# sid2364/dna-sequences-pg-extension

Hardware: AMD Instinct MI355X
Metric: k-mers/sec for k=31 count over 3 Gbase synthetic; % of HBM-read roofline (higher is better)
Workload: dtype u64; 1 GPU; config 4: k=31 count over 3000000000 synthetic bases (splitmix64 seed 0xd2a0003), unordered groups (super-k-mer partitioning), single GPU; n_bases=3000000000, k=31, distinct=2999999968

## Files before the change

dna-sequences-pg-extension_amd/binding.py:

```python
import ctypes as C
import os

import numpy as np

_HERE = os.path.dirname(os.path.abspath(__file__))
_LIB = None

OK = 0
ERR_INVALID_K = 1
ERR_QKMER_LEN_MISMATCH = 2
ERR_PREFIX_TOO_LONG = 3
ERR_QKMER_INVALID = 4
ERR_BAD_ARG = 5
ERR_TOO_LARGE = 6
ERR_NO_DEVICE = 7
ERR_OOM = 8
ERR_HIP = 9
ERR_DNA_EMPTY = 11
ERR_DNA_INVALID_CHAR = 12
DEBUG_POISON_POOL = 1
DEBUG_FORCE_SUPERKMER = 2
DEBUG_HEAVY_EXPAND = 4
DEBUG_GUARD_POOL = 8
DEBUG_NO_SPEC1 = 16
# ... 151 lines not shown
    L.dnagpu_multi_size.argtypes = [vp]
    L.dnagpu_multi_ctx.argtypes = [vp, C.c_int]
    L.dnagpu_multi_ctx.restype = vp
    L.dnagpu_multi_transport.argtypes = [vp]
    L.dnagpu_multi_transport.restype = C.c_char_p
    L.dnagpu_multi_dna_upload.argtypes = [vp, u64p, C.c_uint64, C.POINTER(vp)]
    L.dnagpu_multi_dna_synth.argtypes = [vp, C.c_uint64, C.c_uint64, C.c_uint64, C.POINTER(vp)]
    L.dnagpu_multi_dna_length.argtypes = [vp]
    L.dnagpu_multi_dna_length.restype = C.c_uint64
    L.dnagpu_multi_dna_free.argtypes = [vp, vp]
    L.dnagpu_multi_dna_free.restype = None
    L.dnagpu_count_multi.argtypes = [vp, vp, C.c_int, C.c_uint64, C.c_uint64, C.POINTER(vp)]
    L.dnagpu_count_multi_unordered.argtypes = [vp, vp, C.c_int, C.c_uint64, C.c_uint64, C.POINTER(vp)]
    L.dnagpu_device_count.restype = C.c_int
    L.dnagpu_multi_set_option.argtypes = [vp, C.c_int, C.c_double]
    L.dnagpu_multi_last_times.argtypes = [vp, C.POINTER(_MultiTimes)]
    L.dnagpu_multi_exchange_transport.argtypes = [vp]
    L.dnagpu_multi_exchange_transport.restype = C.c_char_p
    L.dnagpu_multi_rccl_ranks.argtypes = [vp]
    L.dnagpu_multi_last_phase_times.argtypes = [vp, C.c_int, C.POINTER(_PhaseTimes)]
    L.dnagpu_hist_parts.argtypes = [vp]
    L.dnagpu_hist_parts.restype = C.c_uint32
    L.dnagpu_hist_part.argtypes = [vp, C.c_uint32]
    L.dnagpu_hist_part.restype = vp
    L.dnagpu_last_phase_times.argtypes = [vp, C.POINTER(_PhaseTimes)]
    L.dnagpu_set_profiling.argtypes = [vp, C.c_int]
    L.dnagpu_set_debug.argtypes = [vp, C.c_uint]
    _LIB = L
    return L


class DnaGpuError(Exception):
    def __init__(self, code):
        self.code = code
        self.message = lib().dnagpu_strerror(code).decode()
        detail = lib().dnagpu_last_error().decode()
        super().__init__(self.message + (f" [{detail}]" if detail and code >= ERR_BAD_ARG else ""))


def _chk(rc):
    if rc != OK:
        raise DnaGpuError(rc)


def strerror(code):
    return lib().dnagpu_strerror(code).decode()


def device_count():
    return int(lib().dnagpu_device_count())


def abi_version():
    return lib().dnagpu_abi_version()


def kmer_count(n_bases, k):
    out = C.c_uint64()
    _chk(lib().dnagpu_kmer_count(n_bases, k, C.byref(out)))
    return out.value


class Filter:

    def __init__(self, kind, length=0, bits=0, pattern=""):
        self.c = _FilterC()
        self.c.kind = kind
        self.c.length = length
        self.c.bits = int(bits)
        self.c.pattern = pattern.encode()[:35]

    @staticmethod
    def equals(length, bits):
        return Filter(FILTER_EQUALS, length, bits)

    @staticmethod
    def starts_with(length, bits):
        return Filter(FILTER_STARTS_WITH, length, bits)

    @staticmethod
    def contains(pattern):
        return Filter(FILTER_CONTAINS, 0, 0, pattern)


class Dna:
    def __init__(self, ctx, handle):
        self.ctx, self.h = ctx, handle

    @property
    def n_bases(self):
        return int(lib().dnagpu_dna_length(self.h))

    @property
    def device_words(self):
        return lib().dnagpu_dna_device_words(self.h)

    def download(self):
        nw = (self.n_bases + 31) // 32
        out = np.empty(max(nw, 1), dtype=np.uint64)
        _chk(lib().dnagpu_dna_download(self.ctx.h, self.h, out.ctypes.data_as(u64p)))
        return out[:nw]

    def set_sequences(self, seq_starts):
        st = np.ascontiguousarray(seq_starts, dtype=np.uint64)
        _chk(lib().dnagpu_dna_set_sequences(self.ctx.h, self.h, st.ctypes.data_as(u64p), max(len(st) - 1, 0)))

    @property
    def n_sequences(self):
        return int(lib().dnagpu_dna_sequences(self.h))

    def free(self):
        if self.h:
            lib().dnagpu_dna_free(self.ctx.h, self.h)
            self.h = None


class Records:

    def __init__(self, ctx, h):
        self.ctx, self.h = ctx, h
        self.n_buckets = int(lib().dnagpu_records_buckets(h))
        self.offsets = np.zeros(self.n_buckets + 1, dtype=np.uint64)
        _chk(lib().dnagpu_records_offsets(h, self.offsets.ctypes.data_as(u64p)))
        self.device_ptr = lib().dnagpu_records_device(h)
        self.n_records = int(self.offsets[-1])

    def free(self):
        if self.h:
            lib().dnagpu_records_free(self.ctx.h, self.h)
            self.h = None


class _CountQueries:

    _obj = None

    def _q(self, name):
        return getattr(lib(), f"dnagpu_{self._obj}_{name}")

    def spectrum(self, n_bins):
        bins = np.zeros(max(int(n_bins), 1), dtype=np.uint64)
        _chk(self._q("spectrum")(self.ctx.h, self.h, n_bins, bins.ctypes.data_as(u64p)))
        return bins[:n_bins]

    def select(self, min_count, max_count=U64_MAX, cap=None, on_device=False, out=None):
        n = C.c_uint64()
        fn = self._q("select")
        if cap is None:
            _chk(fn(self.ctx.h, self.h, min_count, max_count, None, None, 0, C.byref(n), 0))
            cap = n.value
        if on_device:
            dk, dc = out if out is not None else (self.ctx.buffer_alloc(8 * max(cap, 1)), self.ctx.buffer_alloc(8 * max(cap, 1)))
            _chk(fn(self.ctx.h, self.h, min_count, max_count, dk, dc, cap, C.byref(n), 1))
            return n.value if out is not None else (dk, dc, n.value)
        keys = np.empty(max(cap, 1), dtype=np.uint64)
        counts = np.empty(max(cap, 1), dtype=np.uint64)
        _chk(fn(self.ctx.h, self.h, min_count, max_count, keys.ctypes.data, counts.ctypes.data, cap, C.byref(n), 0))
        m = min(n.value, cap)
        return keys[:m], counts[:m], n.value

    def top(self, n, on_device=False, out=None):
        got = C.c_uint64()
        fn = self._q("top")
        if on_device:
            dk, dc = out if out is not None else (self.ctx.buffer_alloc(8 * max(n, 1)), self.ctx.buffer_alloc(8 * max(n, 1)))
            _chk(fn(self.ctx.h, self.h, n, dk, dc, C.byref(got), 1))
            return got.value if out is not None else (dk, dc, got.value)
        rows = min(n, self.distinct)
        keys = np.empty(max(rows, 1), dtype=np.uint64)
        counts = np.empty(max(rows, 1), dtype=np.uint64)
        _chk(fn(self.ctx.h, self.h, n, keys.ctypes.data, counts.ctypes.data, C.byref(got), 0))
        return keys[:got.value], counts[:got.value]


class Hist(_CountQueries):
    _obj = "hist"

    def __init__(self, ctx, handle):
        self.ctx, self.h = ctx, handle

    @property
    def distinct(self):
        return int(lib().dnagpu_hist_distinct(self.h))

    @property
    def total(self):
        return int(lib().dnagpu_hist_total(self.h))

    @property
    def extent(self):
        return int(lib().dnagpu_hist_extent(self.h))

    @property
    def device_keys(self):
        return lib().dnagpu_hist_device_keys(self.h)

    @property
    def device_counts(self):
        return lib().dnagpu_hist_device_counts(self.h)

    @property
    def n_parts(self):
        return int(lib().dnagpu_hist_parts(self.h))

    def part_arrays(self, i):
        ph = C.c_void_p(lib().dnagpu_hist_part(self.h, i))
        return (lib().dnagpu_hist_device_keys(ph), lib().dnagpu_hist_device_counts(ph), int(lib().dnagpu_hist_extent(ph)))

    @property
    def is_sorted(self):
        return bool(lib().dnagpu_hist_is_sorted(self.h))

    def download(self, first=0, count=None, want_keys=True, want_counts=True):
        if count is None:
            count = self.distinct - first
        keys = np.empty(max(count, 1), dtype=np.uint64) if want_keys else None
        counts = np.empty(max(count, 1), dtype=np.uint64) if want_counts else None
        _chk(lib().dnagpu_hist_download(self.ctx.h, self.h, first, count,
                                        keys.ctypes.data_as(u64p) if want_keys else None,
                                        counts.ctypes.data_as(u64p) if want_counts else None))
        return (keys[:count] if want_keys else None, counts[:count] if want_counts else None)

    def sorted_view_device(self, dev_keys, dev_counts, first=0, count=None):
        if count is None:
            count = self.distinct - first
        _chk(lib().dnagpu_hist_sorted_view(self.ctx.h, self.h, first, count, dev_keys, dev_counts))

    def summary(self):
        t, u, c = C.c_uint64(), C.c_uint64(), C.c_uint64()
        _chk(lib().dnagpu_hist_summary(self.ctx.h, self.h, C.byref(t), C.byref(u), C.byref(c)))
        return t.value, self.distinct, u.value, c.value

    def merge(self, other):
        h = C.c_void_p()
        _chk(lib().dnagpu_hist_merge(self.ctx.h, self.h, other.h, C.byref(h)))
        return Hist(self.ctx, h)

    def free(self):
        if self.h:
            if self.ctx._base_debug & DEBUG_GUARD_POOL:
                self.ctx.synchronize()
            lib().dnagpu_hist_free(self.ctx.h, self.h)
            self.h = None


class Accumulator(_CountQueries):

    _obj = "acc"

    def __init__(self, ctx, k):
        self.ctx, self.h = ctx, C.c_void_p()
        _chk(lib().dnagpu_acc_create(ctx.h, k, C.byref(self.h)))

    def add(self, hist):
        _chk(lib().dnagpu_acc_add(self.ctx.h, self.h, hist.h))

    @property
    def distinct(self):
        return int(lib().dnagpu_acc_distinct(self.h))

    @property
    def total(self):
        return int(lib().dnagpu_acc_total(self.h))

    def summary(self):
        t, u, c = C.c_uint64(), C.c_uint64(), C.c_uint64()
        _chk(lib().dnagpu_acc_summary(self.ctx.h, self.h, C.byref(t), C.byref(u), C.byref(c)))
        return t.value, self.distinct, u.value, c.value

    def download(self, first=0, count=None):
        if count is None:
            count = self.distinct - first
        keys = np.empty(max(count, 1), dtype=np.uint64)
        counts = np.empty(max(count, 1), dtype=np.uint64)
        _chk(lib().dnagpu_acc_download(self.ctx.h, self.h, first, count, keys.ctypes.data_as(u64p),
                                       counts.ctypes.data_as(u64p)))
        return keys[:count], counts[:count]

    def free(self):
        if self.h:
            if self.ctx._base_debug & DEBUG_GUARD_POOL:
                self.ctx.synchronize()
            lib().dnagpu_acc_free(self.ctx.h, self.h)
            self.h = None

    def __enter__(self):
        return self

    def __exit__(self, *a):
        self.free()


class Context:
    def __init__(self, device=0):
        self.h = C.c_void_p()
        _chk(lib().dnagpu_init(device, C.byref(self.h)))
        self._base_debug = _env_debug()
        if self._base_debug:
            self.set_debug(0)

    def set_debug(self, flags):
        _chk(lib().dnagpu_set_debug(self.h, int(flags) | self._base_debug))

    def close(self):
        if self.h:
            lib().dnagpu_destroy(self.h)
            self.h = None

    def __enter__(self):
        return self

    def __exit__(self, *a):
        self.close()

    def synchronize(self):
        _chk(lib().dnagpu_synchronize(self.h))

    @property
    def stream(self):
        return lib().dnagpu_stream(self.h)

    def trim(self):
        _chk(lib().dnagpu_trim(self.h))

    def device_bytes(self):
        return int(lib().dnagpu_device_bytes(self.h))

    def set_profiling(self, on):
        _chk(lib().dnagpu_set_profiling(self.h, int(bool(on))))

    def last_phase_times(self):
        pt = _PhaseTimes()
        _chk(lib().dnagpu_last_phase_times(self.h, C.byref(pt)))
        return [(pt.names[i].decode(), float(pt.ms[i])) for i in range(pt.n)]

    def upload(self, words, n_bases):
        w = np.ascontiguousarray(words, dtype=np.uint64)
        if w.size < (n_bases + 31) // 32:
            raise ValueError("words shorter than n_bases")
        h = C.c_void_p()
        _chk(lib().dnagpu_dna_upload(self.h, w.ctypes.data_as(u64p), n_bases, C.byref(h)))
        return Dna(self, h)

    def wrap(self, dev_ptr, n_words, n_bases):
        h = C.c_void_p()
        _chk(lib().dnagpu_dna_wrap(self.h, dev_ptr, n_words, n_bases, C.byref(h)))
        return Dna(self, h)

    def _pack(self, text, n_bases, on_device):
        h = C.c_void_p()
        pos, ch = C.c_uint64(), C.create_string_buffer(1)
        rc = lib().dnagpu_dna_pack(self.h, text, n_bases, on_device, C.byref(h), C.byref(pos), ch)
        if rc == ERR_DNA_INVALID_CHAR:
            e = DnaGpuError(rc)
            e.message = f"{e.message}: {ch.raw.decode(errors='replace')}"
            e.bad_pos = pos.value
            e.bad_char = ch.raw
            e.args = (e.message,)
            raise e
        _chk(rc)
        return Dna(self, h)

    def pack(self, text):
        b = text.encode() if isinstance(text, str) else bytes(text)
        return self._pack(b, len(b), 0)

    def pack_device(self, dev_text, n_bases):
        return self._pack(C.cast(C.c_void_p(dev_text), C.c_char_p), n_bases, 1)

    def unpack(self, dna, first=0, count=None):
        if count is None:
            count = dna.n_bases - first
        buf = C.create_string_buffer(max(count, 1))
        _chk(lib().dnagpu_dna_unpack(self.h, dna.h, first, count, buf, 0))
        return buf.raw[:count].decode()

    def unpack_device(self, dna, first, count, dev_text):
        _chk(lib().dnagpu_dna_unpack(self.h, dna.h, first, count, dev_text, 1))

    def from_wire_device(self, dev_wire, wire_bytes):
        h = C.c_void_p()
        _chk(lib().dnagpu_dna_from_wire(self.h, dev_wire, wire_bytes, 1, C.byref(h)))
        return Dna(self, h)

    def to_wire_device(self, dna, dev_wire, wire_cap):
        _chk(lib().dnagpu_dna_to_wire(self.h, dna.h, dev_wire, wire_cap, 1))

    def kmers_to_text_device(self, dev_keys, n, k, dev_text):
        _chk(lib().dnagpu_kmers_to_text(self.h, dev_keys, n, k, dev_text, 1))

    def from_wire(self, wire):
        b = bytes(wire)
        h = C.c_void_p()
        _chk(lib().dnagpu_dna_from_wire(self.h, b, len(b), 0, C.byref(h)))
        return Dna(self, h)

    def to_wire(self, dna):
        n = lib().dnagpu_dna_wire_size(dna.n_bases)
        buf = C.create_string_buffer(int(n))
        _chk(lib().dnagpu_dna_to_wire(self.h, dna.h, buf, n, 0))
        return buf.raw

    def kmers_to_text(self, keys, k):
        a = np.ascontiguousarray(keys, dtype=np.uint64)
        buf = C.create_string_buffer(max(a.size * (k + 1), 1))
        _chk(lib().dnagpu_kmers_to_text(self.h, a.ctypes.data, a.size, k, buf, 0))
        raw = buf.raw
        return [raw[i * (k + 1): i * (k + 1) + k].decode() for i in range(a.size)]

    def synth(self, seed, n_bases, motif_len=0):
        h = C.c_void_p()
        _chk(lib().dnagpu_dna_synth(self.h, seed, n_bases, motif_len, C.byref(h)))
        return Dna(self, h)

    def generate_kmers(self, dna, k, first=0, count=None):
        total = kmer_count(dna.n_bases, k)
        if count is None:
            count = max(total - first, 0)
        out = np.empty(max(count, 1), dtype=np.uint64)
        _chk(lib().dnagpu_generate_kmers(self.h, dna.h, k, first, count, out.ctypes.data, 0))
        return out[:count]

    def generate_kmers_device(self, dna, k, first, count, dev_out):
        _chk(lib().dnagpu_generate_kmers(self.h, dna.h, k, first, count, dev_out, 1))

    def generate_kmers_filtered(self, dna, k, flt, first=0, count=None, cap=None, want_keys=True,
                                want_pos=True):
        total = kmer_count(dna.n_bases, k)
        if count is None:
            count = max(total - first, 0)
        if cap is None:
            cap = count
        keys = np.empty(max(cap, 1), dtype=np.uint64) if want_keys else None
        pos = np.empty(max(cap, 1), dtype=np.uint64) if want_pos else None
        n = C.c_uint64()
        _chk(lib().dnagpu_generate_kmers_filtered(
            self.h, dna.h, k, C.byref(flt.c), first, count,
            keys.ctypes.data if want_keys else None, pos.ctypes.data if want_pos else None,
            cap, C.byref(n), 0))
        m = min(n.value, cap)
        return (keys[:m] if want_keys else None, pos[:m] if want_pos else None, n.value)

    def count_matches_device(self, dna, k, flt, first, count, dev_keys=None, dev_pos=None, cap=0):
        n = C.c_uint64()
        _chk(lib().dnagpu_generate_kmers_filtered(self.h, dna.h, k, C.byref(flt.c), first, count,
                                                  dev_keys, dev_pos, cap, C.byref(n), 1))
        return n.value

    def count_kmers(self, dna, k, first=0, count=None):
        total = kmer_count(dna.n_bases, k)
        if count is None:
            count = max(total - first, 0)
        h = C.c_void_p()
        _chk(lib().dnagpu_count_kmers(self.h, dna.h, k, first, count, C.byref(h)))
        return Hist(self, h)

    def count_kmers_unordered(self, dna, k, first=0, count=None):
        total = kmer_count(dna.n_bases, k)
        if count is None:
            count = max(total - first, 0)
        h = C.c_void_p()
        _chk(lib().dnagpu_count_kmers_unordered(self.h, dna.h, k, first, count, C.byref(h)))
        return Hist(self, h)

    def count_kmers_batch(self, dna, seq_starts, k):
        st = np.ascontiguousarray(seq_starts, dtype=np.uint64)
        h = C.c_void_p()
        _chk(lib().dnagpu_count_kmers_batch(self.h, dna.h, st.ctypes.data_as(u64p), max(len(st) - 1, 0), k, C.byref(h)))
        return Hist(self, h)

    def count_kmers_table(self, dna, k):
        h = C.c_void_p()
        _chk(lib().dnagpu_count_kmers_table(self.h, dna.h, k, C.byref(h)))
        return Hist(self, h)

    def accumulator(self, k):
        return Accumulator(self, k)

    def sk_buckets(self, global_rows, k):
        return int(lib().dnagpu_sk_buckets(self.h, global_rows, k))

    def sk_records(self, dna, k, first, count, global_rows):
        r = C.c_void_p()
        _chk(lib().dnagpu_sk_records(self.h, dna.h, k, first, count, global_rows, C.byref(r)))
        return Records(self, r)

    def count_records(self, pieces, k, global_rows):
        n = len(pieces)
        ptrs = (C.c_void_p * max(n, 1))(*[C.c_void_p(int(p[0])) for p in pieces])
        lens = np.asarray([int(p[1]) for p in pieces], dtype=np.uint64)
        bks = np.asarray([int(p[2]) for p in pieces], dtype=np.uint32)
        h = C.c_void_p()
        _chk(lib().dnagpu_count_records(self.h, ptrs, lens.ctypes.data_as(u64p), bks.ctypes.data_as(C.POINTER(C.c_uint32)), n, k,
                                        global_rows, C.byref(h)))
        return Hist(self, h)

    def count_kmers_owned(self, dna, k, owner, n_owners, first=0, count=None):
        total = kmer_count(dna.n_bases, k)
        if count is None:
            count = max(total - first, 0)
        h = C.c_void_p()
        _chk(lib().dnagpu_count_kmers_owned(self.h, dna.h, k, first, count, owner, n_owners, C.byref(h)))
        return Hist(self, h)

    def count_keys_device(self, dev_keys, n, k):
        h = C.c_void_p()
        _chk(lib().dnagpu_count_keys(self.h, dev_keys, n, k, C.byref(h)))
        return Hist(self, h)

    def count_keys_device_in_range(self, dev_keys, n, k, key_min, key_max):
        h = C.c_void_p()
        _chk(lib().dnagpu_count_keys_in_range(self.h, dev_keys, n, k, key_min, key_max, C.byref(h)))
        return Hist(self, h)

    def partition_kmers(self, dna, k, first, count, n_owners):
        ptr = C.c_void_p()
        offs = np.zeros(n_owners + 1, dtype=np.uint64)
        _chk(lib().dnagpu_partition_kmers(self.h, dna.h, k, first, count, n_owners, C.byref(ptr),
                                          offs.ctypes.data_as(u64p)))
        return ptr.value, offs

    def buffer_alloc(self, nbytes):
        p = C.c_void_p()
        _chk(lib().dnagpu_buffer_alloc(self.h, nbytes, C.byref(p)))
        return p.value

    def buffer_free(self, ptr):
        lib().dnagpu_buffer_free(self.h, ptr)

    def download_bytes(self, ptr, n):
        out = np.empty(max(n, 1), dtype=np.uint8)
        _chk(lib().dnagpu_buffer_download(self.h, ptr, n, out.ctypes.data))
        return out[:n]

    def upload_bytes(self, ptr, arr):
        a = np.ascontiguousarray(arr, dtype=np.uint8)
        _chk(lib().dnagpu_buffer_upload(self.h, ptr, a.ctypes.data, a.size))

    def download_u64(self, ptr, n):
        out = np.empty(max(n, 1), dtype=np.uint64)
        _chk(lib().dnagpu_buffer_download(self.h, ptr, n * 8, out.ctypes.data))
        return out[:n]

    def upload_u64(self, ptr, arr):
        a = np.ascontiguousarray(arr, dtype=np.uint64)
        _chk(lib().dnagpu_buffer_upload(self.h, ptr, a.ctypes.data, a.size * 8))

    def kmer_hash(self, keys):
        k = np.ascontiguousarray(keys, dtype=np.uint64)
        out = np.empty(max(k.size, 1), dtype=np.uint32)
        _chk(lib().dnagpu_kmer_hash(self.h, k.ctypes.data, k.size, out.ctypes.data, 0))
        return out[:k.size]

    def kmer_hash_device(self, dev_keys, n, dev_out):
        _chk(lib().dnagpu_kmer_hash(self.h, dev_keys, n, dev_out, 1))

    def kmer_match_device(self, dev_keys, n, k, flt, dev_flags):
        _chk(lib().dnagpu_kmer_match(self.h, dev_keys, n, k, C.byref(flt.c), dev_flags, 1))

    def kmer_match(self, keys, k, flt):
        a = np.ascontiguousarray(keys, dtype=np.uint64)
        out = np.empty(max(a.size, 1), dtype=np.uint8)
        _chk(lib().dnagpu_kmer_match(self.h, a.ctypes.data, a.size, k, C.byref(flt.c), out.ctypes.data, 0))
        return out[:a.size].astype(bool)


MULTI_AUTO, MULTI_RCCL, MULTI_COPY = 0, 1, 2
MULTI_OPT_PARTS, MULTI_OPT_EMULATE_LINK_GBS, MULTI_OPT_PROBE_OWNER, MULTI_OPT_EXCHANGE_RCCL = 1, 2, 3, 4


class _BorrowedContext(Context):

    def __init__(self, handle):
        self.h = C.c_void_p(handle)
        self._base_debug = _env_debug()
        if self._base_debug:
            self.set_debug(0)

    def close(self):
        self.h = None


class Multi:

    def __init__(self, devices, transport=MULTI_AUTO):
        n = len(devices)
        arr = (C.c_int * n)(*devices)
        self.h = C.c_void_p()
        _chk(lib().dnagpu_multi_init(arr, n, transport, C.byref(self.h)))
        self.n = n
        self.ranks = [_BorrowedContext(lib().dnagpu_multi_ctx(self.h, r)) for r in range(n)]

    @property
    def transport(self):
        return lib().dnagpu_multi_transport(self.h).decode()

    @property
    def exchange_transport(self):
        return lib().dnagpu_multi_exchange_transport(self.h).decode()

    @property
    def rccl_ranks(self):
        return int(lib().dnagpu_multi_rccl_ranks(self.h))

    def set_exchange_rccl(self, mode):
        _chk(lib().dnagpu_multi_set_option(self.h, MULTI_OPT_EXCHANGE_RCCL, float(mode)))
# ... 63 lines not shown
```

dna-sequences-pg-extension_amd/csrc/kernels.hpp:

```cpp
#pragma once
#include <hip/hip_runtime.h>
#include <stdint.h>

#include "kmer_device.hpp"

namespace dnagpu {

hipError_t launch_synth(u64 *words, u64 w_begin, u64 w_end, u64 n_bases, u64 seed, u64 motif_len, hipStream_t s);
hipError_t launch_extract(const u64 *words, u64 n_words, u64 first, u64 count, int k, u64 *out_keys,
                          hipStream_t s);

constexpr int FILTER_MAX_GROUPS = 8192;
void filter_bits_geometry(u64 count, u32 *n_groups, u32 *tiles_per_group);
hipError_t launch_filter_bits_count(const u64 *words, u64 n_words, u64 first, u64 count, const FilterBits &fb,
                                    u32 *group_counts, hipStream_t s);
hipError_t launch_filter_bits_write(const u64 *words, u64 n_words, u64 first, u64 count, int k, const FilterBits &fb,
                                    const u32 *group_counts, u64 *out_keys, u64 *out_pos, u64 cap, u64 *total_out,
                                    hipStream_t s);

hipError_t launch_hash_batch(const u64 *keys, u64 n, u32 *out, hipStream_t s);
hipError_t launch_match_batch(const u64 *keys, u64 n, const FilterDev &f, uint8_t *flags, hipStream_t s);
hipError_t launch_hist_summary(const u64 *keys, const u32 *counts, u64 n, u64 *result3, hipStream_t s);

hipError_t launch_pack(const unsigned char *text, u64 n_bases, u64 *words, u64 *bad_pos, hipStream_t s);
hipError_t launch_unpack(const u64 *words, u64 first, u64 count, unsigned char *text, hipStream_t s);
hipError_t launch_kmers_to_text(const u64 *keys, u64 n, int k, unsigned char *text, hipStream_t s);
hipError_t launch_wire_swap(const u64 *src, u64 *dst, u64 n_words, u64 last_mask, hipStream_t s);

u64 scan_tmp_words(u64 n);
struct ScanSet {
    const u32 *in[4];
    u32 *out[4];
    u32 *total[4];
    u32 *tmp;
};
hipError_t launch_scan_u32_multi(const ScanSet &set, int n_arrays, u64 n, hipStream_t s);
hipError_t launch_scan_u32(const u32 *in, u32 *out, u64 n, u32 *tmp, u32 *total, hipStream_t s);

constexpr int LEAF_CAP = 6144;
constexpr int LEAF_CAP_TINY = 1024;
constexpr int LEAF_CAP_SMALL = 4096;
constexpr int LEAF_TARGET = 5800;
constexpr int MAX_SPLIT_BITS = 10;
constexpr int ROW_STRIDE = 1 << MAX_SPLIT_BITS;

struct Node {
    u32 start;
    u32 len;
    u32 meta;
    u32 split;
    u64 prefix;
    u32 child_base;
    u32 chunk_base;
};
constexpr u32 NODE_BUF = 1u << 8;
constexpr u32 NODE_TERMINAL = 1u << 9;
constexpr u32 NODE_SKIP = 1u << 10;
constexpr u32 NODE_PEEL = 1u << 11;
constexpr int NODE_STAT_WORDS = 8;

struct Chunk {
    u32 node;
    u32 off;
    u32 len;
    u32 pad;
};

struct LevelCounters {
    u32 n_next;
    u32 n_chunks;
    u32 n_split;
    u32 n_scatter;
    u32 max_bits;
    u32 n_big;
    u32 n_small;
    u32 n_tiny;
    u32 n_over;
};

hipError_t launch_plan(Node *nodes, u32 n_nodes, int level, u32 chunk_len, u32 *outc, u32 *nch,
                       LevelCounters *ctr, hipStream_t s, int skew_from = 2);
hipError_t launch_plan_level(Node *nodes, u32 n_nodes, int level, u32 chunk_len, u32 *outc, u32 *nch, u32 *scan_tmp,
                             LevelCounters *ctr, hipStream_t s, int skew_from = 2);
hipError_t launch_fill_chunks(const Node *nodes, u32 n_nodes, u32 chunk_len, const u32 *child_base,
                              const u32 *chunk_base, Node *nodes_rw, Chunk *chunks, hipStream_t s);
hipError_t launch_level_hist(const Node *nodes, const Chunk *chunks, u32 n_chunks, int src_dna,
                             const u64 *words, u64 n_words, u64 first, int k, const u64 *buf0,
                             const u64 *buf1, u32 *hist, u32 flt_lo, u32 flt_span, u32 flt_tb, u32 *vary, int multi_ref,
                             u32 stat_min_len, hipStream_t s);
hipError_t launch_level_prefix(const Node *nodes, const Chunk *chunks, u32 n_chunks, u32 n_split_nodes, u32 chunk_len,
                               u32 *hist, u32 *tot, hipStream_t s, u32 n_nodes = 0);
hipError_t launch_level_children(Node *nodes, u32 n_nodes, u32 *tot, Node *next, u32 *vary, const u64 *buf0,
                                 const u64 *buf1, u32 stat_min_len, hipStream_t s);
hipError_t launch_peel_scatter(const Node *nodes, u32 n_nodes, const Chunk *chunks, u32 n_chunks, Node *next, u64 *buf0,
                               u64 *buf1, u32 *stat, hipStream_t s);
hipError_t launch_level_scatter(const Node *nodes, const Chunk *chunks, u32 n_chunks, int src_dna,
                                const u64 *words, u64 n_words, u64 first, int k, u64 *buf0, u64 *buf1,
                                const u32 *hist, const u32 *tot, u32 flt_lo, u32 flt_span, u32 flt_tb, u32 max_bits,
                                hipStream_t s);
hipError_t launch_leaves(const Node *leaves, u32 n_leaves, u32 n_tiny, u32 n_small, u32 n_big, const u64 *buf0, const u64 *buf1,
                         u64 *cursor, u64 *seg_off, u32 *seg_cnt, u64 *out_keys, u32 *out_counts, u32 *flags,
                         u32 *scan_tmp, u32 *list, hipStream_t s, bool hashed = false, u64 out_base = 0);
int dense_max_bits();
hipError_t launch_dense_count(const u64 *words, u64 n_words, u64 first, u64 count, int bits, u32 *table, u64 *out_keys,
                              u32 *out_counts, u64 *n_out, hipStream_t s);
hipError_t launch_dense_table(const u64 *words, u64 n_words, u64 first, u64 count, int bits, u32 *table, hipStream_t s);
hipError_t launch_dense_compact(const u32 *table, int bits, u64 *out_keys, u32 *out_counts, u64 *n_out, hipStream_t s);
hipError_t launch_table_add(u32 *dst, const u32 *src, u32 n, hipStream_t s);
hipError_t launch_gather_sorted(const u64 *seg_off, const u32 *seg_cnt, const u32 *seg_pre, u32 n_leaves,
                                u64 first, u64 count, const u64 *keys, const u32 *counts, u64 *dst_keys,
                                u64 *dst_counts, hipStream_t s);

hipError_t launch_merge_insert(const u64 *keys, const u32 *counts, u64 n, u64 *tkeys, u32 *tcnt, u64 t_slots,
                               unsigned long long *ones, hipStream_t s);
hipError_t launch_merge_compact(const u64 *tkeys, const u32 *tcnt, u64 t_slots, u64 *out_keys, u32 *out_counts,
                                unsigned long long *cursor, hipStream_t s);

constexpr int ACC_SLOTS = 4096;
hipError_t launch_acc_bin(const u64 *keys, const u32 *counts, u64 n, int pbits, u32 *cursor, u64 *bins, u32 bin_cap,
                          hipStream_t s);
hipError_t launch_acc_bin_stats(const u32 *occ, const u32 *cursor, u64 P, u32 *stats, hipStream_t s);
hipError_t launch_acc_merge(u64 *table, u32 *occ, u64 P, const u32 *cursor, const u64 *bins, u32 bin_cap, int commit, u32 *stats,
                            hipStream_t s);
hipError_t launch_acc_split(const u64 *old_table, const u32 *old_occ, int old_bits, u64 *new_table, u32 *new_occ, int new_bits,
                            u32 *stats, hipStream_t s);
hipError_t launch_acc_summary(const u64 *table, const u32 *occ, u64 P, u64 *res3, hipStream_t s);
hipError_t launch_acc_gather(const u64 *table, const u32 *occ, const u64 *pre, u64 p_lo, u64 n_parts, u64 first, u64 count,
                             u64 *out_keys, u64 *out_counts, hipStream_t s);

constexpr int Q_TILE = 2048;
constexpr int Q_DIGITS = 2048;
constexpr u32 Q_LDS_BINS = 8192;
struct QHistSrc {
    const u64 *keys;
    const u32 *counts;
    u64 n;
};
struct QAccSrc {
    const u64 *table;
    const u32 *occ;
    u64 n;
};
struct QDigit {
    int spectrum;
    u64 n_bins;
    int shift;
    int has_prefix;
    int prefix_shift;
    u64 prefix;
    u32 lds_bins;
    int want_max;
};
hipError_t launch_query_digits(const QHistSrc &s, const QDigit &a, u64 *bins, u64 *maxc, hipStream_t st);
hipError_t launch_query_digits(const QAccSrc &s, const QDigit &a, u64 *bins, u64 *maxc, hipStream_t st);
hipError_t launch_query_select(const QHistSrc &s, u64 lo, u64 hi, u64 *out_keys, u64 *out_counts, u64 cap, u64 *cursor,
                               hipStream_t st);
hipError_t launch_query_select(const QAccSrc &s, u64 lo, u64 hi, u64 *out_keys, u64 *out_counts, u64 cap, u64 *cursor,
                               hipStream_t st);
hipError_t launch_query_sort(u64 *keys, u64 *counts, u32 m, hipStream_t st);

hipError_t launch_batch_marks(const u64 *starts, u64 n_seqs, u32 *marks, u64 n_mark_words, hipStream_t s);
hipError_t launch_batch_rows(const u64 *starts, u64 n_seqs, int k, u64 *rows, hipStream_t s);
hipError_t launch_batch_keys(const u64 *words, u64 n_words, const u32 *marks, u64 n_mark_words, u64 n_rows, int k, u64 *out_keys,
                             unsigned long long *cursor, hipStream_t s);

int sk_min_k();
int sk_minimizer_len(int k);
int sk_tile_rows();
int sk_max_c0();
hipError_t launch_sk_level0(bool scatter, const Chunk *chunks, u32 n_chunks, const u64 *words, u64 n_words, u64 first, int k,
                            u32 c0n, u32 b1bits, u32 r0bits, u32 *hist, const u32 *tot, void *recs, hipStream_t s,
                            u32 *aux = nullptr, const u32 *marks = nullptr, u64 n_mark_words = 0);
hipError_t launch_sk_sample_chunks(Chunk *chunks, u32 n_chunks, u32 stride, u32 len, u32 n, hipStream_t s);
int sk_slab_words();
u32 sk_slab_cap(u32 est, u64 chunk_rows, u64 sampled);
hipError_t launch_sk_slab_init(const u32 *est, u32 r0bits, u32 chunk_rows, u32 sampled, u32 n_chunks, u32 *slab, Node *nodes,
                               hipStream_t s);
hipError_t launch_sk_hist1(const Node *nodes, const Chunk *chunks, u32 n_chunks, const void *recs, u32 *hist, u32 *kcount,
                           hipStream_t s, bool by_d2 = false);
hipError_t launch_sk_scatter1(const Node *nodes, const Chunk *chunks, u32 n_chunks, const void *src, void *dst, const u32 *hist,
                              const u32 *tot, hipStream_t s, bool by_d2 = false, u32 *gcur = nullptr);
u64 sk_spec_span(u32 len, int bits);
hipError_t launch_sk_spec_regions(const Node *nodes, u32 n_nodes, u32 *spec, u32 *out, u32 *gcur, hipStream_t s,
                                  const u32 *rstart = nullptr);
hipError_t launch_sk_scatter1_spec(const Node *nodes, const Chunk *chunks, u32 n_chunks, const void *src, void *dst, u32 *gcur,
                                   const u32 *spec, u32 *kcount, u32 *over, hipStream_t s, const u32 *rstart = nullptr,
                                   const u32 *rcap = nullptr);
hipError_t launch_sk_spec_nodes(const Node *nodes, u32 n_nodes, const u32 *spec, const u32 *gcur, Node *next, u32 *over,
                                hipStream_t s, const u32 *rstart = nullptr, const u32 *rcap = nullptr);
u32 sk_sample1_len();
u32 sk_sample1_every();
hipError_t launch_sk_sampled_regions(const Node *nodes, const Chunk *samples, u32 n_samples, const void *recs, u32 n_mid, u32 *est,
                                     u32 *rcap, u32 *rstart, u32 *scan_tmp, u32 *total, hipStream_t s);
hipError_t launch_sk_heavy_finals(const Node *kids, u32 n, const u32 *kcount, Node *out, hipStream_t s);
int sk_flat_slice();
hipError_t launch_sk_take_heavy(Node *mids, const u32 *idx, u32 n_heavy, const u32 *kcount, Node *out, hipStream_t s);
hipError_t launch_sk_slice_count(const Node *buckets, u32 nb, u32 *n_slices, hipStream_t s);
hipError_t launch_sk_slice_fill(const Node *buckets, u32 nb, const u32 *slice_first, u32 *slice_rec0, u32 *slice_nrec, hipStream_t s);
hipError_t launch_sk_slice_kmers(const void *recs, const u32 *slice_rec0, const u32 *slice_nrec, u32 n_slices, u32 *slice_km,
                                 hipStream_t s);
hipError_t launch_sk_slice_nodes(const Node *buckets, u32 nb, const u32 *slice_first, const u32 *slice_koff, u32 n_slices,
                                 const u32 *total_keys, u32 key_base, int k, bool check_kmers, Node *out, u64 *n_bad, hipStream_t s);
hipError_t launch_sk_unmix(u64 *keys, u64 first, const u64 *end, u64 max_groups, int k, hipStream_t s);
hipError_t launch_sk_expand_flat(const void *recs, const u32 *slice_rec0, const u32 *slice_nrec, const u32 *slice_koff, u32 key_base,
                                 u32 n_slices, int k, u64 *keys, hipStream_t s);
int sk_regroup_tile();
hipError_t launch_sk_regroup(const Node *mids, u32 n_mids, const void *src, void *dst, Node *out_nodes, bool any_long, hipStream_t s);
hipError_t launch_sk_count(const Node *fin, const u32 *list, const u32 *list_off, u32 n_list, const void *recs, int k, u64 *n_groups,
                           u64 *seg_off, u32 *seg_cnt, u64 *out_keys, u32 *out_counts, u32 *left, hipStream_t s);

int sk_count_cap();
hipError_t launch_sk_select_flags(const Node *fin, u32 n_fin, u32 cap, u32 big_limit, u32 *f_small, u32 *f_big, u32 *k_range,
                                  u32 *k_big, hipStream_t s);
hipError_t launch_sk_select_lists(const Node *fin, u32 n_fin, u32 cap, u32 big_limit, const u32 *p_small, const u32 *p_big,
                                  const u32 *kb_range, u32 *list_small, u32 *off_small, u32 *list_big, u32 *off_big, hipStream_t s);
hipError_t launch_sk_over_flags(const Node *fin, u32 n_fin, u32 cap, u32 big_limit, const u32 *p_big, const u32 *big_status,
                                u32 *f_over, u32 *k_over, hipStream_t s);
hipError_t launch_sk_over_list(const Node *fin, u32 n_fin, const u32 *f_raw, const u32 *p_over, const u32 *kb_over, Node *over_nodes,
                               u32 *over_kbase, hipStream_t s);
hipError_t launch_sk_node_lens(const Node *nodes, u32 n, u32 *lens, hipStream_t s);
u32 sk_big_slice_records();
u64 sk_big_partial_slots();
hipError_t launch_sk_big_slices(const Node *fin, const u32 *list, u32 n_list, u32 *nsl, u32 *msl, hipStream_t s);
hipError_t launch_sk_big_slice_fill(const u32 *nsl_raw, const u32 *sfirst, u32 n_list, u32 *sl_bucket, u32 *sl_idx, hipStream_t s);
hipError_t launch_sk_count_big(const Node *fin, const u32 *list, const u32 *list_off, const u32 *nsl, const u32 *mfirst,
                               const u32 *sl_bucket, const u32 *sl_idx, u32 n_slices, u32 n_list, const void *recs, int k,
                               u64 *n_groups, u64 *seg_off, u32 *seg_cnt, u64 *out_keys, u32 *out_counts, u32 *status, u64 *part_keys,
                               u32 *part_cnts, u32 *part_n, bool any_sliced, hipStream_t s);

int scatter_tile_keys();
int scatter_threads();

}
```

dna-sequences-pg-extension_amd/csrc/sk_host.hip:

```cpp
#include "host_common.hpp"

using namespace dnagpu;

constexpr u64 SK_LEAF_MEAN = 2500;
constexpr u64 SK_MID_LIMIT = (u64)1 << 27;
#ifndef SK_MID_RECORDS_LOG2
#define SK_MID_RECORDS_LOG2 16
#endif
constexpr u32 SK_MID_RECORDS = 1u << SK_MID_RECORDS_LOG2;
constexpr u64 SK_BIG_LIMIT = 0xFFFFFFFFull;
constexpr int SK_B1_MAX = 9;

struct SkLevel {
    Node *next;
    u32 n_next;
    u32 *hist, *tot;
    Chunk *chunks;
    u32 n_chunks;
};

static int sk_level_begin(dnagpu_ctx *ctx, PoolScope &ps, Node *cur, u32 n_nodes, int bits, u32 chunk_len, SkLevel *lv)
{
    hipStream_t st = ctx->stream;
    u32 *outc = nullptr, *nch = nullptr, *scan_tmp = nullptr;
    LevelCounters *ctr = nullptr;
    RC_TRY(ps.alloc(n_nodes, &outc));
    RC_TRY(ps.alloc(n_nodes, &nch));
    RC_TRY(ps.alloc((size_t)scan_tmp_words(n_nodes), &scan_tmp));
    RC_TRY(ps.alloc(1, &ctr));
    HIP_TRY(launch_plan_level(cur, n_nodes, -bits, chunk_len, outc, nch, scan_tmp, ctr, st));
    LevelCounters hc;
    RC_TRY(read_back(ctx, &hc, ctr, sizeof hc));
    lv->n_next = hc.n_next;
    lv->n_chunks = hc.n_chunks;
    RC_TRY(ps.alloc(std::max<u32>(hc.n_chunks, 1), &lv->chunks));
    RC_TRY(ps.alloc((size_t)std::max<u32>(hc.n_chunks, 1) * ROW_STRIDE, &lv->hist));
    RC_TRY(ps.alloc((size_t)std::max<u32>(hc.n_chunks, 1) * ROW_STRIDE, &lv->tot));
    RC_TRY(ps.alloc(std::max<u32>(hc.n_next, 1), &lv->next));
    HIP_TRY(launch_fill_chunks(cur, n_nodes, chunk_len, outc, nch, cur, lv->chunks, st));
    return DNAGPU_OK;
}

struct SkHeavy {
    Node *nodes = nullptr;
    u32 n = 0;
    bool counted = true;
    void *recs = nullptr;
    u64 total = 0;
};
SkGeom dnagpu::sk_geometry(const dnagpu_ctx *ctx, u64 n, int k)
{
    SkGeom g;
    const u64 leaf_mean = std::min<u64>(SK_LEAF_MEAN, 225 * (u64)(k - sk_minimizer_len(k) + 2));
    const u64 n_final = std::max<u64>(n / leaf_mean, 16);
    const u64 n_mid = (n_final + 15) / 16;
    g.b1 = 1;
    while (g.b1 < SK_B1_MAX && ((u64)1 << g.b1) < n_mid)
        g.b1++;
    g.c0n = (u32)std::min<u64>((n_mid + ((u64)1 << g.b1) - 1) >> g.b1, (u64)sk_max_c0());
    g.r0bits = 1;
    while ((1u << g.r0bits) < g.c0n)
        g.r0bits++;
    g.mid_limit = (ctx->debug_flags & DNAGPU_DEBUG_FORCE_SUPERKMER) ? 3 * (n / ((u64)g.c0n << g.b1) + 1) : SK_MID_LIMIT;
    return g;
}

static bool sk_even(const u32 *lens, u32 n, double tol, int b1 = 0, u64 *span_out = nullptr)
{
    u64 tot = 0, big = 0, used = 0, span = 0;
    for (u32 i = 0; i < n; i++) {
        tot += lens[i];
        big = std::max<u64>(big, lens[i]);
        used += lens[i] ? 1 : 0;
        if (span_out)
            span += sk_spec_span(lens[i], b1);
    }
    if (span_out)
        *span_out = span;
    return (double)big * (double)used <= tol * (double)tot + 64.0 * (double)used;
}

static int sk_level0_begin(dnagpu_ctx *ctx, PoolScope &ps, u64 n, int r0bits, u64 chunk_target, Node **cur_out, u32 *chunk_rows_out,
                           SkLevel *l0)
{
    Node root;
    memset(&root, 0, sizeof root);
    root.len = (u32)n;
    root.meta = 32;
    Node *cur = nullptr;
    RC_TRY(ps.alloc(1, &cur));
    HIP_TRY(poke(cur, &root, sizeof root, ctx->stream));
    const u64 tile = (u64)sk_tile_rows();
    u64 chunk_rows = std::max<u64>(4 * tile, (n + chunk_target - 1) / chunk_target);
    chunk_rows = (chunk_rows + tile - 1) / tile * tile;
    prof_mark(ctx, "sk_plan0");
    RC_TRY(sk_level_begin(ctx, ps, cur, 1, r0bits, (u32)chunk_rows, l0));
    *cur_out = cur;
    *chunk_rows_out = (u32)chunk_rows;
    return DNAGPU_OK;
}

static int sk_level0(dnagpu_ctx *ctx, PoolScope &ps, const SkRows &rows, int k, const SkGeom &g, void **rec0_out, Node **coarse,
                     u32 *n_coarse, std::vector<u32> *lens_out, u64 *n_recs_out, u64 *rec0_cap = nullptr)
{
    hipStream_t st = ctx->stream;
    const dnagpu_dna *dna = rows.dna;
    const int b1 = g.b1, r0bits = g.r0bits;
    const u32 c0n = g.c0n;
    Node *cur = nullptr;
    u32 chunk_rows = 0;
    SkLevel l0;
    RC_TRY(sk_level0_begin(ctx, ps, rows.n, r0bits, 4096, &cur, &chunk_rows, &l0));
    prof_mark(ctx, "sk_hist0");
    HIP_TRY(launch_sk_level0(false, l0.chunks, l0.n_chunks, dna->words, dna->n_words, rows.first, k, c0n, (u32)b1, (u32)r0bits,
                             l0.hist, nullptr, nullptr, st, nullptr, rows.marks, rows.n_mark_words));
    prof_mark(ctx, "sk_prefix0");
    HIP_TRY(launch_level_prefix(cur, l0.chunks, l0.n_chunks, 1, chunk_rows, l0.hist, l0.tot, st));
    HIP_TRY(launch_level_children(cur, 1, l0.tot, l0.next, nullptr, nullptr, nullptr, 0, st));
    std::vector<Node> kids(l0.n_next);
    RC_TRY(read_back(ctx, kids.data(), l0.next, (size_t)l0.n_next * sizeof(Node)));
    std::vector<u32> &lens = *lens_out;
    lens.resize(kids.size());
    u64 n_recs = 0;
    for (size_t i = 0; i < kids.size(); i++) {
        lens[i] = kids[i].len;
        n_recs += kids[i].len;
    }
    if (n_recs > 0xFFFFFFFFull)
        return DNAGPU_ERR_TOO_LARGE;
    void *rec0 = nullptr;
    u64 cap = std::max<u64>(n_recs, 1);
    if (rec0_cap) {
        u64 span = 0;
        const bool even = sk_even(lens.data(), (u32)lens.size(), 1.02, b1, &span);
        if (span <= 0xFFFFFFFFull)
            cap = std::max(cap, span);
        if ((ctx->debug_flags & DNAGPU_DEBUG_SAMPLE1) || !even) {
            const u64 roomy = n_recs + n_recs / 3 + ((u64)lens.size() << b1) * 136;
            if (roomy <= 0xFFFFFFFFull)
                cap = std::max(cap, roomy);
        }
        *rec0_cap = cap;
    }
    RC_TRY(pool_alloc(ctx, (size_t)cap * 16, &rec0));
    ps.ptrs.push_back(rec0);
    prof_mark(ctx, "sk_scatter0");
    HIP_TRY(launch_sk_level0(true, l0.chunks, l0.n_chunks, dna->words, dna->n_words, rows.first, k, c0n, (u32)b1, (u32)r0bits,
                             l0.hist, l0.tot, rec0, st, nullptr, rows.marks, rows.n_mark_words));
    *rec0_out = rec0;
    *coarse = l0.next;
    *n_coarse = l0.n_next;
    *n_recs_out = n_recs;
    return DNAGPU_OK;
}

constexpr u64 SK_SLAB_MIN_ROWS = (u64)1 << 29;
static int sk_level0_slab(dnagpu_ctx *ctx, PoolScope &ps, const SkRows &rows, int k, const SkGeom &g, void **rec0_out, Node **coarse,
                          u32 *n_coarse, std::vector<u32> *lens, u64 *n_recs, u64 *rec0_cap, bool *ok)
{
    hipStream_t st = ctx->stream;
    const dnagpu_dna *dna = rows.dna;
    const u64 first = rows.first, n = rows.n;
    *ok = false;
    const u32 r0n = 1u << g.r0bits;
    const u64 tile = (u64)sk_tile_rows();
    Node *cur = nullptr;
    u32 chunk_rows = 0;
    SkLevel l0;
    RC_TRY(sk_level0_begin(ctx, ps, n, g.r0bits, 1024, &cur, &chunk_rows, &l0));
    if (l0.n_chunks == 0)
        return DNAGPU_OK;
    const u64 samp_len = 4 * tile, samp_stride = 64 * samp_len;
    const u32 n_samp = (u32)((n + samp_stride - 1) / samp_stride);
    u64 sampled = 0;
    for (u32 i = 0; i < n_samp; i++)
        sampled += std::min<u64>(samp_len, n - (u64)i * samp_stride);
    Chunk *samp = nullptr;
    u32 *est = nullptr, *slab = nullptr;
    Node *nodes = nullptr;
    RC_TRY(ps.alloc((size_t)n_samp, &samp));
    RC_TRY(ps.alloc((size_t)sk_max_c0(), &est));
    RC_TRY(ps.alloc((size_t)sk_slab_words(), &slab));
    RC_TRY(ps.alloc((size_t)r0n, &nodes));
    prof_mark(ctx, "sk_sample0");
    HIP_TRY(hipMemsetAsync(est, 0, (size_t)sk_max_c0() * sizeof(u32), st));
    HIP_TRY(launch_sk_sample_chunks(samp, n_samp, (u32)samp_stride, (u32)samp_len, (u32)n, st));
    HIP_TRY(launch_sk_level0(false, samp, n_samp, dna->words, dna->n_words, first, k, g.c0n, (u32)g.b1, (u32)g.r0bits, nullptr, nullptr,
                             nullptr, st, est, rows.marks, rows.n_mark_words));
    HIP_TRY(launch_sk_slab_init(est, (u32)g.r0bits, chunk_rows, (u32)sampled, l0.n_chunks, slab, nodes, st));
    std::vector<u32> h_est(r0n);
    RC_TRY(read_back(ctx, h_est.data(), est, (size_t)r0n * sizeof(u32)));
    u64 tot = 0, span = 0, span1 = 0;
    lens->assign(r0n, 0);
    for (u32 d = 0; d < r0n; d++) {
        tot += h_est[d];
        const u64 len = (u64)sk_slab_cap(h_est[d], chunk_rows, sampled) * l0.n_chunks;
        span += len;
        if (len > 0xFFFFFFFFull)
            return DNAGPU_OK;
        (*lens)[d] = (u32)len;
        span1 += sk_spec_span((u32)len, g.b1);
    }
    if (tot == 0 || !sk_even(h_est.data(), r0n, 1.05) || span > 0xFFFFFFFFull)
        return DNAGPU_OK;
    const u64 cap = std::max<u64>(span, span1 <= 0xFFFFFFFFull ? span1 : 0);
    void *rec0 = nullptr;
    RC_TRY(pool_alloc(ctx, (size_t)std::max<u64>(cap, 1) * 16, &rec0));
    prof_mark(ctx, "sk_scatter0");
    const hipError_t e = launch_sk_level0(true, l0.chunks, l0.n_chunks, dna->words, dna->n_words, first, k, g.c0n, (u32)g.b1,
                                          (u32)g.r0bits, nullptr, nullptr, rec0, st, slab, rows.marks, rows.n_mark_words);
    u32 status[2] = {1, 0};
    int rc = e == hipSuccess ? read_back(ctx, status, slab + 18 * (size_t)sk_max_c0(), sizeof status) : DNAGPU_ERR_HIP;
    if (rc != DNAGPU_OK || status[0] || status[1] != (u32)span || (ctx->debug_flags & DNAGPU_DEBUG_SLAB0_OVERFLOW)) {
        pool_free(ctx, rec0);
        if (e != hipSuccess)
            set_err("sk_scatter0 (slabs): %s", hipGetErrorString(e));
        return rc;
    }
    ps.ptrs.push_back(rec0);
    *rec0_out = rec0;
    *coarse = nodes;
    *n_coarse = r0n;
    *n_recs = span;
    *rec0_cap = cap;
    *ok = true;
    return DNAGPU_OK;
}

static int sk_levels12(dnagpu_ctx *ctx, PoolScope &ps, const SkGeom &g, Node *coarse, u32 n_coarse, void *rec0, u64 n_recs, u64 n,
                       void **recs, Node **fin, u32 *n_fin, SkHeavy *heavy, u64 *n_kmers, const u32 *host_lens = nullptr,
                       u64 rec0_cap = 0)
{
    hipStream_t st = ctx->stream;
    const int b1 = g.b1;
    const u64 mid_limit = g.mid_limit;
    void *rec1 = nullptr;

    u64 chunk_recs = std::max<u64>(4 * 8192, (n_recs + 4095) / 4096);
    chunk_recs = (chunk_recs + 8191) / 8192 * 8192;
    prof_mark(ctx, "sk_plan1");
    SkLevel l1;
    RC_TRY(sk_level_begin(ctx, ps, coarse, n_coarse, b1, (u32)chunk_recs, &l1));
    u32 *kcount = nullptr;
    RC_TRY(ps.alloc(std::max<u32>(l1.n_next, 1), &kcount));
    HIP_TRY(hipMemsetAsync(kcount, 0, (size_t)std::max<u32>(l1.n_next, 1) * sizeof(u32), st));
    u32 *d_lens = nullptr;
    RC_TRY(ps.alloc((size_t)l1.n_next + 4, &d_lens));
    u32 *gcur = nullptr;
    RC_TRY(ps.alloc((size_t)std::max<u32>(l1.n_chunks, 1) * ROW_STRIDE, &gcur));
    std::vector<u32> kc(l1.n_next), rcn((size_t)l1.n_next + 4);
    auto lens_to_host = [&](u32 extra) -> int {
        const size_t nb = (size_t)l1.n_next * sizeof(u32), nb2 = nb + (size_t)extra * sizeof(u32);
        if (nb + nb2 <= MAILBOX_BYTES - 8) {
            char *mb = reinterpret_cast<char *>(ctx->mailbox);
            HIP_TRY(hipMemcpyAsync(mb, kcount, nb, hipMemcpyDeviceToHost, st));
            HIP_TRY(hipMemcpyAsync(mb + nb, d_lens, nb2, hipMemcpyDeviceToHost, st));
            HIP_TRY(hipStreamSynchronize(st));
            memcpy(kc.data(), mb, nb);
            memcpy(rcn.data(), mb + nb, nb2);
        } else {
            HIP_TRY(hipMemcpyAsync(kc.data(), kcount, nb, hipMemcpyDeviceToHost, st));
            RC_TRY(read_back(ctx, rcn.data(), d_lens, nb2));
        }
        return DNAGPU_OK;
    };
    u64 span = 0;
    bool even = true;
    if (host_lens) {
        even = sk_even(host_lens, n_coarse, 1.02, b1, &span);
    }
    const bool can_spec = host_lens && !(ctx->debug_flags & DNAGPU_DEBUG_NO_SPEC1) && n_coarse <= (u32)sk_max_c0() && l1.n_chunks > 0;
    const bool force_sample = (ctx->debug_flags & DNAGPU_DEBUG_SAMPLE1) != 0;
    bool spec = can_spec && even && !force_sample && span <= rec0_cap && span <= 0xFFFFFFFFull;
    u32 *rstart = nullptr, *rcapv = nullptr;
    bool sampled = false;
    if (can_spec && (!even || force_sample) && !spec) {
        std::vector<Chunk> samp;
        const u32 slen = sk_sample1_len(), sstep = slen * sk_sample1_every();
        for (u32 i = 0; i < n_coarse; i++)
            for (u64 off = 0; off < host_lens[i]; off += sstep) {
                Chunk c;
                c.node = i;
                c.off = (u32)off;
                c.len = (u32)std::min<u64>(slen, host_lens[i] - off);
                c.pad = 0;
                samp.push_back(c);
            }
        Chunk *d_samp = nullptr;
        u32 *est = nullptr, *stmp = nullptr, *tot1 = nullptr;
        RC_TRY(ps.alloc(std::max<size_t>(samp.size(), 1), &d_samp));
        RC_TRY(ps.alloc((size_t)l1.n_next, &est));
        RC_TRY(ps.alloc((size_t)l1.n_next, &rcapv));
        RC_TRY(ps.alloc((size_t)l1.n_next, &rstart));
        RC_TRY(ps.alloc((size_t)scan_tmp_words(l1.n_next), &stmp));
        RC_TRY(ps.alloc(1, &tot1));
        prof_mark(ctx, "sk_sample1");
        if (!samp.empty())
            HIP_TRY(hipMemcpyAsync(d_samp, samp.data(), samp.size() * sizeof(Chunk), hipMemcpyHostToDevice, st));
        HIP_TRY(launch_sk_sampled_regions(coarse, d_samp, (u32)samp.size(), rec0, l1.n_next, est, rcapv, rstart, stmp, tot1, st));
        u32 total = 0;
        RC_TRY(read_back(ctx, &total, tot1, sizeof total));
        u64 chk = 0;
        for (u32 i = 0; i < n_coarse; i++)
            chk += host_lens[i];
        if ((u64)total >= chk && (u64)total <= rec0_cap) {
            span = total;
            spec = sampled = true;
        }
    }
    bool moved = false;
    if (spec) {
        u32 *sp = nullptr;
        RC_TRY(ps.alloc((size_t)2 * n_coarse, &sp));
        u32 *status = d_lens + l1.n_next;
        prof_mark(ctx, "sk_spec1");
        HIP_TRY(launch_sk_spec_regions(coarse, n_coarse, sp, status, gcur, st, sampled ? rstart : nullptr));
        RC_TRY(pool_alloc(ctx, (size_t)std::max<u64>(std::max(n_recs, span), 1) * 16, &rec1));
        ps.ptrs.push_back(rec1);
        prof_mark(ctx, "sk_scatter1");
        HIP_TRY(launch_sk_scatter1_spec(coarse, l1.chunks, l1.n_chunks, rec0, rec1, gcur, sp, kcount, status + 2, st,
                                        sampled ? rstart : nullptr, sampled ? rcapv : nullptr));
        HIP_TRY(launch_sk_spec_nodes(coarse, n_coarse, sp, gcur, l1.next, status + 2, st, sampled ? rstart : nullptr,
                                     sampled ? rcapv : nullptr));
        HIP_TRY(launch_sk_node_lens(l1.next, l1.n_next, d_lens, st));
        RC_TRY(lens_to_host(3));
        const u32 *stw = rcn.data() + l1.n_next;
        if ((!sampled && stw[0] != (u32)span) || (!sampled && stw[1]) || stw[2] || (ctx->debug_flags & DNAGPU_DEBUG_SPEC1_OVERFLOW)) {
            spec = false;
            HIP_TRY(hipMemsetAsync(kcount, 0, (size_t)std::max<u32>(l1.n_next, 1) * sizeof(u32), st));
        } else {
            moved = true;
        }
    }
    if (!spec) {
        prof_mark(ctx, "sk_hist1");
        HIP_TRY(launch_sk_hist1(coarse, l1.chunks, l1.n_chunks, rec0, l1.hist, kcount, st));
        prof_mark(ctx, "sk_prefix1");
        HIP_TRY(launch_level_prefix(coarse, l1.chunks, l1.n_chunks, n_coarse, (u32)chunk_recs, l1.hist, l1.tot, st, n_coarse));
        HIP_TRY(launch_level_children(coarse, n_coarse, l1.tot, l1.next, nullptr, nullptr, nullptr, 0, st));
        HIP_TRY(launch_sk_node_lens(l1.next, l1.n_next, d_lens, st));
        RC_TRY(lens_to_host(0));
    }
    const bool forced = (ctx->debug_flags & DNAGPU_DEBUG_FORCE_SUPERKMER) != 0;
    auto is_heavy = [&](u32 i) { return kc[i] > mid_limit || (!forced && rcn[i] > SK_MID_RECORDS); };
    u64 run = 0, heaviest = 0;
    for (u32 i = 0; i < l1.n_next; i++) {
        run += kc[i];
        if (is_heavy(i))
            heaviest = std::max<u64>(heaviest, std::max<u64>(kc[i], mid_limit + 1));
    }
    if (n != 0 && run != n) {
        set_err("super-k-mer partition lost rows: %llu of %llu", (unsigned long long)run, (unsigned long long)n);
        return DNAGPU_ERR_INTERNAL;
    }
    if (run > 0xFFFFFFFFull)
        return DNAGPU_ERR_TOO_LARGE;
    *n_kmers = run;
    std::vector<u32> heavy_idx;
    if (heaviest > mid_limit) {
        for (u32 i = 0; i < l1.n_next; i++)
            if (is_heavy(i)) {
                heavy_idx.push_back(i);
                heavy->total += kc[i];
            }
        if (((ctx->debug_flags & DNAGPU_DEBUG_HEAVY_EXPAND) && heavy->total * 2 > run) || heavy_idx.size() > 32768)
            return DNAGPU_SK_SKEWED;
    }

    if (!moved) {
        if (!rec1) {
            RC_TRY(pool_alloc(ctx, (size_t)std::max<u64>(n_recs, 1) * 16, &rec1));
            ps.ptrs.push_back(rec1);
        }
        prof_mark(ctx, "sk_scatter1");
        HIP_TRY(hipMemcpyAsync(gcur, l1.tot, (size_t)std::max<u32>(l1.n_chunks, 1) * ROW_STRIDE * sizeof(u32), hipMemcpyDeviceToDevice, st));
        HIP_TRY(launch_sk_scatter1(coarse, l1.chunks, l1.n_chunks, rec0, rec1, l1.hist, l1.tot, st, false, gcur));
    }

    const u32 nh = (u32)heavy_idx.size();
    const bool heavy_expand = (ctx->debug_flags & DNAGPU_DEBUG_HEAVY_EXPAND) != 0;
    SkLevel lh;
    memset(&lh, 0, sizeof lh);
    u32 *kcount2 = nullptr;
    Node *hnodes = nullptr;
    if (nh) {
        u32 *d_idx = nullptr;
        RC_TRY(ps.alloc((size_t)nh, &d_idx));
        RC_TRY(ps.alloc((size_t)nh, &hnodes));
        HIP_TRY(hipMemcpyAsync(d_idx, heavy_idx.data(), (size_t)nh * sizeof(u32), hipMemcpyHostToDevice, st));
        HIP_TRY(launch_sk_take_heavy(l1.next, d_idx, nh, kcount, hnodes, st));
        HIP_TRY(hipStreamSynchronize(st));
        if (heavy_expand) {
            heavy->nodes = hnodes;
            heavy->n = nh;
            heavy->recs = rec1;
        } else {
            u64 hrecs = 0;
            for (u32 i : heavy_idx)
                hrecs += rcn[i];
            u64 chunk_h = std::max<u64>(4 * 8192, (hrecs + 4095) / 4096);
            chunk_h = (chunk_h + 8191) / 8192 * 8192;
            prof_mark(ctx, "sk_heavy_split");
            RC_TRY(sk_level_begin(ctx, ps, hnodes, nh, 4, (u32)chunk_h, &lh));
            RC_TRY(ps.alloc(std::max<u32>(lh.n_next, 1), &kcount2));
            HIP_TRY(hipMemsetAsync(kcount2, 0, (size_t)std::max<u32>(lh.n_next, 1) * sizeof(u32), st));
            HIP_TRY(launch_sk_hist1(hnodes, lh.chunks, lh.n_chunks, rec1, lh.hist, kcount2, st, true));
            HIP_TRY(launch_level_prefix(hnodes, lh.chunks, lh.n_chunks, nh, (u32)chunk_h, lh.hist, lh.tot, st, nh));
            HIP_TRY(launch_level_children(hnodes, nh, lh.tot, lh.next, nullptr, nullptr, nullptr, 0, st));
            HIP_TRY(launch_sk_scatter1(hnodes, lh.chunks, lh.n_chunks, rec1, rec0, lh.hist, lh.tot, st, true));
            heavy->total = 0;
        }
    }
    Node *fn = nullptr;
    RC_TRY(ps.alloc((size_t)l1.n_next * 16 + lh.n_next, &fn));
    prof_mark(ctx, "sk_regroup");
    bool any_long = false;
    for (u32 i = 0; i < l1.n_next && !any_long; i++)
        any_long = rcn[i] > (u32)sk_regroup_tile();
    HIP_TRY(launch_sk_regroup(l1.next, l1.n_next, rec1, rec0, fn, any_long, st));
    if (lh.n_next)
        HIP_TRY(launch_sk_heavy_finals(lh.next, lh.n_next, kcount2, fn + (size_t)l1.n_next * 16, st));
    if (nh == 0 || !heavy_expand)
        ps.free_now(rec1);
    *recs = rec0;
    *fin = fn;
    *n_fin = l1.n_next * 16 + lh.n_next;
    return DNAGPU_OK;
}

static int count_sk_tail(dnagpu_ctx *ctx, PoolScope &ps, void *recs, Node *fin, u32 n_fin, const SkHeavy &heavy, u64 n, int k,
                         dnagpu_hist *h)
{
    hipStream_t st = ctx->stream;
    const u32 n_heavy = heavy.n;
    prof_mark(ctx, "sk_select");
    const u32 cap = (u32)sk_count_cap();
    const u32 big_limit = (u32)SK_BIG_LIMIT;
    u32 *f_small = nullptr, *f_big = nullptr, *f_over = nullptr, *f_over_raw = nullptr, *k_over = nullptr, *k_range = nullptr,
        *scan_tmp = nullptr, *totals = nullptr, *list_small = nullptr, *off_small = nullptr, *list_big = nullptr, *off_big = nullptr;
    RC_TRY(ps.alloc((size_t)n_fin, &f_small));
    RC_TRY(ps.alloc((size_t)n_fin, &f_big));
    RC_TRY(ps.alloc((size_t)n_fin, &k_range));
    RC_TRY(ps.alloc((size_t)scan_tmp_words(n_fin) * 4, &scan_tmp));
    RC_TRY(ps.alloc(8, &totals));
    RC_TRY(ps.alloc((size_t)n_fin, &list_small));
    RC_TRY(ps.alloc((size_t)n_fin, &off_small));
    RC_TRY(ps.alloc((size_t)n_fin, &f_over));
    HIP_TRY(launch_sk_select_flags(fin, n_fin, cap, big_limit, f_small, f_big, k_range, f_over, st));
    {
        ScanSet ss;
        u32 *arr[4] = {f_small, f_big, k_range, f_over};
        for (int a = 0; a < 4; a++) {
            ss.in[a] = arr[a];
            ss.out[a] = arr[a];
            ss.total[a] = totals + a;
        }
        ss.tmp = scan_tmp;
        HIP_TRY(launch_scan_u32_multi(ss, 4, n_fin, st));
    }
    u32 ht[4] = {0, 0, 0, 0};
    RC_TRY(read_back(ctx, ht, totals, sizeof ht));
    const u32 n_small = ht[0], n_big = ht[1];
    const u64 small_keys = ht[2];
    const u64 out_cap = n + ht[3];
    RC_TRY(ps.alloc((size_t)std::max<u32>(n_big, 1), &list_big));
    RC_TRY(ps.alloc((size_t)std::max<u32>(n_big, 1), &off_big));
    HIP_TRY(launch_sk_select_lists(fin, n_fin, cap, big_limit, f_small, f_big, k_range, list_small, off_small, list_big, off_big, st));

    u64 *cursor = nullptr, *ok = nullptr;
    u32 *oc = nullptr;
    RC_TRY(ps.alloc(3, &cursor));
    RC_TRY(ps.alloc((size_t)out_cap, &ok));
    RC_TRY(ps.alloc((size_t)out_cap, &oc));
    {
        const u64 init[3] = {small_keys, 0, 0};
        HIP_TRY(poke(cursor, init, sizeof init, st));
    }
    u64 *seg_off = nullptr;
    u32 *seg_cnt = nullptr;
    u64 *seg_off_fin = nullptr;
    u32 *seg_cnt_fin = nullptr;
    RC_TRY(ps.alloc((size_t)std::max<u32>(n_fin, 1), &seg_off_fin));
    RC_TRY(ps.alloc((size_t)std::max<u32>(n_fin, 1), &seg_cnt_fin));
    HIP_TRY(hipMemsetAsync(seg_cnt_fin, 0, (size_t)n_fin * sizeof(u32), st));
    HIP_TRY(hipMemsetAsync(seg_off_fin, 0, (size_t)n_fin * sizeof(u64), st));
    u32 *big_status = nullptr;
    RC_TRY(ps.alloc((size_t)std::max<u32>(n_big, 1), &big_status));
    if (n_big) {
        prof_mark(ctx, "sk_count_big");
        u32 *nsl = nullptr, *sfirst = nullptr, *mfirst = nullptr, *sl_bucket = nullptr, *sl_idx = nullptr, *part_n = nullptr, *part_cnts = nullptr;
        u64 *part_keys = nullptr;
        RC_TRY(ps.alloc((size_t)n_big, &nsl));
        RC_TRY(ps.alloc((size_t)n_big, &sfirst));
        RC_TRY(ps.alloc((size_t)n_big, &mfirst));
        HIP_TRY(launch_sk_big_slices(fin, list_big, n_big, nsl, mfirst, st));
        HIP_TRY(launch_scan_u32(nsl, sfirst, n_big, scan_tmp, totals + 6, st));
        HIP_TRY(launch_scan_u32(mfirst, mfirst, n_big, scan_tmp, totals + 7, st));
        u32 hs[2] = {0, 0};
        RC_TRY(read_back(ctx, hs, totals + 6, sizeof hs));
        const u32 n_slices = hs[0], n_part = hs[1];
        RC_TRY(ps.alloc((size_t)std::max<u32>(n_slices, 1), &sl_bucket));
        RC_TRY(ps.alloc((size_t)std::max<u32>(n_slices, 1), &sl_idx));
        RC_TRY(ps.alloc((size_t)std::max<u32>(n_part, 1), &part_n));
        RC_TRY(ps.alloc((size_t)std::max<u32>(n_part, 1) * sk_big_partial_slots(), &part_keys));
        RC_TRY(ps.alloc((size_t)std::max<u32>(n_part, 1) * sk_big_partial_slots(), &part_cnts));
        HIP_TRY(launch_sk_big_slice_fill(nsl, sfirst, n_big, sl_bucket, sl_idx, st));
        HIP_TRY(launch_sk_count_big(fin, list_big, off_big, nsl, mfirst, sl_bucket, sl_idx, n_slices, n_big, recs, k, cursor + 2,
                                    seg_off_fin, seg_cnt_fin, ok, oc, big_status, part_keys, part_cnts, part_n, n_part > 0, st));
    }
    prof_mark(ctx, "sk_select_over");
    RC_TRY(ps.alloc((size_t)n_fin, &f_over_raw));
    RC_TRY(ps.alloc((size_t)n_fin, &k_over));
    HIP_TRY(launch_sk_over_flags(fin, n_fin, cap, big_limit, f_big, big_status, f_over_raw, k_over, st));
    {
        ScanSet ss;
        memset(&ss, 0, sizeof ss);
        ss.in[0] = f_over_raw;
        ss.out[0] = f_over;
        ss.total[0] = totals + 4;
        ss.in[1] = k_over;
        ss.out[1] = k_over;
        ss.total[1] = totals + 5;
        ss.tmp = scan_tmp;
        HIP_TRY(launch_scan_u32_multi(ss, 2, n_fin, st));
    }
    u32 ho[2] = {0, 0};
    RC_TRY(read_back(ctx, ho, totals + 4, sizeof ho));
    const u32 n_over = ho[0];
    const u64 over_keys = ho[1];
    Node *over_nodes = nullptr;
    u32 *over_kbase = nullptr;
    RC_TRY(ps.alloc((size_t)std::max<u32>(n_over, 1), &over_nodes));
    RC_TRY(ps.alloc((size_t)std::max<u32>(n_over, 1), &over_kbase));
    HIP_TRY(launch_sk_over_list(fin, n_fin, f_over_raw, f_over, k_over, over_nodes, over_kbase, st));
    TreeResult tr;
    memset(&tr, 0, sizeof tr);
    if (n_over + n_heavy > 0) {
        const u64 tree_keys = over_keys + heavy.total;
        if (tree_keys > 0xFFFFFFFFull)
            return DNAGPU_ERR_TOO_LARGE;
        const u32 n_tree = n_over + n_heavy;
        u64 *kbuf = nullptr;
        Node *knodes = nullptr;
        RC_TRY(ps.alloc((size_t)tree_keys, &kbuf));
        RC_TRY(ps.alloc((size_t)n_tree, &knodes));
        prof_mark(ctx, "sk_expand_flat");
        for (int part = 0; part < 2; part++) {
            const u32 nb = part == 0 ? n_over : n_heavy;
            if (nb == 0)
                continue;
            const void *rbuf = part == 0 ? recs : heavy.recs;
            const Node *bk = part == 0 ? over_nodes : heavy.nodes;
            u32 *sfirst = nullptr, *stmp = nullptr, *stot = nullptr;
            RC_TRY(ps.alloc((size_t)nb, &sfirst));
            RC_TRY(ps.alloc((size_t)scan_tmp_words(nb), &stmp));
            RC_TRY(ps.alloc(2, &stot));
            HIP_TRY(launch_sk_slice_count(bk, nb, sfirst, st));
            HIP_TRY(launch_scan_u32(sfirst, sfirst, nb, stmp, stot, st));
            u32 n_slices = 0;
            RC_TRY(read_back(ctx, &n_slices, stot, 4));
            u32 *d_r0 = nullptr, *d_nr = nullptr, *d_ko = nullptr, *ktmp = nullptr;
            RC_TRY(ps.alloc((size_t)std::max<u32>(n_slices, 1), &d_r0));
            RC_TRY(ps.alloc((size_t)std::max<u32>(n_slices, 1), &d_nr));
            RC_TRY(ps.alloc((size_t)std::max<u32>(n_slices, 1), &d_ko));
            RC_TRY(ps.alloc((size_t)scan_tmp_words(std::max<u32>(n_slices, 1)), &ktmp));
            HIP_TRY(launch_sk_slice_fill(bk, nb, sfirst, d_r0, d_nr, st));
            HIP_TRY(launch_sk_slice_kmers(rbuf, d_r0, d_nr, n_slices, d_ko, st));
            HIP_TRY(launch_scan_u32(d_ko, d_ko, n_slices, ktmp, stot + 1, st));
            const u32 key_base = part == 0 ? 0u : (u32)over_keys;
            HIP_TRY(launch_sk_slice_nodes(bk, nb, sfirst, d_ko, n_slices, stot + 1, key_base, k, part == 0 || heavy.counted,
                                          knodes + (part == 0 ? 0 : n_over), cursor + 1, st));
            HIP_TRY(launch_sk_expand_flat(rbuf, d_r0, d_nr, d_ko, key_base, n_slices, k, kbuf, st));
        }
        RC_TRY(run_tree(ctx, ps, nullptr, 0, tree_keys, k, kbuf, 0, &tr, 0, 0, true, 0, ~0u, 0, knodes, n_tree, 2));
    }
#ifdef DNAGPU_STAMPS
    fprintf(stderr, "[sk select] n_fin %u small %u big %u (k-mers of big %u) over %u (keys %llu) heavy %u (keys %llu) tree nodes %u tiny %u small %u big %u\n",
            n_fin, n_small, n_big, ht[3], n_over, (unsigned long long)over_keys, n_heavy, (unsigned long long)heavy.total, tr.n_nodes,
            tr.n_tiny, tr.n_small, tr.n_big);
#endif
    const u32 n_segs = n_fin + tr.n_nodes;
    RC_TRY(ps.alloc((size_t)n_segs, &seg_off));
    RC_TRY(ps.alloc((size_t)n_segs, &seg_cnt));
    HIP_TRY(hipMemcpyAsync(seg_cnt, seg_cnt_fin, (size_t)n_fin * sizeof(u32), hipMemcpyDeviceToDevice, st));
    HIP_TRY(hipMemcpyAsync(seg_off, seg_off_fin, (size_t)n_fin * sizeof(u64), hipMemcpyDeviceToDevice, st));
    if (tr.n_nodes > 0) {
        u32 *flags = nullptr, *ltmp = nullptr, *cls_list = nullptr;
        RC_TRY(ps.alloc((size_t)tr.n_nodes + 1, &flags));
        RC_TRY(ps.alloc((size_t)scan_tmp_words(tr.n_nodes), &ltmp));
        RC_TRY(ps.alloc((size_t)tr.n_nodes, &cls_list));
        prof_mark(ctx, "leaves");
        HIP_TRY(launch_leaves(tr.nodes, tr.n_nodes, tr.n_tiny, tr.n_small, tr.n_big, tr.buf0, tr.buf1, cursor, seg_off + n_fin,
                              seg_cnt + n_fin, ok, oc, flags, ltmp, cls_list, st, true, small_keys));
        HIP_TRY(launch_sk_unmix(ok, small_keys, cursor, tr.n_keys, k, st));
    }
    prof_mark(ctx, "sk_count");
    u32 *left = nullptr;
    RC_TRY(ps.alloc((size_t)2 * n_small + 1, &left));
    HIP_TRY(launch_sk_count(fin, list_small, off_small, n_small, recs, k, cursor + 2, seg_off, seg_cnt, ok, oc, left, st));
#ifdef DNAGPU_STAMPS
    {
        u32 nl = 0;
        RC_TRY(read_back(ctx, &nl, left + 2 * (size_t)n_small, 4));
        fprintf(stderr, "[sk count] %u small buckets, %u left to sk_count by sk_count_clean\n", n_small, nl);
    }
#endif
    prof_mark(ctx, "end");
    u64 fin_ctr[3] = {0, 0, 0};
    RC_TRY(read_back(ctx, fin_ctr, cursor, 24));
    const u64 extent = fin_ctr[0];
    const u64 total_groups = fin_ctr[2] + (extent - small_keys);
    if (fin_ctr[1] != 0) {
        set_err("super-k-mer count: %llu buckets whose records expand to a different number of k-mers than the partition counted",
                (unsigned long long)fin_ctr[1]);
        return DNAGPU_ERR_INTERNAL;
    }
    if (extent > out_cap) {
        set_err("super-k-mer count: %llu output slots used, %llu allocated", (unsigned long long)extent, (unsigned long long)out_cap);
        return DNAGPU_ERR_INTERNAL;
    }
    if (total_groups > n) {
        set_err("super-k-mer count: %llu groups for %llu rows", (unsigned long long)total_groups, (unsigned long long)n);
        return DNAGPU_ERR_INTERNAL;
    }
    h->total = n;
    hist_adopt(ps, h, ok, oc, seg_off, seg_cnt, n_segs, total_groups, false, extent);
    return DNAGPU_OK;
}

int dnagpu::count_sk(dnagpu_ctx *ctx, const SkRows &rows, int k, dnagpu_hist *h, u64 n_kmers_expected)
{
    PoolScope ps(ctx);
    const SkGeom g = sk_geometry(ctx, std::max<u64>(n_kmers_expected, 1), k);
    void *rec0 = nullptr, *recs = nullptr;
    Node *coarse = nullptr, *fin = nullptr;
    u32 n_coarse = 0, n_fin = 0;
    u64 n_recs = 0, n_kmers = 0;
    SkHeavy heavy;
    u64 rec0_cap = 0;
    std::vector<u32> lens;
    bool slabs = false;
    const unsigned dbg = ctx->debug_flags;
    if (!(dbg & DNAGPU_DEBUG_NO_SLAB0) && (rows.n >= SK_SLAB_MIN_ROWS || (dbg & (DNAGPU_DEBUG_SLAB0 | DNAGPU_DEBUG_SLAB0_OVERFLOW))))
        RC_TRY(sk_level0_slab(ctx, ps, rows, k, g, &rec0, &coarse, &n_coarse, &lens, &n_recs, &rec0_cap, &slabs));
    if (!slabs)
        RC_TRY(sk_level0(ctx, ps, rows, k, g, &rec0, &coarse, &n_coarse, &lens, &n_recs, &rec0_cap));
    RC_TRY(sk_levels12(ctx, ps, g, coarse, n_coarse, rec0, n_recs, n_kmers_expected, &recs, &fin, &n_fin, &heavy, &n_kmers,
                       lens.size() == n_coarse ? lens.data() : nullptr, rec0_cap));
    return count_sk_tail(ctx, ps, recs, fin, n_fin, heavy, n_kmers_expected, k, h);
}

u64 dnagpu::sk_received_cap(const std::vector<u64> &blen, u32 n_coarse, const SkGeom &g)
{
    u64 n_recs = 0, span = 0;
    for (u32 d = 0; d < n_coarse; d++) {
        n_recs += blen[d];
        span += sk_spec_span((u32)std::min<u64>(blen[d], 0xFFFFFFFFull), g.b1);
    }
    return span <= 0xFFFFFFFFull ? std::max(n_recs, span) : n_recs;
}

int dnagpu::count_sk_received(dnagpu_ctx *ctx, void *rec0, const std::vector<u64> &boff, const std::vector<u64> &blen, const SkGeom &g,
                              int k, dnagpu_hist *h, u64 rec0_cap)
{
    hipStream_t st = ctx->stream;
    PoolScope ps(ctx);
    ps.ptrs.push_back(rec0);
    const u32 n_coarse = 1u << g.r0bits;
    const u64 n_recs = boff[n_coarse];
    std::vector<Node> hn(n_coarse);
    for (u32 d = 0; d < n_coarse; d++) {
        memset(&hn[d], 0, sizeof(Node));
        hn[d].start = (u32)boff[d];
        hn[d].len = (u32)blen[d];
        hn[d].meta = (u32)(32 - g.r0bits);
    }
    Node *coarse = nullptr;
    RC_TRY(ps.alloc((size_t)n_coarse, &coarse));
    HIP_TRY(hipMemcpyAsync(coarse, hn.data(), (size_t)n_coarse * sizeof(Node), hipMemcpyHostToDevice, st));
    HIP_TRY(hipStreamSynchronize(st));
    void *recs = nullptr;
    Node *fin = nullptr;
    u32 n_fin = 0;
    u64 n_kmers = 0;
    SkHeavy heavy;
    std::vector<u32> lens(n_coarse);
    for (u32 d = 0; d < n_coarse; d++)
        lens[d] = (u32)blen[d];
    int rc = sk_levels12(ctx, ps, g, coarse, n_coarse, rec0, n_recs, 0, &recs, &fin, &n_fin, &heavy, &n_kmers, lens.data(), rec0_cap);
    if (rc == DNAGPU_SK_SKEWED) {
        heavy = SkHeavy();
        heavy.nodes = coarse;
        heavy.n = n_coarse;
        heavy.recs = rec0;
        heavy.total = n_kmers;
        heavy.counted = false;
        n_fin = 0;
        rc = DNAGPU_OK;
    }
    RC_TRY(rc);
    return count_sk_tail(ctx, ps, recs, fin, n_fin, heavy, n_kmers, k, h);
}

static int count_sk_records(dnagpu_ctx *ctx, const void *const *pieces, const u64 *piece_len, const u32 *piece_bucket, u32 n_pieces,
                            int k, u64 global_rows, dnagpu_hist *h)
{
    hipStream_t st = ctx->stream;
    const SkGeom g = sk_geometry(ctx, global_rows, k);
    const u32 n_coarse = 1u << g.r0bits;
    std::vector<u64> blen(n_coarse, 0), boff(n_coarse + 1, 0);
    for (u32 i = 0; i < n_pieces; i++) {
        if (piece_bucket[i] >= g.c0n || (piece_len[i] && !pieces[i]))
            return DNAGPU_ERR_BAD_ARG;
        blen[piece_bucket[i]] += piece_len[i];
    }
    for (u32 d = 0; d < n_coarse; d++)
        boff[d + 1] = boff[d] + blen[d];
    const u64 n_recs = boff[n_coarse];
    if (n_recs > 0xFFFFFFFFull)
        return DNAGPU_ERR_TOO_LARGE;
    if (n_recs == 0) {
        h->total = 0;
        return DNAGPU_OK;
    }
    void *rec0 = nullptr;
    const u64 cap0 = sk_received_cap(blen, n_coarse, g);
    RC_TRY(pool_alloc(ctx, (size_t)cap0 * 16, &rec0));
    std::vector<u64> fill(boff.begin(), boff.end() - 1);
    for (u32 i = 0; i < n_pieces; i++)
        if (piece_len[i]) {
            const hipError_t e = hipMemcpyAsync(static_cast<char *>(rec0) + fill[piece_bucket[i]] * 16, pieces[i], (size_t)piece_len[i] * 16,
                                                hipMemcpyDeviceToDevice, st);
            if (e != hipSuccess) {
                pool_free(ctx, rec0);
                set_err("record pieces: %s", hipGetErrorString(e));
                return DNAGPU_ERR_HIP;
            }
            fill[piece_bucket[i]] += piece_len[i];
        }
    return count_sk_received(ctx, rec0, boff, blen, g, k, h, cap0);
}

extern "C" int dnagpu_sk_buckets(const dnagpu_ctx *ctx, uint64_t global_rows, int k)
{
    if (!ctx || k < sk_min_k() || k > 32 || global_rows == 0 || global_rows > 0xFFFFFFFFull)
        return 0;
    return (int)sk_geometry(ctx, global_rows, k).c0n;
}

extern "C" int dnagpu_sk_records(dnagpu_ctx *ctx, const dnagpu_dna *dna, int k, uint64_t first, uint64_t count,
                                 uint64_t global_rows, dnagpu_records **out)
{
    return guarded([&]() -> int {
    if (!ctx || !dna || !out || k < sk_min_k() || k > 32 || global_rows < count || global_rows == 0 || global_rows > 0xFFFFFFFFull)
        return DNAGPU_ERR_BAD_ARG;
    RC_TRY(check_range(dna, k, first, count));
    HIP_TRY(hipSetDevice(ctx->device));
    const SkGeom g = sk_geometry(ctx, global_rows, k);
    std::unique_ptr<dnagpu_records> r(new (std::nothrow) dnagpu_records());
    if (!r)
        return DNAGPU_ERR_OOM;
    r->off.assign((size_t)g.c0n + 1, 0);
    if (count > 0) {
        PoolScope ps(ctx);
        void *rec0 = nullptr;
        Node *coarse = nullptr;
        u32 n_coarse = 0;
        u64 n_recs = 0;
        std::vector<u32> lens;
        prof_begin(ctx);
        const int rc = sk_level0(ctx, ps, SkRows{dna, first, count, nullptr, 0}, k, g, &rec0, &coarse, &n_coarse, &lens, &n_recs);
        prof_mark(ctx, "end");
        prof_end(ctx);
        RC_TRY(rc);
        for (u32 d = 0; d < g.c0n; d++)
            r->off[d + 1] = r->off[d] + (d < lens.size() ? lens[d] : 0);
        const hipError_t se = hipStreamSynchronize(ctx->stream);
        if (r->off[g.c0n] != n_recs || se != hipSuccess) {
            set_err("super-k-mer level 0: %llu records in the buckets, %llu counted (%s)", (unsigned long long)r->off[g.c0n],
                    (unsigned long long)n_recs, hipGetErrorString(se));
            return se != hipSuccess ? DNAGPU_ERR_HIP : DNAGPU_ERR_INTERNAL;
        }
        ps.release(rec0);
        r->recs = rec0;
    }
    *out = r.release();
    return DNAGPU_OK;
    });
}

extern "C" uint32_t dnagpu_records_buckets(const dnagpu_records *r) { return r ? (uint32_t)(r->off.size() - 1) : 0; }
extern "C" int dnagpu_records_offsets(const dnagpu_records *r, uint64_t *offsets)
{
    if (!r || !offsets)
        return DNAGPU_ERR_BAD_ARG;
    for (size_t i = 0; i < r->off.size(); i++)
        offsets[i] = r->off[i];
    return DNAGPU_OK;
}
extern "C" void *dnagpu_records_device(const dnagpu_records *r) { return r ? r->recs : nullptr; }
extern "C" void dnagpu_records_free(dnagpu_ctx *ctx, dnagpu_records *r)
{
    if (!r)
        return;
    if (ctx)
        pool_free(ctx, r->recs);
    delete r;
}

extern "C" int dnagpu_count_records(dnagpu_ctx *ctx, const void *const *pieces, const uint64_t *piece_len,
                                    const uint32_t *piece_bucket, uint32_t n_pieces, int k, uint64_t global_rows, dnagpu_hist **out)
{
    return guarded([&]() -> int {
    if (!ctx || !out || (n_pieces && (!pieces || !piece_len || !piece_bucket)) || k < sk_min_k() || k > 32 || global_rows == 0 ||
        global_rows > 0xFFFFFFFFull)
        return DNAGPU_ERR_BAD_ARG;
    HIP_TRY(hipSetDevice(ctx->device));
    HistPtr h = hist_new(0, false);
    if (!h)
        return DNAGPU_ERR_OOM;
    prof_begin(ctx);
    const int rc = count_sk_records(ctx, pieces, piece_len, piece_bucket, n_pieces, k, global_rows, h.get());
    prof_end(ctx);
    RC_TRY(rc);
    *out = h.release();
    return DNAGPU_OK;
    });
}
```

dna-sequences-pg-extension_amd/csrc/superkmer_kernels.hip:

```cpp
#include <algorithm>
#include <cstdlib>
#include <type_traits>

#include "kernels.hpp"

namespace dnagpu {

constexpr int SK_NT = 256;
constexpr int SKW_ROWS = 63 * 32;
constexpr int SK_TILE_ROWS = (SK_NT / 64) * SKW_ROWS;
constexpr int SK_MAX_C0 = 256;
constexpr int SKW_LIST = 768;
__host__ __device__ constexpr u32 sk_plain_max(int w) { return (u32)(2 * SKW_ROWS * 17 / (10 * (w + 1))) < (u32)SKW_LIST ? (u32)(2 * SKW_ROWS * 17 / (10 * (w + 1))) : (u32)SKW_LIST; }

int sk_tile_rows() { return SK_TILE_ROWS; }
int sk_max_c0() { return SK_MAX_C0; }
int sk_count_cap() { return 4096; }

typedef unsigned long long ull2_t __attribute__((ext_vector_type(2)));

constexpr int SK_REC_MULTI_BIT = 58;
constexpr int SK_POS_SHIFT = 39;
constexpr u32 SK_POS_MASK = 31u;
constexpr u32 SK_GPOS_MASK = 63u;
// ... 195 lines not shown
    const int lane = threadIdx.x & 63;
    u32 r0 = (u32)lane * 32;
    asm volatile("" : "+v"(r0));
    u32 lb = 0;
    u32 kprev = key.prev_last;
    const u32 k0 = key(0);
    u32 kcur = k0;
#pragma unroll 8
    for (int j = 0; j < 32; j++) {
        const bool brk = j == 0 ? (lane == 0 || kcur != kprev) : kcur != kprev;
        if (brk)
            lb = r0 + (u32)j + 1u;
        kprev = kcur;
        if (j < 31)
            kcur = key(j + 1);
    }
    const u32 before = wave_prev(wave_incl_max(lb));
    f.ns0 = before ? before - 1u : 0u;
    const bool first_break = lane == 0 || k0 != key.prev_last;
    f.c0 = first_break ? 0u : (r0 - f.ns0) % lmax;
    if (first_break)
        f.ns0 = r0;
}

template <int W, typename Keys, typename Emit>
__device__ __forceinline__ void sk_records_all(const SkFront<W> &f, const Keys &key, u32 lmax, Emit &&emit)
{
    u32 r0 = (u32)(threadIdx.x & 63) * 32;
    asm volatile("" : "+v"(r0));
    u32 c = f.c0;
    u32 kprev = 0, kcur = key(0);
#pragma unroll 8
    for (int j = 0; j < 32; j++) {
        const u32 nxt = j < 31 ? key(j + 1) : key.next_first;
        bool end = false;
        if ((u32)j < f.n_valid) {
            if (j > 0 && kcur != kprev)
                c = 0;
            end = r0 + (u32)j + 1 == f.n_rows || nxt != kcur || c + 1 == lmax;
        }
        emit(j, end, r0 + (u32)j, c + 1, f.hm[j], kcur);
        c = end ? 0u : c + 1;
        kprev = kcur;
        kcur = nxt;
    }
}

template <int W, typename Keys, typename Emit>
__device__ __forceinline__ void sk_records(const SkFront<W> &f, const Keys &key, u32 lmax, Emit &&emit)
{
    u32 r0 = (u32)(threadIdx.x & 63) * 32;
    asm volatile("" : "+v"(r0));
    u32 c = f.c0;
    u32 kprev = 0, kcur = key(0);
#pragma unroll 8
    for (int j = 0; j < 32; j++) {
        const u32 nxt = j < 31 ? key(j + 1) : key.next_first;
        if ((u32)j < f.n_valid) {
            if (j > 0 && kcur != kprev)
                c = 0;
            const bool last = r0 + (u32)j + 1 == f.n_rows;
            const bool end = last || nxt != kcur || c + 1 == lmax;
            if (end) {
                emit(j, r0 + (u32)j, c + 1, f.hm[j], kcur);
                c = 0;
            } else {
                c++;
            }
        }
        kprev = kcur;
        kcur = nxt;
    }
}

template <int W, bool BATCH>
__device__ __forceinline__ u32 sk_uniform_value(const SkFront<W> &f, const u64 *__restrict__ words, u64 n_words, u64 pos0, u32 mmask)
{
    const int lane = threadIdx.x & 63;
    u32 x = 0, y = f.hm[0];
#pragma unroll 2
    for (int j = 1; j < 32; j++) {
        x |= f.hm[j] ^ f.hm[0];
        if (BATCH)
            y &= f.hm[j];
    }
    const u32 h0 = (u32)__builtin_amdgcn_readfirstlane((int)f.hm[0]) >> 7;
    const bool same = lane == 63 || ((x >> 7) == 0 && (f.hm[0] >> 7) == h0 && (!BATCH || (y & 64u)));
    if (__ballot(!same))
        return ~0u;
    const u64 pos = pos0 + (u64)lane * 32;
    const u64 w = pos >> 5;
    const unsigned sh = (unsigned)(pos & 31) * 2;
    const u64 w0 = w < n_words ? words[w] : 0, w1 = w + 1 < n_words ? words[w + 1] : 0;
    u64 lo = w0, hi = w1;
    if (sh) {
        const u64 w2 = w + 2 < n_words ? words[w + 2] : 0;
        lo = (w0 >> sh) | (w1 << (64 - sh));
        hi = (w1 >> sh) | (w2 << (64 - sh));
    }
    const u32 v0 = (u32)sk_shr128(lo, hi, 2u * (f.hm[0] & SK_GPOS_MASK)) & mmask;
    u32 d = 0;
#pragma unroll 2
    for (int j = 1; j < 32; j++)
        d |= ((u32)sk_shr128(lo, hi, 2u * (f.hm[j] & SK_GPOS_MASK)) & mmask) ^ v0;
    const u32 V = (u32)__builtin_amdgcn_readfirstlane((int)v0);
    const bool ok = lane == 63 || (d == 0 && v0 == V);
    return __ballot(!ok) ? ~0u : V;
}

template <int W, bool BATCH>
__device__ __forceinline__ void sk_hist0_general(SkFront<W> &f, const u64 *__restrict__ words, u64 n_words, u64 pos0, u32 lmax, u32 mmask,
                                              u32 c0n, u32 *h )
{
    SkKeys<W, BATCH, true> vk(f, words, n_words, pos0, mmask);
    sk_front_open<W>(f, vk, lmax);
    vk.forget();
    if ((threadIdx.x & 63) < 63)
        sk_records<W>(f, vk, lmax, [&](int, u32, u32, u32 hmin, u32 v) {
            if (!BATCH || v != ~0u)
                atomicAdd(&h[sk_digit0(sk_digit_word(hmin), c0n)], 1u);
        });
}

template <int W, bool BATCH>
__global__ __launch_bounds__(SK_NT, 4) void sk_hist0_kernel(const Chunk *__restrict__ chunks, u32 n_chunks,
                                                         const u64 *__restrict__ words, u64 n_words, u64 first,
                                                         u32 lmax, u32 mmask, u32 c0n, u32 b1mask, u32 r0n ,
                                                         u32 *__restrict__ hist, u32 *__restrict__ accum ,
                                                         const u32 *__restrict__ marks, u64 n_mark_words)
{
    __shared__ u32 h[SK_MAX_C0 + 64];
    if (blockIdx.x >= n_chunks)
        return;
    const Chunk ch = chunks[blockIdx.x];
    const int wave = threadIdx.x >> 6, lane = threadIdx.x & 63;
    for (u32 d = threadIdx.x; d < r0n; d += SK_NT)
        h[d] = 0;
    __syncthreads();
    for (u32 t0 = (u32)wave * SKW_ROWS; t0 < ch.len; t0 += SK_TILE_ROWS) {
        const u32 n_rows = ch.len - t0 < (u32)SKW_ROWS ? ch.len - t0 : (u32)SKW_ROWS;
        SkFront<W> f;
        sk_front<W, BATCH>(f, words, n_words, first + ch.off + t0, n_rows, lmax, mmask, nullptr, marks, n_mark_words);
        bool plain = f.plain;
        const u32 nf = lane == 62 ? ~f.hm[31] : f.next_first;
        if (plain) {
            u32 cnt = 0;
#pragma unroll
            for (int j = 0; j < 32; j++)
                cnt += ((j < 31 ? f.hm[j + 1] : nf) != f.hm[j]) ? 1u : 0u;
            plain = wave_sum(lane < 63 ? cnt : 0u) <= sk_plain_max(W);
        }
        if (plain) {
            if (lane < 63) {
#pragma unroll
                for (int j = 0; j < 32; j++) {
                    const u32 nxt = j < 31 ? f.hm[j + 1] : nf;
                    const u32 d0 = sk_digit0(sk_digit_word(f.hm[j]), c0n);
                    atomicAdd(&h[nxt != f.hm[j] && (!BATCH || f.hm[j] >= 64u) ? d0 : (u32)SK_MAX_C0 + (u32)lane], 1u);
                }
            }
        } else {
            SkFront<W> fm = f;
            const u32 uv = fm.plain ? sk_uniform_value<W, BATCH>(fm, words, n_words, first + ch.off + t0, mmask) : ~0u;
            if (uv != ~0u) {
                if (lane == 0)
                    atomicAdd(&h[sk_digit0(sk_digit_word(fm.hm[0]), c0n)], ((u32)SKW_ROWS + lmax - 1u) / lmax);
            } else {
                sk_hist0_general<W, BATCH>(fm, words, n_words, first + ch.off + t0, lmax, mmask, c0n, h);
            }
        }
    }
    __syncthreads();
    if (accum) {
        for (u32 d = threadIdx.x; d < r0n; d += SK_NT)
            if (h[d])
                atomicAdd(&accum[d], h[d]);
        return;
    }
    u32 *row = hist + (u64)blockIdx.x * ROW_STRIDE;
    for (u32 d = threadIdx.x; d < r0n; d += SK_NT)
        row[d] = h[d];
}

struct SkBuild {
    u64 *wl;
    const u64 *wsh;
    u32 *gpos;
    const u32 *gend;
    ull2_t *recs;
    u32 fo, c0n, b1mask, mmask;
    int k, dbg;
};

template <bool BATCH>
__device__ __forceinline__ bool sk_build(const SkBuild &b, u32 wrun, int mode)
{
    const bool exact = mode != 0;
    const int dbg = b.dbg;
    (void)dbg;
    bool dropped = false;
    if (SK_DBG(2))
        return false;
    for (u32 e = threadIdx.x & 63u; e < wrun; e += 64) {
        const u64 en = b.wl[e];
        const u32 key = (u32)(en >> 32);
        if (BATCH && (exact ? key < 64u : key == ~0u))
            continue;
        const u32 end_row = (u32)en & 0xFFFFu;
        u32 v = key, hmin = key;
        if (exact) {
            const u32 xq = (end_row & ~31u) + (key & SK_GPOS_MASK) + b.fo;
            v = (u32)funnel(b.wsh[xq >> 5], b.wsh[(xq >> 5) + 1], (xq & 31u) * 2u) & b.mmask;
        } else {
            hmin = sk_hash_of(v);
        }
        const SkDigits dg = sk_digits(hmin, v, b.c0n, b.b1mask);
        const u32 gslot = atomicAdd(&b.gpos[dg.d0], 1u);
        u32 start = ((u32)en >> 16) & 0xFFFFu;
        if (mode == 2)
            start = e ? ((u32)b.wl[e - 1] & 0xFFFFu) + 1u : 0u;
        const u32 len = end_row - start + 1u;
        const u32 q = start + b.fo;
        const u32 wi = q >> 5, sh = (q & 15u) * 2u;
        const u64 a0 = b.wsh[wi], a1 = b.wsh[wi + 1], a2 = b.wsh[wi + 2];
        const bool odd = (q & 16u) != 0;
        const u32 e0 = odd ? (u32)(a0 >> 32) : (u32)a0, e1 = odd ? (u32)a1 : (u32)(a0 >> 32),
                  e2 = odd ? (u32)(a1 >> 32) : (u32)a1, e3 = odd ? (u32)a2 : (u32)(a1 >> 32),
                  e4 = odd ? (u32)(a2 >> 32) : (u32)a2;
        u64 lo = ((u64)__builtin_amdgcn_alignbit(e2, e1, sh) << 32) | __builtin_amdgcn_alignbit(e1, e0, sh);
        u64 hi = ((u64)__builtin_amdgcn_alignbit(e4, e3, sh) << 32) | __builtin_amdgcn_alignbit(e3, e2, sh);
        const u32 nb = len + (u32)b.k - 1;
        if (nb < 32) {
            lo &= ((u64)1 << (2 * nb)) - 1;
            hi = 0;
        } else {
            hi &= ((u64)1 << (2 * (nb - 32))) - 1;
        }
        const u32 mpos = (end_row & ~31u) + (key & SK_GPOS_MASK) - start;
        const u32 tag = exact ? (mpos & SK_POS_MASK) << (SK_POS_SHIFT - 32) : 1u << (SK_REC_MULTI_BIT - 32);
        hi |= ((u64)(len - 1) << 44) | ((u64)dg.d1 << 49) | ((u64)dg.d2 << 59) | ((u64)tag << 32);
        ull2_t r;
        r.x = lo;
        r.y = hi;
        if (gslot >= b.gend[dg.d0])
            dropped = true;
        else if (!SK_DBG(1))
            b.recs[gslot] = r;
        else if (r.x == 0x1234567 && r.y == 0x89)
            b.recs[0] = r;
    }
    return dropped;
}

template <int W, bool BATCH, bool BYV>
__device__ __forceinline__ bool sk_scatter0_walk(SkFront<W> &f, const SkBuild &bx, const u64 *__restrict__ words, u64 n_words,
                                                 u64 tile_pos, u32 lmax)
{
    const u64 below = ((u64)1 << (threadIdx.x & 63)) - 1;
    u64 *wl = bx.wl;
    bool dropped = false;
    SkKeys<W, BATCH, BYV> key(f, words, n_words, tile_pos, bx.mmask);
    sk_front_open<W>(f, key, lmax);
    for (int n_pass = BYV ? 1 : 4, pass = 0; pass < n_pass; pass++) {
        const int jlo = pass * (32 / n_pass), jhi = jlo + 32 / n_pass;
        u32 wrun = 0;
        key.forget();
        sk_records_all<W>(f, key, lmax, [&](int j, bool end_any, u32 end_row, u32 len, u32, u32 kj) {
            const bool end = end_any && j >= jlo && j < jhi;
            const u64 b = __ballot(end);
            if (end) {
                const u32 pos = wrun + (u32)__popcll(b & below);
                if (pos < (u32)SKW_LIST)
                    wl[pos] = ((u64)kj << 32) | ((u64)(end_row + 1 - len) << 16) | (u64)end_row;
            }
            wrun += (u32)__popcll(b);
        });
        if (wrun > (u32)SKW_LIST) {
            n_pass = 4;
            pass = -1;
            sk_wave_fence();
            continue;
        }
        sk_wave_fence();
        if (sk_build<BATCH>(bx, wrun, BYV ? 0 : 1))
            dropped = true;
        sk_wave_fence();
    }
    return dropped;
}
template <int W, bool BATCH>
__device__ __forceinline__ bool sk_scatter0_general(SkFront<W> &f, const SkBuild &bx, const u64 *__restrict__ words, u64 n_words,
                                                    u64 tile_pos, u32 lmax)
{
    return sk_scatter0_walk<W, BATCH, true>(f, bx, words, n_words, tile_pos, lmax);
}

template <int W, bool BATCH>
__global__ __launch_bounds__(SK_NT, 4) void sk_scatter0_kernel(const Chunk *__restrict__ chunks, u32 n_chunks,
                                                            const u64 *__restrict__ words, u64 n_words, u64 first, int k,
                                                            u32 lmax, u32 mmask, u32 c0n, u32 b1mask, u32 r0n,
                                                            const u32 *__restrict__ hist, const u32 *__restrict__ tot,
                                                            ull2_t *__restrict__ recs, int dbg,
                                                            u32 *__restrict__ slab ,
                                                            const u32 *__restrict__ marks, u64 n_mark_words)
{
    __shared__ u32 gpos[SK_MAX_C0];
    __shared__ u32 gend[SK_MAX_C0], gbeg[SK_MAX_C0];
    __shared__ u64 wsh_all[SK_NT / 64][66];
    __shared__ u64 list_all[SK_NT / 64][SKW_LIST + 64];
    if (blockIdx.x >= n_chunks)
        return;
    const int tid = threadIdx.x, wave = tid >> 6, lane = tid & 63;
    const Chunk ch = chunks[blockIdx.x];
    if (slab) {
        for (u32 d = tid; d < r0n; d += SK_NT) {
            const u32 cap = slab[d];
            const u32 base = cap ? atomicAdd(&slab[SK_MAX_C0 + 16 * d], cap) : 0u;
            gpos[d] = base;
            gbeg[d] = base;
            gend[d] = base + cap;
        }
    } else {
        const u32 *hrow = hist + (u64)blockIdx.x * ROW_STRIDE;
        const u32 *trow = tot;
        for (u32 d = tid; d < r0n; d += SK_NT) {
            gpos[d] = trow[d] + hrow[d];
            gend[d] = ~0u;
        }
    }
    __syncthreads();
    u64 *wsh = wsh_all[wave], *wl = list_all[wave];
    bool dropped = false;
    SkBuild bx;
    bx.wl = wl;
    bx.wsh = wsh;
    bx.gpos = gpos;
    bx.gend = gend;
    bx.recs = recs;
    bx.fo = 0;
    bx.c0n = c0n;
    bx.b1mask = b1mask;
    bx.mmask = mmask;
    bx.k = k;
    bx.dbg = dbg;
    for (u32 t0 = (u32)wave * SKW_ROWS; t0 < ch.len; t0 += SK_TILE_ROWS) {
        const u32 n_rows = ch.len - t0 < (u32)SKW_ROWS ? ch.len - t0 : (u32)SKW_ROWS;
        const u64 tile_pos = first + ch.off + t0;
        const u32 fo = (u32)(tile_pos & 31);
        SkFront<W> f;
        sk_front<W, BATCH>(f, words, n_words, tile_pos, n_rows, lmax, mmask, wsh, marks, n_mark_words);
        bx.fo = fo;
        auto build = [&](u32 wrun, int mode) {
            if (sk_build<BATCH>(bx, wrun, mode))
                dropped = true;
        };
        if (f.plain) {
            const u32 nf = lane == 62 ? ~f.hm[31] : f.next_first;
            u32 cnt = 0;
#pragma unroll
            for (int j = 0; j < 32; j++)
                cnt += ((j < 31 ? f.hm[j + 1] : nf) != f.hm[j]) ? 1u : 0u;
            cnt = lane < 63 ? cnt : 0u;
            const u32 incl = wave_incl_scan(cnt);
            const u32 wrun = (u32)__builtin_amdgcn_readlane((int)incl, 63);
            if (wrun <= sk_plain_max(W)) {
                u32 p = incl - cnt;
                const u32 dummy = (u32)SKW_LIST + (u32)lane;
                u32 r0 = (u32)lane * 32;
                asm volatile("" : "+v"(r0));
#pragma unroll
                for (int j = 0; j < 32; j++) {
                    const bool end = ((j < 31 ? f.hm[j + 1] : nf) != f.hm[j]) && lane < 63;
                    wl[end ? p : dummy] = ((u64)f.hm[j] << 32) | (u64)(r0 + (u32)j);
                    p += end ? 1u : 0u;
                }
                sk_wave_fence();
                build(wrun, 2);
                sk_wave_fence();
                continue;
            }
        }
        {
            SkFront<W> fm = f;
            const SkBuild bm = bx;
            const u32 uv = fm.plain ? sk_uniform_value<W, BATCH>(fm, words, n_words, tile_pos, mmask) : ~0u;
            if (uv != ~0u) {
                const u32 n_rec = ((u32)SKW_ROWS + lmax - 1u) / lmax;
                for (u32 e = (u32)lane; e < n_rec; e += 64) {
                    const u32 s0 = e * lmax, e1 = (s0 + lmax < (u32)SKW_ROWS ? s0 + lmax : (u32)SKW_ROWS) - 1u;
                    wl[e] = ((u64)uv << 32) | (u64)((s0 << 16) | e1);
                }
                sk_wave_fence();
                if (sk_build<BATCH>(bm, n_rec, 0))
                    dropped = true;
                sk_wave_fence();
            } else if (sk_scatter0_general<W, BATCH>(fm, bm, words, n_words, tile_pos, lmax)) {
                dropped = true;
            }
        }
    }
    if (slab) {
        if (dropped)
            slab[18 * SK_MAX_C0] = 1u;
        __syncthreads();
        ull2_t null_rec;
        null_rec.x = 0;
        null_rec.y = (unsigned long long)1 << 63;
        for (u32 d = (u32)wave; d < r0n; d += SK_NT / 64) {
            const u32 e = gend[d], u = gpos[d] < e ? gpos[d] : e;
            for (u32 i = u + (u32)lane; i < e; i += 64)
                __builtin_nontemporal_store(null_rec, &recs[i]);
            if (lane == 0 && u > gbeg[d])
                atomicAdd(&slab[17 * SK_MAX_C0 + d], u - gbeg[d]);
        }
    }
}

__global__ __launch_bounds__(256) void sk_sample_chunks_kernel(Chunk *__restrict__ chunks, u32 n_chunks, u32 stride, u32 len, u32 n)
{
    const u32 i = blockIdx.x * blockDim.x + threadIdx.x;
    if (i >= n_chunks)
        return;
    const u64 off = (u64)i * stride;
    Chunk c;
    c.node = 0;
    c.off = (u32)off;
    c.len = off >= (u64)n ? 0u : (u32)((u64)len < (u64)n - off ? (u64)len : (u64)n - off);
    c.pad = 0;
    chunks[i] = c;
}

__host__ __device__ inline u32 sk_isqrt(u64 v)
{
    u64 r = 0, bit = (u64)1 << 62;
    while (bit > v)
        bit >>= 2;
    while (bit) {
        if (v >= r + bit) {
            v -= r + bit;
            r = (r >> 1) + bit;
        } else {
            r >>= 1;
        }
        bit >>= 2;
    }
    return (u32)r;
}
__host__ __device__ inline u32 sk_slab_cap_of(u32 est, u64 chunk_rows, u64 sampled)
{
    if (est == 0)
        return 0;
    const u64 e = ((u64)est * chunk_rows) / sampled + 1;
    return (u32)((e + e / 32 + 6 * (u64)sk_isqrt(e) + 24 + 7) & ~(u64)7);
}
u32 sk_slab_cap(u32 est, u64 chunk_rows, u64 sampled) { return sk_slab_cap_of(est, chunk_rows, sampled); }

__global__ __launch_bounds__(SK_MAX_C0) void sk_slab_init_kernel(const u32 *__restrict__ est, u32 r0n, u32 chunk_rows, u32 sampled,
                                                                u32 n_chunks, u32 child_meta, u32 *__restrict__ slab,
                                                                Node *__restrict__ nodes)
{
    __shared__ u64 sc[SK_MAX_C0];
    const u32 d = threadIdx.x;
    const u32 cap = d < r0n ? sk_slab_cap_of(est[d], chunk_rows, sampled) : 0u;
    sc[d] = (u64)cap * n_chunks;
    __syncthreads();
    if (d == 0) {
        u64 run = 0;
        for (u32 i = 0; i < (u32)SK_MAX_C0; i++) {
            const u64 c = sc[i];
            sc[i] = run;
            run += c;
        }
        slab[18 * SK_MAX_C0] = 0;
        slab[18 * SK_MAX_C0 + 1] = (u32)(run < 0xFFFFFFFFull ? run : 0xFFFFFFFFull);
    }
    __syncthreads();
    if (d < r0n) {
        const u32 start = (u32)(sc[d] < 0xFFFFFFFFull ? sc[d] : 0xFFFFFFFFull);
        slab[d] = cap;
        slab[SK_MAX_C0 + 16 * d] = start;
        slab[17 * SK_MAX_C0 + d] = 0;
        Node o;
        o.start = start;
        o.len = cap * n_chunks;
        o.meta = child_meta;
        o.split = 0;
        o.prefix = 0;
        o.child_base = 0;
        o.chunk_base = 0;
        nodes[d] = o;
    }
}

constexpr int SK1_NT = 1024;
__global__ __launch_bounds__(SK1_NT) void sk_hist1_kernel(const Node *__restrict__ nodes, const Chunk *__restrict__ chunks,
                                                          u32 n_chunks, const ull2_t *__restrict__ recs,
                                                          u32 *__restrict__ hist, u32 *__restrict__ kcount, int shift)
{
    __shared__ u32 h[ROW_STRIDE];
    __shared__ u32 kc[ROW_STRIDE];
    if (blockIdx.x >= n_chunks)
        return;
    const Chunk ch = chunks[blockIdx.x];
    const Node nd = nodes[ch.node];
    const u32 R = 1u << nd.split;
    for (u32 d = threadIdx.x; d < R; d += SK1_NT) {
        h[d] = 0;
        kc[d] = 0;
    }
    __syncthreads();
    const u64 *hi = reinterpret_cast<const u64 *>(recs + (u64)nd.start + ch.off) + 1;
    u32 i = threadIdx.x;
    for (; i + 3u * SK1_NT < ch.len; i += 4u * SK1_NT) {
        u64 m[4];
#pragma unroll
        for (int j = 0; j < 4; j++)
            m[j] = __builtin_nontemporal_load(&hi[(u64)(i + (u32)j * SK1_NT) * 2]);
#pragma unroll
        for (int j = 0; j < 4; j++) {
            if (m[j] >> 63)
                continue;
            const u32 d1 = (u32)(m[j] >> shift) & (R - 1);
            atomicAdd(&h[d1], 1u);
            atomicAdd(&kc[d1], (u32)((m[j] >> 44) & 31) + 1u);
        }
    }
    for (; i < ch.len; i += SK1_NT) {
        const u64 m = __builtin_nontemporal_load(&hi[(u64)i * 2]);
        if (m >> 63)
            continue;
        const u32 d1 = (u32)(m >> shift) & (R - 1);
        atomicAdd(&h[d1], 1u);
        atomicAdd(&kc[d1], (u32)((m >> 44) & 31) + 1u);
    }
    __syncthreads();
    u32 *row = hist + (u64)blockIdx.x * ROW_STRIDE;
    for (u32 d = threadIdx.x; d < R; d += SK1_NT) {
        row[d] = h[d];
        if (kc[d])
            atomicAdd(&kcount[nd.child_base + d], kc[d]);
    }
}

constexpr u32 SK1_SAMPLE_LEN = 1024, SK1_SAMPLE_EVERY = 8;
u32 sk_sample1_len() { return SK1_SAMPLE_LEN; }
u32 sk_sample1_every() { return SK1_SAMPLE_EVERY; }
__global__ __launch_bounds__(SK1_NT) void sk_sample1_kernel(const Node *__restrict__ nodes, const Chunk *__restrict__ chunks,
                                                            u32 n_chunks, const ull2_t *__restrict__ recs, u32 *__restrict__ est)
{
    __shared__ u32 h[ROW_STRIDE];
    if (blockIdx.x >= n_chunks)
        return;
    const Chunk ch = chunks[blockIdx.x];
    const Node nd = nodes[ch.node];
    const u32 R = 1u << nd.split;
    for (u32 d = threadIdx.x; d < R; d += SK1_NT)
        h[d] = 0;
    __syncthreads();
    const u64 *hi = reinterpret_cast<const u64 *>(recs + (u64)nd.start + ch.off) + 1;
    for (u32 i = threadIdx.x; i < ch.len; i += SK1_NT) {
        const u64 m = __builtin_nontemporal_load(&hi[(u64)i * 2]);
        if (!(m >> 63))
            atomicAdd(&h[(u32)(m >> 49) & (R - 1)], 1u);
    }
    __syncthreads();
    for (u32 d = threadIdx.x; d < R; d += SK1_NT)
        if (h[d])
            atomicAdd(&est[nd.child_base + d], h[d]);
}

__global__ __launch_bounds__(256) void sk_sampled_caps_kernel(const u32 *__restrict__ est, u32 n_mid, u32 *__restrict__ rcap)
{
    const u32 i = blockIdx.x * blockDim.x + threadIdx.x;
    if (i >= n_mid)
        return;
    const u64 e = est[i];
    const u64 cap = e * SK1_SAMPLE_EVERY + 5ull * SK1_SAMPLE_EVERY * sk_isqrt(e) + 128ull + 7ull;
    rcap[i] = (u32)(cap < 0xFFFFFFF8ull ? cap : 0xFFFFFFF8ull) & ~7u;
}

constexpr int SK1_ITEMS = 8;
constexpr int SK1_TILE = SK1_NT * SK1_ITEMS;
constexpr int SK1_STAGE = SK1_TILE / 2 + 64;
template <bool SPEC>
__global__ __launch_bounds__(SK1_NT, 8) void sk_scatter1_kernel(const Node *__restrict__ nodes, const Chunk *__restrict__ chunks,
                                                             u32 n_chunks, const ull2_t *__restrict__ src_all,
                                                             ull2_t *__restrict__ dst_all, const u32 *__restrict__ hist,
                                                             const u32 *__restrict__ tot, int shift, u32 *__restrict__ gcur,
                                                             const u32 *__restrict__ spec, u32 *__restrict__ kcount,
                                                             u32 *__restrict__ over, const u32 *__restrict__ rstart,
                                                             const u32 *__restrict__ rcapv )
{
    __shared__ u32 cnt[ROW_STRIDE];
    __shared__ u32 glim[SPEC ? ROW_STRIDE : 1];
    __shared__ u32 gadj[ROW_STRIDE];
    __shared__ u32 gpos[SPEC ? 1 : ROW_STRIDE];
    __shared__ __attribute__((aligned(16))) ull2_t stage[SK1_STAGE];
    unsigned short *idx = reinterpret_cast<unsigned short *>(stage);
    u64 *c64 = reinterpret_cast<u64 *>(stage);
    u32 kacc = 0;
    __shared__ u32 wtmp[SK1_NT / 64];
    __shared__ u32 split[4];
    if (blockIdx.x >= n_chunks)
        return;
    int tid = threadIdx.x;
    const Chunk ch = chunks[blockIdx.x];
    const Node nd = nodes[ch.node];
    const u32 R = 1u << nd.split;
    const u32 *hrow = hist + (u64)blockIdx.x * ROW_STRIDE;
    const u32 *trow = tot + (u64)nd.chunk_base * ROW_STRIDE;
    u32 *gc = gcur ? gcur + (u64)nd.chunk_base * ROW_STRIDE : nullptr;
    if (!SPEC && !gc)
        for (u32 d = tid; d < R; d += SK1_NT)
            gpos[d] = trow[d] + hrow[d];
    const ull2_t *src = src_all + (u64)nd.start + ch.off;
    const u32 dmask = R - 1;
    bool dropped = false;
    if (SPEC) {
        const u32 reg0 = spec[2 * ch.node], rcap = spec[2 * ch.node + 1];
        for (u32 d = tid; d < R; d += SK1_NT)
            glim[d] = rcapv ? rstart[nd.child_base + d] + rcapv[nd.child_base + d] : reg0 + (d + 1) * rcap;
    }
    u32 pl_base = 0;
    bool pl_pending = false;
    auto place_issue = [&]() {
        if ((u32)tid < R) {
            const u32 lo = cnt[tid], c = cnt[tid + 1] - lo;
            pl_base = 0;
            if (gc) {
                if (c)
                    pl_base = atomicAdd(&gc[tid], c);
            } else if (!SPEC) {
                pl_base = gpos[tid];
                gpos[tid] = pl_base + c;
            }
            gadj[tid] = 0u - lo;
            pl_pending = true;
        }
    };
    auto place_finish = [&]() {
        if (pl_pending) {
            gadj[tid] += pl_base;
            pl_pending = false;
        }
    };
    auto scan_counts = [&]() {
        u32 v = 0;
        if ((u32)tid <= R) {
            if (SPEC) {
                const u64 w = c64[tid];
                v = (u32)w;
                kacc += (u32)(w >> 32);
            } else {
                v = cnt[tid];
            }
        }
        block_scan_value<SK1_NT>(v, cnt, (int)R + 1, wtmp, tid);
    };
    for (u32 t0 = 0; t0 < ch.len; t0 += SK1_TILE) {
        const u32 n_tile = ch.len - t0 < (u32)SK1_TILE ? ch.len - t0 : (u32)SK1_TILE;
        asm volatile("" : "+v"(tid));
        for (u32 d = tid; d <= R; d += SK1_NT) {
            if (SPEC)
                c64[d] = 0;
            else
                cnt[d] = 0;
        }
        if (tid == 0) {
            split[0] = R;
            split[2] = 0;
        }
        __syncthreads();
        bool gather = n_tile != (u32)SK1_TILE, placed = false;
        if (!gather) {
            ull2_t rec[SK1_ITEMS];
#pragma unroll
            for (int j = 0; j < SK1_ITEMS; j++)
                rec[j] = src[t0 + tid + j * SK1_NT];
#pragma unroll
            for (int j = 0; j < SK1_ITEMS; j++) {
                const bool null = (rec[j].y >> 63) != 0;
                const u32 dg = null ? R : (u32)(rec[j].y >> shift) & dmask;
                if (SPEC)
                    atomicAdd(reinterpret_cast<unsigned long long *>(&c64[dg]),
                              null ? 1ull : 1ull | ((unsigned long long)(((u32)(rec[j].y >> 44) & 31u) + 1u) << 32));
                else
                    atomicAdd(&cnt[dg], 1u);
            }
            __syncthreads();
            scan_counts();
            const u32 n_valid = cnt[R];
            if ((u32)tid < R && cnt[tid] <= (u32)SK1_STAGE && cnt[tid + 1] > (u32)SK1_STAGE) {
                split[0] = (u32)tid;
                split[1] = cnt[tid];
                split[2] = n_valid - cnt[tid] > (u32)SK1_STAGE ? 1u : 0u;
            }
            place_issue();
            placed = true;
            __syncthreads();
            const u32 s_dig = split[0];
            gather = split[2] != 0;
            if (!gather) {
                const u32 s_off = s_dig < R ? split[1] : n_valid;
#pragma unroll
                for (int h = 0; h < 2; h++) {
                    const u32 lo = h ? s_off : 0u, hi = h ? n_valid : s_off;
                    if (lo == hi)
                        continue;
#pragma unroll
                    for (int j = 0; j < SK1_ITEMS; j++) {
                        const u32 dg = (u32)(rec[j].y >> shift) & dmask;
                        if (!(rec[j].y >> 63) && (dg >= s_dig) == (h != 0))
                            stage[atomicAdd(&cnt[dg], 1u) - lo] = rec[j];
                    }
                    place_finish();
                    __syncthreads();
#pragma unroll
                    for (int j = 0; j < (SK1_STAGE + SK1_NT - 1) / SK1_NT; j++) {
                        const u32 sl = lo + (u32)tid + (u32)j * SK1_NT;
                        if (sl >= hi)
                            continue;
                        const ull2_t r = stage[sl - lo];
                        const u32 d = (u32)(r.y >> shift) & dmask;
                        const u32 p = gadj[d] + sl;
                        if (!SPEC || p < glim[d])
                            dst_all[p] = r;
                        else
                            dropped = true;
                    }
                    __syncthreads();
                }
            } else {
                place_finish();
                for (u32 d = tid; d <= R; d += SK1_NT)
                    cnt[d] = 0;
                __syncthreads();
            }
        }
        if (gather) {
            u32 dig[SK1_ITEMS], rank[SK1_ITEMS];
#pragma unroll
            for (int j = 0; j < SK1_ITEMS; j++) {
                const u32 i = tid + j * SK1_NT;
                dig[j] = 0;
                rank[j] = 0;
                if (i < n_tile) {
                    const u64 m = reinterpret_cast<const u64 *>(src + t0 + i)[1];
                    const bool null = (m >> 63) != 0;
                    dig[j] = null ? R : (u32)(m >> shift) & dmask;
                    if (SPEC && !placed) {
                        rank[j] = (u32)atomicAdd(reinterpret_cast<unsigned long long *>(&c64[dig[j]]),
                                                 null ? 1ull : 1ull | ((unsigned long long)(((u32)(m >> 44) & 31u) + 1u) << 32));
                    } else {
                        rank[j] = atomicAdd(&cnt[dig[j]], 1u);
                    }
                }
            }
            __syncthreads();
            if (SPEC && !placed)
                scan_counts();
            else
                block_scan_small<SK1_NT>(cnt, (int)R + 1, wtmp, tid);
            if (!placed) {
                place_issue();
                place_finish();
            }
#pragma unroll
            for (int j = 0; j < SK1_ITEMS; j++) {
                const u32 i = tid + j * SK1_NT;
                if (i < n_tile)
                    idx[cnt[dig[j]] + rank[j]] = (unsigned short)i;
            }
            __syncthreads();
#pragma unroll
            for (int j = 0; j < SK1_ITEMS; j++) {
                const u32 sl = tid + j * SK1_NT;
                if (sl < cnt[R]) {
                    const ull2_t r = src[t0 + idx[sl]];
                    const u32 d = (u32)(r.y >> shift) & dmask;
                    const u32 p = gadj[d] + sl;
                    if (!SPEC || p < glim[d])
                        __builtin_nontemporal_store(r, &dst_all[p]);
                    else
                        dropped = true;
                }
            }
            __syncthreads();
        }
    }
    if (SPEC) {
        if ((u32)tid < R && kacc)
            atomicAdd(&kcount[nd.child_base + (u32)tid], kacc);
        if (dropped)
            *over = 1u;
    }
}

__host__ __device__ inline u32 sk_spec_cap(u32 len, u32 R)
{
    return ((u32)(((u64)len + (len >> 3)) / R) + 72u + 7u) & ~7u;
}
u64 sk_spec_span(u32 len, int bits) { return len ? (u64)sk_spec_cap(len, 1u << bits) << bits : 0; }

__global__ __launch_bounds__(SK_MAX_C0) void sk_spec_caps_kernel(const Node *__restrict__ nodes, u32 n_nodes, u32 *__restrict__ spec,
                                                                u32 *__restrict__ out)
{
    __shared__ u64 span[SK_MAX_C0];
    const u32 i = threadIdx.x;
    u32 cap = 0;
    u64 sp = 0;
    if (i < n_nodes && nodes[i].split) {
        cap = sk_spec_cap(nodes[i].len, 1u << nodes[i].split);
        sp = (u64)cap << nodes[i].split;
    }
    span[i] = sp;
    __syncthreads();
    if (i == 0) {
        u64 run = 0;
        for (u32 q = 0; q < (u32)SK_MAX_C0; q++) {
            const u64 c = span[q];
            span[q] = run;
            run += c;
        }
        out[0] = (u32)(run < 0xFFFFFFFFull ? run : 0xFFFFFFFFull);
        out[1] = run > 0xFFFFFFFFull ? 1u : 0u;
        out[2] = 0;
    }
    __syncthreads();
    if (i < n_nodes) {
        spec[2 * i] = (u32)(span[i] < 0xFFFFFFFFull ? span[i] : 0xFFFFFFFFull);
        spec[2 * i + 1] = cap;
    }
}

__global__ __launch_bounds__(ROW_STRIDE) void sk_spec_init_kernel(const Node *__restrict__ nodes, u32 n_nodes, const u32 *__restrict__ spec,
                                                                 u32 *__restrict__ gcur, const u32 *__restrict__ rstart)
{
    const u32 i = blockIdx.x, d = threadIdx.x;
    if (i >= n_nodes)
        return;
    const Node nd = nodes[i];
    if (nd.split && d < (1u << nd.split))
        gcur[(u64)nd.chunk_base * ROW_STRIDE + d] = rstart ? rstart[nd.child_base + d] : spec[2 * i] + d * spec[2 * i + 1];
}

__global__ __launch_bounds__(ROW_STRIDE) void sk_spec_nodes_kernel(const Node *__restrict__ nodes, u32 n_nodes, const u32 *__restrict__ spec,
                                                                  const u32 *__restrict__ gcur, Node *__restrict__ next,
                                                                  u32 *__restrict__ over, const u32 *__restrict__ rstart,
                                                                  const u32 *__restrict__ rcapv)
{
    const u32 i = blockIdx.x, d = threadIdx.x;
    if (i >= n_nodes)
        return;
    const Node nd = nodes[i];
    if (nd.split == 0) {
        if (d == 0) {
            Node o = nd;
            o.split = 0;
            next[nd.child_base] = o;
        }
        return;
    }
    if (d >= (1u << nd.split))
        return;
    const int bits = (int)nd.split, rem = (int)(nd.meta & 0xff);
    const u32 cap = rcapv ? rcapv[nd.child_base + d] : spec[2 * i + 1];
    const u32 start = rcapv ? rstart[nd.child_base + d] : spec[2 * i] + d * cap;
    u32 used = gcur[(u64)nd.chunk_base * ROW_STRIDE + d] - start;
    if (used > cap) {
        used = cap;
        *over = 1u;
    }
    Node c;
    c.start = start;
    c.len = used;
    c.meta = (u32)(rem - bits) | ((nd.meta & NODE_BUF) ^ NODE_BUF) | ((bits == rem) ? NODE_TERMINAL : 0u);
    c.split = 0;
    c.prefix = nd.prefix | ((u64)d << (rem - bits));
    c.child_base = 0;
    c.chunk_base = 0;
    next[nd.child_base + d] = c;
}

__device__ __forceinline__ u32 row16_excl_scan(u32 x)
{
    int v = (int)x;
    v += __builtin_amdgcn_update_dpp(0, v, 0x111, 0xf, 0xf, false);
    v += __builtin_amdgcn_update_dpp(0, v, 0x112, 0xf, 0xf, false);
    v += __builtin_amdgcn_update_dpp(0, v, 0x114, 0xf, 0xf, false);
    v += __builtin_amdgcn_update_dpp(0, v, 0x118, 0xf, 0xf, false);
    return (u32)v - x;
}

constexpr int SKF_SLICE = 4096;
int sk_flat_slice() { return SKF_SLICE; }

__global__ __launch_bounds__(256) void sk_slice_count_kernel(const Node *__restrict__ buckets, u32 nb, u32 *__restrict__ n_slices)
{
    const u32 i = blockIdx.x * blockDim.x + threadIdx.x;
    if (i < nb)
        n_slices[i] = (buckets[i].len + (u32)SKF_SLICE - 1u) / (u32)SKF_SLICE;
}

__global__ __launch_bounds__(256) void sk_slice_fill_kernel(const Node *__restrict__ buckets, u32 nb,
                                                            const u32 *__restrict__ slice_first, u32 *__restrict__ slice_rec0,
                                                            u32 *__restrict__ slice_nrec)
{
    const u32 lane = threadIdx.x & 63;
    const u32 i = blockIdx.x * 4 + (threadIdx.x >> 6);
    if (i >= nb)
        return;
    const u32 start = buckets[i].start, len = buckets[i].len, s0 = slice_first[i];
    const u32 ns = (len + (u32)SKF_SLICE - 1u) / (u32)SKF_SLICE;
    for (u32 j = lane; j < ns; j += 64) {
        slice_rec0[s0 + j] = start + j * (u32)SKF_SLICE;
        slice_nrec[s0 + j] = min((u32)SKF_SLICE, len - j * (u32)SKF_SLICE);
    }
}

__global__ __launch_bounds__(256) void sk_slice_kmers_kernel(const ull2_t *__restrict__ recs, const u32 *__restrict__ slice_rec0,
                                                             const u32 *__restrict__ slice_nrec, u32 n_slices,
                                                             u32 *__restrict__ slice_km)
{
    const int lane = threadIdx.x & 63;
    const u32 si = blockIdx.x * 4 + (threadIdx.x >> 6);
    if (si >= n_slices)
        return;
    const u64 *hi = reinterpret_cast<const u64 *>(recs + (u64)slice_rec0[si]) + 1;
    const u32 n = slice_nrec[si];
    u32 sum = 0;
    for (u32 r = lane; r < n; r += 64)
        sum += (u32)((__builtin_nontemporal_load(&hi[(u64)r * 2]) >> 44) & 31) + 1u;
    sum = wave_sum(sum);
    if (lane == 0)
        slice_km[si] = sum;
}

__global__ __launch_bounds__(256) void sk_slice_nodes_kernel(const Node *__restrict__ buckets, u32 nb,
                                                             const u32 *__restrict__ slice_first, const u32 *__restrict__ slice_koff,
                                                             u32 n_slices, const u32 *__restrict__ total_keys, u32 key_base, int k,
                                                             int check_kmers, Node *__restrict__ out,
                                                             unsigned long long *__restrict__ n_bad)
{
    const u32 i = blockIdx.x * blockDim.x + threadIdx.x;
    if (i >= nb)
        return;
    const u32 s0 = slice_first[i], s1 = i + 1 < nb ? slice_first[i + 1] : n_slices;
    const u32 k0 = s0 < n_slices ? slice_koff[s0] : *total_keys, k1 = s1 < n_slices ? slice_koff[s1] : *total_keys;
    Node nd;
    nd.prefix = 0;
    nd.start = key_base + k0;
    nd.len = k1 - k0;
    nd.meta = (u32)(2 * k);
    nd.split = 0;
    nd.child_base = 0;
    nd.chunk_base = 0;
    out[i] = nd;
    if (check_kmers && buckets[i].child_base != k1 - k0)
        atomicAdd(n_bad, 1ull);
}

__global__ __launch_bounds__(256) void sk_expand_flat_kernel(const ull2_t *__restrict__ recs, const u32 *__restrict__ slice_rec0,
                                                             const u32 *__restrict__ slice_nrec,
                                                             const u32 *__restrict__ slice_koff, u32 key_base, u32 n_slices, int k,
                                                             u32 lmax, u64 *__restrict__ keys)
{
    extern __shared__ __attribute__((aligned(16))) unsigned char skf_smem[];
    const int lane = threadIdx.x & 63, wave = threadIdx.x >> 6;
    const u32 si = blockIdx.x * 4 + (u32)wave;
    if (si >= n_slices)
        return;
    u64 *stage = reinterpret_cast<u64 *>(skf_smem) + (size_t)wave * 64 * lmax;
    const ull2_t *src = recs + (u64)slice_rec0[si];
    const u32 n = slice_nrec[si];
    const u64 kmask = kmer_mask(k);
    u64 out = (u64)key_base + slice_koff[si];
    ull2_t nxt;
    nxt.x = nxt.y = 0;
    if ((u32)lane < n)
        nxt = src[lane];
    for (u32 b0 = 0; b0 < n; b0 += 64) {
        const ull2_t rec = nxt;
        const bool have = b0 + (u32)lane < n;
        if (b0 + 64 + (u32)lane < n)
            nxt = src[b0 + 64 + lane];
        const u32 len = have ? (u32)((rec.y >> 44) & 31) + 1u : 0u;
        const u32 inc = wave_incl_scan(len);
        const u32 n_keys = (u32)__builtin_amdgcn_readlane((int)inc, 63);
        const u32 o = inc - len;
        const u64 hi = rec.y & (((u64)1 << 44) - 1);
        for (u32 j = 0; j < len; j++)
            stage[o + j] = key_mix(funnel(rec.x, hi, 2 * j) & kmask, k, kmask);
        sk_wave_fence();
        for (u32 s = lane; s < n_keys; s += 64)
            __builtin_nontemporal_store(stage[s], &keys[out + s]);
        sk_wave_fence();
        out += n_keys;
    }
}

__global__ __launch_bounds__(256) void sk_unmix_kernel(u64 *__restrict__ keys, u64 first, const unsigned long long *__restrict__ end,
                                                       int k)
{
    const u64 e = *end, mask = kmer_mask(k);
    for (u64 i = first + (u64)blockIdx.x * 256 + threadIdx.x; i < e; i += (u64)gridDim.x * 256)
        keys[i] = key_unmix(keys[i], k, mask);
}

hipError_t launch_sk_unmix(u64 *keys, u64 first, const u64 *end, u64 max_groups, int k, hipStream_t s)
{
    if (max_groups == 0)
        return hipSuccess;
    const u64 g = (max_groups + 1023) / 1024;
    hipLaunchKernelGGL(sk_unmix_kernel, dim3((u32)(g < 4096 ? g : 4096)), dim3(256), 0, s, keys, first,
                       reinterpret_cast<const unsigned long long *>(end), k);
    return hipGetLastError();
}

__global__ __launch_bounds__(256) void sk_take_heavy_kernel(Node *__restrict__ mids, const u32 *__restrict__ idx, u32 n_heavy,
                                                            const u32 *__restrict__ kcount, Node *__restrict__ out)
{
    const u32 j = blockIdx.x * blockDim.x + threadIdx.x;
    if (j >= n_heavy)
        return;
    const u32 i = idx[j];
    Node nd = mids[i];
    nd.child_base = kcount[i];
    out[j] = nd;
    mids[i].len = 0;
}

hipError_t launch_sk_take_heavy(Node *mids, const u32 *idx, u32 n_heavy, const u32 *kcount, Node *out, hipStream_t s)
{
    if (n_heavy == 0)
        return hipSuccess;
    hipLaunchKernelGGL(sk_take_heavy_kernel, dim3((n_heavy + 255) / 256), dim3(256), 0, s, mids, idx, n_heavy, kcount, out);
    return hipGetLastError();
}

hipError_t launch_sk_slice_count(const Node *buckets, u32 nb, u32 *n_slices, hipStream_t s)
{
    if (nb == 0)
        return hipSuccess;
    hipLaunchKernelGGL(sk_slice_count_kernel, dim3((nb + 255) / 256), dim3(256), 0, s, buckets, nb, n_slices);
    return hipGetLastError();
}

hipError_t launch_sk_slice_fill(const Node *buckets, u32 nb, const u32 *slice_first, u32 *slice_rec0, u32 *slice_nrec, hipStream_t s)
{
    if (nb == 0)
        return hipSuccess;
    hipLaunchKernelGGL(sk_slice_fill_kernel, dim3((nb + 3) / 4), dim3(256), 0, s, buckets, nb, slice_first, slice_rec0, slice_nrec);
    return hipGetLastError();
}

hipError_t launch_sk_slice_kmers(const void *recs, const u32 *slice_rec0, const u32 *slice_nrec, u32 n_slices, u32 *slice_km,
                                 hipStream_t s)
{
    if (n_slices == 0)
        return hipSuccess;
    hipLaunchKernelGGL(sk_slice_kmers_kernel, dim3((n_slices + 3) / 4), dim3(256), 0, s, reinterpret_cast<const ull2_t *>(recs),
                       slice_rec0, slice_nrec, n_slices, slice_km);
    return hipGetLastError();
}

hipError_t launch_sk_slice_nodes(const Node *buckets, u32 nb, const u32 *slice_first, const u32 *slice_koff, u32 n_slices,
                                 const u32 *total_keys, u32 key_base, int k, bool check_kmers, Node *out, u64 *n_bad, hipStream_t s)
{
    if (nb == 0)
        return hipSuccess;
    hipLaunchKernelGGL(sk_slice_nodes_kernel, dim3((nb + 255) / 256), dim3(256), 0, s, buckets, nb, slice_first, slice_koff, n_slices,
                       total_keys, key_base, k, check_kmers ? 1 : 0, out, reinterpret_cast<unsigned long long *>(n_bad));
    return hipGetLastError();
}

hipError_t launch_sk_expand_flat(const void *recs, const u32 *slice_rec0, const u32 *slice_nrec, const u32 *slice_koff, u32 key_base,
                                 u32 n_slices, int k, u64 *keys, hipStream_t s)
{
    if (n_slices == 0)
        return hipSuccess;
    u32 lmax = (u32)(54 - k + 1);
// ... 1022 lines not shown
        }
        if (ns == 1) {
            if (!failed) {
                const u32 groups = skb_emit(tab, cnt, ones, wtot, out_keys + obase, out_counts + obase);
                for (u32 i = groups + (u32)tid; i < nd.child_base; i += SKB_NT)
                    out_counts[obase + i] = 0;
                if (tid == 0) {
                    seg_off[li] = obase;
                    seg_cnt[li] = groups;
                    status[lq] = 0;
                    my_groups += groups;
                }
            } else {
                for (u32 i = tid; i < nd.child_base; i += SKB_NT)
                    out_counts[obase + i] = 0;
                if (tid == 0) {
                    seg_off[li] = obase;
                    seg_cnt[li] = 0;
                    status[lq] = 1;
                }
            }
        } else {
            const u64 pa = (u64)(mfirst[lq] + sj);
            u32 groups = SKB_FAILED;
            if (!failed)
                groups = skb_emit(tab, cnt, ones, wtot, part_keys + pa * SKB_SLOTS, part_cnts + pa * SKB_SLOTS);
            if (tid == 0)
                part_n[pa] = groups;
        }
        __syncthreads();
    }
    if (tid == 0 && my_groups)
        atomicAdd(n_groups, (unsigned long long)my_groups);
}

__global__ __launch_bounds__(SKB_NT) void sk_big_merge_kernel(const Node *__restrict__ fin, const u32 *__restrict__ list,
                                                              const u32 *__restrict__ list_off, const u32 *__restrict__ nsl,
                                                              const u32 *__restrict__ mfirst, u32 n_list,
                                                              unsigned long long *__restrict__ n_groups,
                                                              u64 *__restrict__ seg_off, u32 *__restrict__ seg_cnt,
                                                              u64 *__restrict__ out_keys, u32 *__restrict__ out_counts,
                                                              u32 *__restrict__ status, const u64 *__restrict__ part_keys,
                                                              const u32 *__restrict__ part_cnts, const u32 *__restrict__ part_n)
{
    constexpr int WAVES = SKB_NT / 64;
    __shared__ __attribute__((aligned(16))) u64 tab[SKB_SLOTS];
    __shared__ u32 cnt[SKB_SLOTS];
    __shared__ u32 wtot[WAVES], wnew[2][WAVES];
    __shared__ u32 ones;
    const int tid = threadIdx.x, lane = tid & 63, wave = tid >> 6;
    const u32 lq = blockIdx.x;
    if (lq >= n_list)
        return;
    const u32 ns = nsl[lq];
    if (ns <= 1)
        return;
    const u32 li = list[lq];
    const u64 obase = list_off[lq];
    for (int q = tid; q < SKB_SLOTS; q += SKB_NT) {
        tab[q] = SKB_EMPTY;
        cnt[q] = 0;
    }
    if (tid == 0)
        ones = 0;
    __syncthreads();
    bool failed = false;
    u32 distinct = 0, rpar = 0;
    for (u32 j = 0; j < ns && !failed; j++) {
        const u64 pa = (u64)(mfirst[lq] + j);
        const u32 n_e = part_n[pa];
        if (n_e == SKB_FAILED) {
            failed = true;
            break;
        }
        for (u32 r0 = 0; r0 < n_e; r0 += SKB_NT) {
            if (distinct > (u32)(SKB_SLOTS - SKB_NT - 64)) {
                failed = true;
                break;
            }
            u32 claimed = 0;
            const u32 e = r0 + (u32)tid;
            if (e < n_e) {
                const u64 kv = part_keys[pa * SKB_SLOTS + e];
                const u32 m = part_cnts[pa * SKB_SLOTS + e];
                if (kv == SKB_EMPTY) {
                    atomicAdd(&ones, m);
                } else {
                    u32 slot = ((((u32)kv ^ (u32)(kv >> 32)) * 0x9E3779B1u) >> 19) & (u32)(SKB_SLOTS - 1);
                    for (;;) {
                        const u64 old = atomicCAS(reinterpret_cast<unsigned long long *>(&tab[slot]), (unsigned long long)SKB_EMPTY,
                                                  (unsigned long long)kv);
                        if (old == SKB_EMPTY || old == kv) {
                            atomicAdd(&cnt[slot], m);
                            claimed = old == SKB_EMPTY ? 1u : 0u;
                            break;
                        }
                        slot = (slot + 1) & (u32)(SKB_SLOTS - 1);
                    }
                }
            }
            const u32 wc = wave_sum(claimed);
            if (lane == 0)
                wnew[rpar][wave] = wc;
            __syncthreads();
            u32 nb = 0, nt = 0;
            sk_wave_prefix16(wnew[rpar], WAVES, wave, lane, nb, nt);
            distinct += nt;
            rpar ^= 1;
        }
    }
    __syncthreads();
    if (!failed) {
        const u32 groups = skb_emit(tab, cnt, ones, wtot, out_keys + obase, out_counts + obase);
        if (tid == 0) {
            seg_off[li] = obase;
            seg_cnt[li] = groups;
            status[lq] = 0;
            atomicAdd(n_groups, (unsigned long long)groups);
        }
    } else {
        if (tid == 0) {
            seg_off[li] = obase;
            seg_cnt[li] = 0;
            status[lq] = 1;
        }
    }
}

u32 sk_big_slice_records() { return SKB_SLICE_REC; }
u64 sk_big_partial_slots() { return SKB_SLOTS; }

__global__ __launch_bounds__(256) void sk_node_lens_kernel(const Node *__restrict__ nodes, u32 n, u32 *__restrict__ lens)
{
    const u32 i = blockIdx.x * blockDim.x + threadIdx.x;
    if (i < n)
        lens[i] = nodes[i].len;
}

hipError_t launch_sk_node_lens(const Node *nodes, u32 n, u32 *lens, hipStream_t s)
{
    if (n == 0)
        return hipSuccess;
    hipLaunchKernelGGL(sk_node_lens_kernel, dim3((n + 255) / 256), dim3(256), 0, s, nodes, n, lens);
    return hipGetLastError();
}

hipError_t launch_sk_big_slices(const Node *fin, const u32 *list, u32 n_list, u32 *nsl, u32 *msl, hipStream_t s)
{
    if (n_list == 0)
        return hipSuccess;
    hipLaunchKernelGGL(sk_big_slices_kernel, dim3((n_list + 255) / 256), dim3(256), 0, s, fin, list, n_list, nsl, msl);
    return hipGetLastError();
}

hipError_t launch_sk_big_slice_fill(const u32 *nsl_raw, const u32 *sfirst, u32 n_list, u32 *sl_bucket, u32 *sl_idx, hipStream_t s)
{
    if (n_list == 0)
        return hipSuccess;
    hipLaunchKernelGGL(sk_big_slice_fill_kernel, dim3((n_list + 3) / 4), dim3(256), 0, s, nsl_raw, sfirst, n_list, sl_bucket, sl_idx);
    return hipGetLastError();
}

hipError_t launch_sk_count_big(const Node *fin, const u32 *list, const u32 *list_off, const u32 *nsl, const u32 *mfirst,
                               const u32 *sl_bucket, const u32 *sl_idx, u32 n_slices, u32 n_list, const void *recs, int k,
                               u64 *n_groups, u64 *seg_off, u32 *seg_cnt, u64 *out_keys, u32 *out_counts, u32 *status, u64 *part_keys,
                               u32 *part_cnts, u32 *part_n, bool any_sliced, hipStream_t s)
{
    if (n_slices == 0)
        return hipSuccess;
    int dev = 0, n_cu = 256, v = 0;
    if (hipGetDevice(&dev) == hipSuccess && hipDeviceGetAttribute(&v, hipDeviceAttributeMultiprocessorCount, dev) == hipSuccess && v > 0)
        n_cu = v;
    const u32 grid = std::min<u32>(n_slices, (u32)n_cu);
    hipLaunchKernelGGL(sk_count_big_kernel, dim3(grid), dim3(SKB_NT), 0, s, fin, list, list_off, nsl, mfirst, sl_bucket, sl_idx,
                       n_slices, reinterpret_cast<const ull2_t *>(recs), k, reinterpret_cast<unsigned long long *>(n_groups), seg_off,
                       seg_cnt, out_keys, out_counts, status, part_keys, part_cnts, part_n);
    if (any_sliced)
        hipLaunchKernelGGL(sk_big_merge_kernel, dim3(n_list), dim3(SKB_NT), 0, s, fin, list, list_off, nsl, mfirst, n_list,
                           reinterpret_cast<unsigned long long *>(n_groups), seg_off, seg_cnt, out_keys, out_counts, status,
                           part_keys, part_cnts, part_n);
    return hipGetLastError();
}

__device__ __forceinline__ u32 sk_bucket_class(const Node &nd, u32 cap, u32 big_limit)
{
    const u32 km = nd.child_base;
    if (km == 0)
        return 0u;
    if (km <= cap && nd.len <= (u32)SKC_MAXREC && nd.chunk_base <= (u32)SKC_MAXQ)
        return 1u;
    return km > 2 * cap && km <= big_limit ? 2u : 3u;
}

__global__ __launch_bounds__(256) void sk_select_flags_kernel(const Node *__restrict__ fin, u32 n_fin, u32 cap, u32 big_limit,
                                                              u32 *__restrict__ f_small, u32 *__restrict__ f_big,
                                                              u32 *__restrict__ k_range, u32 *__restrict__ k_big)
{
    const u32 i = blockIdx.x * blockDim.x + threadIdx.x;
    if (i >= n_fin)
        return;
    const u32 c = sk_bucket_class(fin[i], cap, big_limit);
    f_small[i] = c == 1u ? 1u : 0u;
    f_big[i] = c == 2u ? 1u : 0u;
    k_range[i] = c == 1u || c == 2u ? fin[i].child_base : 0u;
    k_big[i] = c == 2u ? fin[i].child_base : 0u;
}

__global__ __launch_bounds__(256) void sk_select_lists_kernel(const Node *__restrict__ fin, u32 n_fin, u32 cap, u32 big_limit,
                                                              const u32 *__restrict__ p_small, const u32 *__restrict__ p_big,
                                                              const u32 *__restrict__ kb_range, u32 *__restrict__ list_small,
                                                              u32 *__restrict__ off_small, u32 *__restrict__ list_big,
                                                              u32 *__restrict__ off_big)
{
    const u32 i = blockIdx.x * blockDim.x + threadIdx.x;
    if (i >= n_fin)
        return;
    const u32 c = sk_bucket_class(fin[i], cap, big_limit);
    if (c == 1u) {
        list_small[p_small[i]] = i;
        off_small[p_small[i]] = kb_range[i];
    } else if (c == 2u) {
        list_big[p_big[i]] = i;
        off_big[p_big[i]] = kb_range[i];
    }
}

__global__ __launch_bounds__(256) void sk_over_flags_kernel(const Node *__restrict__ fin, u32 n_fin, u32 cap, u32 big_limit,
                                                            const u32 *__restrict__ p_big, const u32 *__restrict__ big_status,
                                                            u32 *__restrict__ f_over, u32 *__restrict__ k_over)
{
    const u32 i = blockIdx.x * blockDim.x + threadIdx.x;
    if (i >= n_fin)
        return;
    const u32 c = sk_bucket_class(fin[i], cap, big_limit);
    const bool over = c == 3u || (c == 2u && big_status[p_big[i]] != 0);
    f_over[i] = over ? 1u : 0u;
    k_over[i] = over ? fin[i].child_base : 0u;
}

__global__ __launch_bounds__(256) void sk_over_list_kernel(const Node *__restrict__ fin, u32 n_fin, const u32 *__restrict__ f_raw,
                                                           const u32 *__restrict__ p_over, const u32 *__restrict__ kb_over,
                                                           Node *__restrict__ over_nodes, u32 *__restrict__ over_kbase)
{
    const u32 i = blockIdx.x * blockDim.x + threadIdx.x;
    if (i >= n_fin || !f_raw[i])
        return;
    over_nodes[p_over[i]] = fin[i];
    over_kbase[p_over[i]] = kb_over[i];
}

hipError_t launch_sk_select_flags(const Node *fin, u32 n_fin, u32 cap, u32 big_limit, u32 *f_small, u32 *f_big, u32 *k_range,
                                  u32 *k_big, hipStream_t s)
{
    if (n_fin == 0)
        return hipSuccess;
    hipLaunchKernelGGL(sk_select_flags_kernel, dim3((n_fin + 255) / 256), dim3(256), 0, s, fin, n_fin, cap, big_limit, f_small, f_big,
                       k_range, k_big);
    return hipGetLastError();
}

hipError_t launch_sk_select_lists(const Node *fin, u32 n_fin, u32 cap, u32 big_limit, const u32 *p_small, const u32 *p_big,
                                  const u32 *kb_range, u32 *list_small, u32 *off_small, u32 *list_big, u32 *off_big, hipStream_t s)
{
    if (n_fin == 0)
        return hipSuccess;
    hipLaunchKernelGGL(sk_select_lists_kernel, dim3((n_fin + 255) / 256), dim3(256), 0, s, fin, n_fin, cap, big_limit, p_small, p_big,
                       kb_range, list_small, off_small, list_big, off_big);
    return hipGetLastError();
}

hipError_t launch_sk_over_flags(const Node *fin, u32 n_fin, u32 cap, u32 big_limit, const u32 *p_big, const u32 *big_status,
                                u32 *f_over, u32 *k_over, hipStream_t s)
{
    if (n_fin == 0)
        return hipSuccess;
    hipLaunchKernelGGL(sk_over_flags_kernel, dim3((n_fin + 255) / 256), dim3(256), 0, s, fin, n_fin, cap, big_limit, p_big, big_status,
                       f_over, k_over);
    return hipGetLastError();
}

hipError_t launch_sk_over_list(const Node *fin, u32 n_fin, const u32 *f_raw, const u32 *p_over, const u32 *kb_over, Node *over_nodes,
                               u32 *over_kbase, hipStream_t s)
{
    if (n_fin == 0)
        return hipSuccess;
    hipLaunchKernelGGL(sk_over_list_kernel, dim3((n_fin + 255) / 256), dim3(256), 0, s, fin, n_fin, f_raw, p_over, kb_over, over_nodes,
                       over_kbase);
    return hipGetLastError();
}

static int sk_dbg()
{
#ifdef DNAGPU_STAMPS
    const char *e = getenv("DNAGPU_DEBUG_SK");
    return e ? atoi(e) : 0;
#else
    return 0;
#endif
}

template <int W, bool BATCH>
static void launch_front(bool scatter, u32 n_chunks, hipStream_t s, const Chunk *chunks, const u64 *words, u64 n_words,
                         u64 first, int k, u32 lmax, u32 mmask, u32 c0n, u32 b1mask, u32 r0n, u32 *hist, const u32 *tot, void *recs,
                         u32 *aux, const u32 *marks, u64 n_mark_words)
{
    if (scatter)
        hipLaunchKernelGGL((sk_scatter0_kernel<W, BATCH>), dim3(n_chunks), dim3(SK_NT), 0, s, chunks, n_chunks, words, n_words, first,
                           k, lmax, mmask, c0n, b1mask, r0n, hist, tot, reinterpret_cast<ull2_t *>(recs), sk_dbg(), aux, marks,
                           n_mark_words);
    else
        hipLaunchKernelGGL((sk_hist0_kernel<W, BATCH>), dim3(n_chunks), dim3(SK_NT), 0, s, chunks, n_chunks, words, n_words, first,
                           lmax, mmask, c0n, b1mask, r0n, hist, aux, marks, n_mark_words);
}

int sk_min_k() { return 20; }
int sk_minimizer_len(int k) { return k >= 23 ? 15 : (k >= 21 ? 13 : 12); }

hipError_t launch_sk_level0(bool scatter, const Chunk *chunks, u32 n_chunks, const u64 *words, u64 n_words, u64 first, int k,
                            u32 c0n, u32 b1bits, u32 r0bits, u32 *hist, const u32 *tot, void *recs, hipStream_t s, u32 *aux,
                            const u32 *marks, u64 n_mark_words)
{
    if (n_chunks == 0)
        return hipSuccess;
    const int m = sk_minimizer_len(k);
    const int w = k - m + 1;
    const u32 mmask = (1u << (2 * m)) - 1u;
    u32 lmax = (u32)(54 - k + 1);
    if (lmax > 32)
        lmax = 32;
    const u32 b1mask = (1u << b1bits) - 1, r0n = 1u << r0bits;
    if (r0n > (u32)SK_MAX_C0)
        return hipErrorInvalidValue;
#define SK_CASE(W_) case W_: \
        if (marks) launch_front<W_, true>(scatter, n_chunks, s, chunks, words, n_words, first, k, lmax, mmask, c0n, b1mask, r0n, hist, tot, recs, aux, marks, n_mark_words); \
        else launch_front<W_, false>(scatter, n_chunks, s, chunks, words, n_words, first, k, lmax, mmask, c0n, b1mask, r0n, hist, tot, recs, aux, nullptr, 0); \
        break;
    switch (w) {
        SK_CASE(9) SK_CASE(10) SK_CASE(11) SK_CASE(12) SK_CASE(13) SK_CASE(14) SK_CASE(15) SK_CASE(16) SK_CASE(17) SK_CASE(18)
    default: return hipErrorInvalidValue;
    }
#undef SK_CASE
    return hipGetLastError();
}

hipError_t launch_sk_sample_chunks(Chunk *chunks, u32 n_chunks, u32 stride, u32 len, u32 n, hipStream_t s)
{
    if (n_chunks == 0)
        return hipSuccess;
    hipLaunchKernelGGL(sk_sample_chunks_kernel, dim3((n_chunks + 255) / 256), dim3(256), 0, s, chunks, n_chunks, stride, len, n);
    return hipGetLastError();
}

int sk_slab_words() { return 18 * SK_MAX_C0 + 4; }

hipError_t launch_sk_slab_init(const u32 *est, u32 r0bits, u32 chunk_rows, u32 sampled, u32 n_chunks, u32 *slab, Node *nodes,
                               hipStream_t s)
{
    hipLaunchKernelGGL(sk_slab_init_kernel, dim3(1), dim3(SK_MAX_C0), 0, s, est, 1u << r0bits, chunk_rows, sampled, n_chunks,
                       (u32)(32 - r0bits), slab, nodes);
    return hipGetLastError();
}

hipError_t launch_sk_hist1(const Node *nodes, const Chunk *chunks, u32 n_chunks, const void *recs, u32 *hist, u32 *kcount,
                           hipStream_t s, bool by_d2)
{
    if (n_chunks == 0)
        return hipSuccess;
    hipLaunchKernelGGL(sk_hist1_kernel, dim3(n_chunks), dim3(SK1_NT), 0, s, nodes, chunks, n_chunks,
                       reinterpret_cast<const ull2_t *>(recs), hist, kcount, by_d2 ? 59 : 49);
    return hipGetLastError();
}

hipError_t launch_sk_scatter1(const Node *nodes, const Chunk *chunks, u32 n_chunks, const void *src, void *dst, const u32 *hist,
                              const u32 *tot, hipStream_t s, bool by_d2, u32 *gcur)
{
    if (n_chunks == 0)
        return hipSuccess;
    hipLaunchKernelGGL(sk_scatter1_kernel<false>, dim3(n_chunks), dim3(SK1_NT), 0, s, nodes, chunks, n_chunks,
                       reinterpret_cast<const ull2_t *>(src), reinterpret_cast<ull2_t *>(dst), hist, tot, by_d2 ? 59 : 49, gcur,
                       nullptr, nullptr, nullptr, nullptr, nullptr);
    return hipGetLastError();
}

hipError_t launch_sk_spec_regions(const Node *nodes, u32 n_nodes, u32 *spec, u32 *out, u32 *gcur, hipStream_t s, const u32 *rstart)
{
    if (n_nodes == 0 || n_nodes > (u32)SK_MAX_C0)
        return hipErrorInvalidValue;
    hipLaunchKernelGGL(sk_spec_caps_kernel, dim3(1), dim3(SK_MAX_C0), 0, s, nodes, n_nodes, spec, out);
    hipLaunchKernelGGL(sk_spec_init_kernel, dim3(n_nodes), dim3(ROW_STRIDE), 0, s, nodes, n_nodes, spec, gcur, rstart);
    return hipGetLastError();
}

hipError_t launch_sk_sampled_regions(const Node *nodes, const Chunk *samples, u32 n_samples, const void *recs, u32 n_mid, u32 *est,
                                     u32 *rcap, u32 *rstart, u32 *scan_tmp, u32 *total, hipStream_t s)
{
    hipError_t e = hipMemsetAsync(est, 0, (size_t)n_mid * sizeof(u32), s);
    if (e != hipSuccess)
        return e;
    if (n_samples)
        hipLaunchKernelGGL(sk_sample1_kernel, dim3(n_samples), dim3(SK1_NT), 0, s, nodes, samples, n_samples,
                           reinterpret_cast<const ull2_t *>(recs), est);
    hipLaunchKernelGGL(sk_sampled_caps_kernel, dim3((n_mid + 255) / 256), dim3(256), 0, s, est, n_mid, rcap);
    e = hipGetLastError();
    if (e != hipSuccess)
        return e;
    return launch_scan_u32(rcap, rstart, n_mid, scan_tmp, total, s);
}

hipError_t launch_sk_scatter1_spec(const Node *nodes, const Chunk *chunks, u32 n_chunks, const void *src, void *dst, u32 *gcur,
                                   const u32 *spec, u32 *kcount, u32 *over, hipStream_t s, const u32 *rstart, const u32 *rcap)
{
    if (n_chunks == 0)
        return hipSuccess;
    hipLaunchKernelGGL(sk_scatter1_kernel<true>, dim3(n_chunks), dim3(SK1_NT), 0, s, nodes, chunks, n_chunks,
                       reinterpret_cast<const ull2_t *>(src), reinterpret_cast<ull2_t *>(dst), nullptr, nullptr, 49, gcur, spec,
                       kcount, over, rstart, rcap);
    return hipGetLastError();
}

hipError_t launch_sk_spec_nodes(const Node *nodes, u32 n_nodes, const u32 *spec, const u32 *gcur, Node *next, u32 *over,
                                hipStream_t s, const u32 *rstart, const u32 *rcap)
{
    if (n_nodes == 0)
        return hipSuccess;
    hipLaunchKernelGGL(sk_spec_nodes_kernel, dim3(n_nodes), dim3(ROW_STRIDE), 0, s, nodes, n_nodes, spec, gcur, next, over, rstart,
                       rcap);
    return hipGetLastError();
}

__global__ __launch_bounds__(256) void sk_heavy_finals_kernel(const Node *__restrict__ kids, u32 n, const u32 *__restrict__ kcount,
                                                              Node *__restrict__ out)
{
    const u32 i = blockIdx.x * blockDim.x + threadIdx.x;
    if (i >= n)
        return;
    Node o;
    o.start = kids[i].start;
    o.len = kids[i].len;
    o.meta = 0;
    o.split = 0;
    o.prefix = 0;
    o.child_base = kids[i].len ? kcount[i] : 0u;
    o.chunk_base = ~0u;
    out[i] = o;
}

hipError_t launch_sk_heavy_finals(const Node *kids, u32 n, const u32 *kcount, Node *out, hipStream_t s)
{
    if (n == 0)
        return hipSuccess;
    hipLaunchKernelGGL(sk_heavy_finals_kernel, dim3((n + 255) / 256), dim3(256), 0, s, kids, n, kcount, out);
    return hipGetLastError();
}


}
```

Baseline: 165.2 billion k-mers/s.

## Replace slab null-record padding with per-slab fill directory in level-1 readers

The level-0 scatter no longer writes null records into the unused tail of each per-chunk slab. Instead it records each slab's fill count in a directory, and a new prefix kernel turns those counts into dense offsets and node lengths. Level-1 hist, sample and scatter kernels use the directory to map dense indices to slab slots, so they read only live records. This removes the padding-store traffic and the dead-record reads downstream, at the cost of an index-mapping lookup in each level-1 reader and an extra directory allocation and prefix pass.

```diff
diff --git a/dna-sequences-pg-extension_amd/binding.py b/dna-sequences-pg-extension_amd/binding.py
--- a/dna-sequences-pg-extension_amd/binding.py
+++ b/dna-sequences-pg-extension_amd/binding.py
@@ -477,6 +477,16 @@
     def set_debug(self, flags):
         _chk(lib().dnagpu_set_debug(self.h, int(flags) | self._base_debug))
 
+    def debug_dir_map(self, fills, cap, off, length, tile=8192):
+        f = np.ascontiguousarray(fills, dtype=np.uint32)
+        out = np.zeros(max(int(length), 1), np.uint32)
+        u32p = C.POINTER(C.c_uint32)
+        fn = lib().dnagpu_debug_dir_map
+        fn.restype = C.c_int
+        fn.argtypes = [C.c_void_p, u32p, C.c_uint32, C.c_uint32, C.c_uint32, C.c_uint32, C.c_uint32, u32p]
+        _chk(fn(self.h, f.ctypes.data_as(u32p), len(f), int(cap), int(off), int(length), int(tile), out.ctypes.data_as(u32p)))
+        return out[:int(length)]
+
     def close(self):
         if self.h:
             lib().dnagpu_destroy(self.h)
diff --git a/dna-sequences-pg-extension_amd/csrc/kernels.hpp b/dna-sequences-pg-extension_amd/csrc/kernels.hpp
--- a/dna-sequences-pg-extension_amd/csrc/kernels.hpp
+++ b/dna-sequences-pg-extension_amd/csrc/kernels.hpp
@@ -170,28 +170,35 @@
 int sk_max_c0();
 hipError_t launch_sk_level0(bool scatter, const Chunk *chunks, u32 n_chunks, const u64 *words, u64 n_words, u64 first, int k,
                             u32 c0n, u32 b1bits, u32 r0bits, u32 *hist, const u32 *tot, void *recs, hipStream_t s,
-                            u32 *aux = nullptr, const u32 *marks = nullptr, u64 n_mark_words = 0);
+                            u32 *aux = nullptr, const u32 *marks = nullptr, u64 n_mark_words = 0, u32 *dir = nullptr);
+struct SkDir {
+    const u32 *prefix = nullptr;
+    const u32 *caps = nullptr;
+    u32 n_slabs = 0;
+};
+hipError_t launch_sk_slab_prefix(u32 *dir, u32 r0bits, u32 n_slabs, Node *nodes, hipStream_t s);
+hipError_t launch_sk_dir_map(const SkDir &dir, u32 off, u32 len, u32 tile, u32 *out, hipStream_t s);
 hipError_t launch_sk_sample_chunks(Chunk *chunks, u32 n_chunks, u32 stride, u32 len, u32 n, hipStream_t s);
 int sk_slab_words();
 u32 sk_slab_cap(u32 est, u64 chunk_rows, u64 sampled);
 hipError_t launch_sk_slab_init(const u32 *est, u32 r0bits, u32 chunk_rows, u32 sampled, u32 n_chunks, u32 *slab, Node *nodes,
                                hipStream_t s);
 hipError_t launch_sk_hist1(const Node *nodes, const Chunk *chunks, u32 n_chunks, const void *recs, u32 *hist, u32 *kcount,
-                           hipStream_t s, bool by_d2 = false);
+                           hipStream_t s, bool by_d2 = false, const SkDir *dir = nullptr);
 hipError_t launch_sk_scatter1(const Node *nodes, const Chunk *chunks, u32 n_chunks, const void *src, void *dst, const u32 *hist,
-                              const u32 *tot, hipStream_t s, bool by_d2 = false, u32 *gcur = nullptr);
+                              const u32 *tot, hipStream_t s, bool by_d2 = false, u32 *gcur = nullptr, const SkDir *dir = nullptr);
 u64 sk_spec_span(u32 len, int bits);
 hipError_t launch_sk_spec_regions(const Node *nodes, u32 n_nodes, u32 *spec, u32 *out, u32 *gcur, hipStream_t s,
                                   const u32 *rstart = nullptr);
 hipError_t launch_sk_scatter1_spec(const Node *nodes, const Chunk *chunks, u32 n_chunks, const void *src, void *dst, u32 *gcur,
                                    const u32 *spec, u32 *kcount, u32 *over, hipStream_t s, const u32 *rstart = nullptr,
-                                   const u32 *rcap = nullptr);
+                                   const u32 *rcap = nullptr, const SkDir *dir = nullptr);
 hipError_t launch_sk_spec_nodes(const Node *nodes, u32 n_nodes, const u32 *spec, const u32 *gcur, Node *next, u32 *over,
                                 hipStream_t s, const u32 *rstart = nullptr, const u32 *rcap = nullptr);
 u32 sk_sample1_len();
 u32 sk_sample1_every();
 hipError_t launch_sk_sampled_regions(const Node *nodes, const Chunk *samples, u32 n_samples, const void *recs, u32 n_mid, u32 *est,
-                                     u32 *rcap, u32 *rstart, u32 *scan_tmp, u32 *total, hipStream_t s);
+                                     u32 *rcap, u32 *rstart, u32 *scan_tmp, u32 *total, hipStream_t s, const SkDir *dir = nullptr);
 hipError_t launch_sk_heavy_finals(const Node *kids, u32 n, const u32 *kcount, Node *out, hipStream_t s);
 int sk_flat_slice();
 hipError_t launch_sk_take_heavy(Node *mids, const u32 *idx, u32 n_heavy, const u32 *kcount, Node *out, hipStream_t s);
diff --git a/dna-sequences-pg-extension_amd/csrc/sk_host.hip b/dna-sequences-pg-extension_amd/csrc/sk_host.hip
--- a/dna-sequences-pg-extension_amd/csrc/sk_host.hip
+++ b/dna-sequences-pg-extension_amd/csrc/sk_host.hip
@@ -156,7 +156,7 @@
 
 constexpr u64 SK_SLAB_MIN_ROWS = (u64)1 << 29;
 static int sk_level0_slab(dnagpu_ctx *ctx, PoolScope &ps, const SkRows &rows, int k, const SkGeom &g, void **rec0_out, Node **coarse,
-                          u32 *n_coarse, std::vector<u32> *lens, u64 *n_recs, u64 *rec0_cap, bool *ok)
+                          u32 *n_coarse, std::vector<u32> *lens, u64 *n_recs, u64 *rec0_cap, bool *ok, SkDir *dir, u64 *extent)
 {
     hipStream_t st = ctx->stream;
     const dnagpu_dna *dna = rows.dna;
@@ -176,14 +176,17 @@
     for (u32 i = 0; i < n_samp; i++)
         sampled += std::min<u64>(samp_len, n - (u64)i * samp_stride);
     Chunk *samp = nullptr;
-    u32 *est = nullptr, *slab = nullptr;
+    u32 *est = nullptr, *slab = nullptr, *fills = nullptr;
     Node *nodes = nullptr;
+    const size_t dir_words = (size_t)r0n * ((size_t)l0.n_chunks + 1);
     RC_TRY(ps.alloc((size_t)n_samp, &samp));
     RC_TRY(ps.alloc((size_t)sk_max_c0(), &est));
     RC_TRY(ps.alloc((size_t)sk_slab_words(), &slab));
     RC_TRY(ps.alloc((size_t)r0n, &nodes));
+    RC_TRY(ps.alloc(dir_words, &fills));
     prof_mark(ctx, "sk_sample0");
     HIP_TRY(hipMemsetAsync(est, 0, (size_t)sk_max_c0() * sizeof(u32), st));
+    HIP_TRY(hipMemsetAsync(fills, 0, dir_words * sizeof(u32), st));
     HIP_TRY(launch_sk_sample_chunks(samp, n_samp, (u32)samp_stride, (u32)samp_len, (u32)n, st));
     HIP_TRY(launch_sk_level0(false, samp, n_samp, dna->words, dna->n_words, first, k, g.c0n, (u32)g.b1, (u32)g.r0bits, nullptr, nullptr,
                              nullptr, st, est, rows.marks, rows.n_mark_words));
@@ -191,14 +194,12 @@
     std::vector<u32> h_est(r0n);
     RC_TRY(read_back(ctx, h_est.data(), est, (size_t)r0n * sizeof(u32)));
     u64 tot = 0, span = 0, span1 = 0;
-    lens->assign(r0n, 0);
     for (u32 d = 0; d < r0n; d++) {
         tot += h_est[d];
         const u64 len = (u64)sk_slab_cap(h_est[d], chunk_rows, sampled) * l0.n_chunks;
         span += len;
         if (len > 0xFFFFFFFFull)
             return DNAGPU_OK;
-        (*lens)[d] = (u32)len;
         span1 += sk_spec_span((u32)len, g.b1);
     }
     if (tot == 0 || !sk_even(h_est.data(), r0n, 1.05) || span > 0xFFFFFFFFull)
@@ -207,10 +208,15 @@
     void *rec0 = nullptr;
     RC_TRY(pool_alloc(ctx, (size_t)std::max<u64>(cap, 1) * 16, &rec0));
     prof_mark(ctx, "sk_scatter0");
-    const hipError_t e = launch_sk_level0(true, l0.chunks, l0.n_chunks, dna->words, dna->n_words, first, k, g.c0n, (u32)g.b1,
-                                          (u32)g.r0bits, nullptr, nullptr, rec0, st, slab, rows.marks, rows.n_mark_words);
-    u32 status[2] = {1, 0};
-    int rc = e == hipSuccess ? read_back(ctx, status, slab + 18 * (size_t)sk_max_c0(), sizeof status) : DNAGPU_ERR_HIP;
+    hipError_t e = launch_sk_level0(true, l0.chunks, l0.n_chunks, dna->words, dna->n_words, first, k, g.c0n, (u32)g.b1,
+                                          (u32)g.r0bits, nullptr, nullptr, rec0, st, slab, rows.marks, rows.n_mark_words, fills);
+    const size_t c0 = (size_t)sk_max_c0();
+    std::vector<u32> back(c0 + 2, 0);
+    back[c0] = 1;
+    u32 *status = back.data() + c0;
+    if (e == hipSuccess)
+        e = launch_sk_slab_prefix(fills, (u32)g.r0bits, l0.n_chunks, nodes, st);
+    int rc = e == hipSuccess ? read_back(ctx, back.data(), slab + 17 * c0, back.size() * sizeof(u32)) : DNAGPU_ERR_HIP;
     if (rc != DNAGPU_OK || status[0] || status[1] != (u32)span || (ctx->debug_flags & DNAGPU_DEBUG_SLAB0_OVERFLOW)) {
         pool_free(ctx, rec0);
         if (e != hipSuccess)
@@ -218,18 +224,26 @@
         return rc;
     }
     ps.ptrs.push_back(rec0);
+    lens->assign(back.begin(), back.begin() + r0n);
+    u64 dense = 0;
+    for (u32 d = 0; d < r0n; d++)
+        dense += back[d];
     *rec0_out = rec0;
     *coarse = nodes;
     *n_coarse = r0n;
-    *n_recs = span;
+    *n_recs = dense;
     *rec0_cap = cap;
+    *extent = span;
+    dir->prefix = fills;
+    dir->caps = slab;
+    dir->n_slabs = l0.n_chunks;
     *ok = true;
     return DNAGPU_OK;
 }
 
 static int sk_levels12(dnagpu_ctx *ctx, PoolScope &ps, const SkGeom &g, Node *coarse, u32 n_coarse, void *rec0, u64 n_recs, u64 n,
                        void **recs, Node **fin, u32 *n_fin, SkHeavy *heavy, u64 *n_kmers, const u32 *host_lens = nullptr,
-                       u64 rec0_cap = 0)
+                       u64 rec0_cap = 0, const SkDir *dir = nullptr, u64 extent = 0)
 {
     hipStream_t st = ctx->stream;
     const int b1 = g.b1;
@@ -297,7 +311,7 @@
         prof_mark(ctx, "sk_sample1");
         if (!samp.empty())
             HIP_TRY(hipMemcpyAsync(d_samp, samp.data(), samp.size() * sizeof(Chunk), hipMemcpyHostToDevice, st));
-        HIP_TRY(launch_sk_sampled_regions(coarse, d_samp, (u32)samp.size(), rec0, l1.n_next, est, rcapv, rstart, stmp, tot1, st));
+        HIP_TRY(launch_sk_sampled_regions(coarse, d_samp, (u32)samp.size(), rec0, l1.n_next, est, rcapv, rstart, stmp, tot1, st, dir));
         u32 total = 0;
         RC_TRY(read_back(ctx, &total, tot1, sizeof total));
         u64 chk = 0;
@@ -315,11 +329,11 @@
         u32 *status = d_lens + l1.n_next;
         prof_mark(ctx, "sk_spec1");
         HIP_TRY(launch_sk_spec_regions(coarse, n_coarse, sp, status, gcur, st, sampled ? rstart : nullptr));
-        RC_TRY(pool_alloc(ctx, (size_t)std::max<u64>(std::max(n_recs, span), 1) * 16, &rec1));
+        RC_TRY(pool_alloc(ctx, (size_t)std::max<u64>(std::max(std::max(n_recs, span), extent), 1) * 16, &rec1));
         ps.ptrs.push_back(rec1);
         prof_mark(ctx, "sk_scatter1");
         HIP_TRY(launch_sk_scatter1_spec(coarse, l1.chunks, l1.n_chunks, rec0, rec1, gcur, sp, kcount, status + 2, st,
-                                        sampled ? rstart : nullptr, sampled ? rcapv : nullptr));
+                                        sampled ? rstart : nullptr, sampled ? rcapv : nullptr, dir));
         HIP_TRY(launch_sk_spec_nodes(coarse, n_coarse, sp, gcur, l1.next, status + 2, st, sampled ? rstart : nullptr,
                                      sampled ? rcapv : nullptr));
         HIP_TRY(launch_sk_node_lens(l1.next, l1.n_next, d_lens, st));
@@ -334,7 +348,7 @@
     }
     if (!spec) {
         prof_mark(ctx, "sk_hist1");
-        HIP_TRY(launch_sk_hist1(coarse, l1.chunks, l1.n_chunks, rec0, l1.hist, kcount, st));
+        HIP_TRY(launch_sk_hist1(coarse, l1.chunks, l1.n_chunks, rec0, l1.hist, kcount, st, false, dir));
         prof_mark(ctx, "sk_prefix1");
         HIP_TRY(launch_level_prefix(coarse, l1.chunks, l1.n_chunks, n_coarse, (u32)chunk_recs, l1.hist, l1.tot, st, n_coarse));
         HIP_TRY(launch_level_children(coarse, n_coarse, l1.tot, l1.next, nullptr, nullptr, nullptr, 0, st));
@@ -369,12 +383,12 @@
 
     if (!moved) {
         if (!rec1) {
-            RC_TRY(pool_alloc(ctx, (size_t)std::max<u64>(n_recs, 1) * 16, &rec1));
+            RC_TRY(pool_alloc(ctx, (size_t)std::max<u64>(std::max(n_recs, extent), 1) * 16, &rec1));
             ps.ptrs.push_back(rec1);
         }
         prof_mark(ctx, "sk_scatter1");
         HIP_TRY(hipMemcpyAsync(gcur, l1.tot, (size_t)std::max<u32>(l1.n_chunks, 1) * ROW_STRIDE * sizeof(u32), hipMemcpyDeviceToDevice, st));
-        HIP_TRY(launch_sk_scatter1(coarse, l1.chunks, l1.n_chunks, rec0, rec1, l1.hist, l1.tot, st, false, gcur));
+        HIP_TRY(launch_sk_scatter1(coarse, l1.chunks, l1.n_chunks, rec0, rec1, l1.hist, l1.tot, st, false, gcur, dir));
     }
 
     const u32 nh = (u32)heavy_idx.size();
@@ -640,13 +654,15 @@
     u64 rec0_cap = 0;
     std::vector<u32> lens;
     bool slabs = false;
+    SkDir dir;
+    u64 extent = 0;
     const unsigned dbg = ctx->debug_flags;
     if (!(dbg & DNAGPU_DEBUG_NO_SLAB0) && (rows.n >= SK_SLAB_MIN_ROWS || (dbg & (DNAGPU_DEBUG_SLAB0 | DNAGPU_DEBUG_SLAB0_OVERFLOW))))
-        RC_TRY(sk_level0_slab(ctx, ps, rows, k, g, &rec0, &coarse, &n_coarse, &lens, &n_recs, &rec0_cap, &slabs));
+        RC_TRY(sk_level0_slab(ctx, ps, rows, k, g, &rec0, &coarse, &n_coarse, &lens, &n_recs, &rec0_cap, &slabs, &dir, &extent));
     if (!slabs)
         RC_TRY(sk_level0(ctx, ps, rows, k, g, &rec0, &coarse, &n_coarse, &lens, &n_recs, &rec0_cap));
     RC_TRY(sk_levels12(ctx, ps, g, coarse, n_coarse, rec0, n_recs, n_kmers_expected, &recs, &fin, &n_fin, &heavy, &n_kmers,
-                       lens.size() == n_coarse ? lens.data() : nullptr, rec0_cap));
+                       lens.size() == n_coarse ? lens.data() : nullptr, rec0_cap, slabs ? &dir : nullptr, slabs ? extent : 0));
     return count_sk_tail(ctx, ps, recs, fin, n_fin, heavy, n_kmers_expected, k, h);
 }
 
@@ -827,3 +843,34 @@
     return DNAGPU_OK;
     });
 }
+
+extern "C" int dnagpu_debug_dir_map(dnagpu_ctx *ctx, const uint32_t *fills, uint32_t n_slabs, uint32_t cap, uint32_t off, uint32_t len,
+                                    uint32_t tile, uint32_t *slots)
+{
+    if (!ctx || !fills || !slots || n_slabs == 0)
+        return DNAGPU_ERR_BAD_ARG;
+    hipStream_t st = ctx->stream;
+    PoolScope ps(ctx);
+    u32 *row = nullptr, *caps = nullptr, *out = nullptr;
+    Node *node = nullptr;
+    RC_TRY(ps.alloc((size_t)n_slabs + 1, &row));
+    RC_TRY(ps.alloc(1, &caps));
+    RC_TRY(ps.alloc(1, &node));
+    RC_TRY(ps.alloc(std::max<u32>(len, 1), &out));
+    HIP_TRY(hipMemcpyAsync(row, fills, (size_t)n_slabs * sizeof(u32), hipMemcpyHostToDevice, st));
+    HIP_TRY(hipMemcpyAsync(caps, &cap, sizeof(u32), hipMemcpyHostToDevice, st));
+    HIP_TRY(hipMemsetAsync(node, 0, sizeof(Node), st));
+    HIP_TRY(launch_sk_slab_prefix(row, 0, n_slabs, node, st));
+    Node nd;
+    RC_TRY(read_back(ctx, &nd, node, sizeof nd));
+    if ((u64)off + len > nd.len)
+        return DNAGPU_ERR_BAD_ARG;
+    SkDir dir;
+    dir.prefix = row;
+    dir.caps = caps;
+    dir.n_slabs = n_slabs;
+    HIP_TRY(launch_sk_dir_map(dir, off, len, tile, out, st));
+    if (len)
+        RC_TRY(read_back(ctx, slots, out, (size_t)len * sizeof(u32)));
+    return DNAGPU_OK;
+}
diff --git a/dna-sequences-pg-extension_amd/csrc/superkmer_kernels.hip b/dna-sequences-pg-extension_amd/csrc/superkmer_kernels.hip
--- a/dna-sequences-pg-extension_amd/csrc/superkmer_kernels.hip
+++ b/dna-sequences-pg-extension_amd/csrc/superkmer_kernels.hip
@@ -521,7 +521,8 @@
                                                             const u32 *__restrict__ hist, const u32 *__restrict__ tot,
                                                             ull2_t *__restrict__ recs, int dbg,
                                                             u32 *__restrict__ slab ,
-                                                            const u32 *__restrict__ marks, u64 n_mark_words)
+                                                            const u32 *__restrict__ marks, u64 n_mark_words,
+                                                            u32 *__restrict__ dir )
 {
     __shared__ u32 gpos[SK_MAX_C0];
     __shared__ u32 gend[SK_MAX_C0], gbeg[SK_MAX_C0];
@@ -622,15 +623,14 @@
         if (dropped)
             slab[18 * SK_MAX_C0] = 1u;
         __syncthreads();
-        ull2_t null_rec;
-        null_rec.x = 0;
-        null_rec.y = (unsigned long long)1 << 63;
-        for (u32 d = (u32)wave; d < r0n; d += SK_NT / 64) {
-            const u32 e = gend[d], u = gpos[d] < e ? gpos[d] : e;
-            for (u32 i = u + (u32)lane; i < e; i += 64)
-                __builtin_nontemporal_store(null_rec, &recs[i]);
-            if (lane == 0 && u > gbeg[d])
-                atomicAdd(&slab[17 * SK_MAX_C0 + d], u - gbeg[d]);
+        for (u32 d = (u32)tid; d < r0n; d += SK_NT) {
+            const u32 b = gbeg[d], cap = gend[d] - b;
+            if (cap == 0)
+                continue;
+            const u32 u = (gpos[d] < gend[d] ? gpos[d] : gend[d]) - b;
+            dir[(u64)d * (n_chunks + 1) + (b - slab[SK_MAX_C0 + 16 * d + 1]) / cap] = u;
+            if (u)
+                atomicAdd(&slab[17 * SK_MAX_C0 + d], u);
         }
     }
 }
@@ -698,6 +698,7 @@
         const u32 start = (u32)(sc[d] < 0xFFFFFFFFull ? sc[d] : 0xFFFFFFFFull);
         slab[d] = cap;
         slab[SK_MAX_C0 + 16 * d] = start;
+        slab[SK_MAX_C0 + 16 * d + 1] = start;
         slab[17 * SK_MAX_C0 + d] = 0;
         Node o;
         o.start = start;
@@ -711,13 +712,146 @@
     }
 }
 
+__global__ __launch_bounds__(256) void sk_slab_prefix_kernel(u32 *__restrict__ dir, u32 n_slabs, Node *__restrict__ nodes)
+{
+    __shared__ u32 part[256];
+    __shared__ u32 wtmp[4];
+    const int tid = threadIdx.x;
+    u32 *row = dir + (u64)blockIdx.x * (n_slabs + 1);
+    const u32 per = (n_slabs + 255u) / 256u;
+    const u32 b = (u32)tid * per < n_slabs ? (u32)tid * per : n_slabs, e = b + per < n_slabs ? b + per : n_slabs;
+    u32 sum = 0;
+    for (u32 i = b; i < e; i++)
+        sum += row[i];
+    const u32 total = block_scan_value<256>(sum, part, 256, wtmp, tid);
+    u32 run = part[tid];
+    for (u32 i = b; i < e; i++) {
+        const u32 v = row[i];
+        row[i] = run;
+        run += v;
+    }
+    if (tid == 0) {
+        row[n_slabs] = total;
+        nodes[blockIdx.x].len = total;
+    }
+}
+
+constexpr u32 SK_DIR_WIN = 256;
+struct SkDirView {
+    const u32 *row;
+    const u32 *bnd;
+    u32 n_slabs, cap, s0;
+};
+template <int NT>
+__device__ __forceinline__ void sk_dir_open(SkDirView &v, const SkDir &dir, u32 node, u32 off, u32 *bnd, u32 *s0_sh, int tid)
+{
+    v.row = dir.prefix + (u64)node * (dir.n_slabs + 1);
+    v.bnd = bnd;
+    v.n_slabs = dir.n_slabs;
+    v.cap = (u32)__builtin_amdgcn_readfirstlane((int)dir.caps[node]);
+    if (tid == 0)
+        *s0_sh = 0;
+    __syncthreads();
+    for (u32 s = (u32)tid; s < v.n_slabs; s += NT)
+        if (v.row[s] <= off && off < v.row[s + 1])
+            *s0_sh = s;
+    __syncthreads();
+    v.s0 = (u32)__builtin_amdgcn_readfirstlane((int)*s0_sh);
+    for (u32 t = (u32)tid; t <= SK_DIR_WIN; t += NT)
+        bnd[t] = v.row[v.s0 + t < v.n_slabs ? v.s0 + t : v.n_slabs];
+    __syncthreads();
+}
+__device__ __forceinline__ u32 sk_dir_slot_win(const SkDirView &v, u32 i, u32 &q)
+{
+    while (i >= v.bnd[q + 1])
+        q++;
+    return (v.s0 + q) * v.cap + (i - v.bnd[q]);
+}
+__device__ __forceinline__ u32 sk_dir_slot(const SkDirView &v, u32 i, u32 &q)
+{
+    while (q < SK_DIR_WIN && i >= v.bnd[q + 1])
+        q++;
+    if (q < SK_DIR_WIN)
+        return (v.s0 + q) * v.cap + (i - v.bnd[q]);
+    u32 lo = v.s0 + SK_DIR_WIN, hi = v.n_slabs;
+    while (hi - lo > 1) {
+        const u32 mid = lo + (hi - lo) / 2;
+        if (v.row[mid] <= i)
+            lo = mid;
+        else
+            hi = mid;
+    }
+    return lo * v.cap + (i - v.row[lo]);
+}
+template <int NT>
+__device__ __forceinline__ bool sk_dir_tile(SkDirView &v, const SkDir &dir, u32 node, bool begin, u32 first, u32 n, u32 *bnd,
+                                            u32 *s0_sh, int tid, u32 &qt)
+{
+    if (begin || first + n > (u32)__builtin_amdgcn_readfirstlane((int)bnd[SK_DIR_WIN])) {
+        sk_dir_open<NT>(v, dir, node, first, bnd, s0_sh, tid);
+        qt = 0;
+        if (first + n > (u32)__builtin_amdgcn_readfirstlane((int)bnd[SK_DIR_WIN]))
+            return false;
+    }
+    (void)sk_dir_slot_win(v, first, qt);
+    qt = (u32)__builtin_amdgcn_readfirstlane((int)qt);
+    return true;
+}
+
+__device__ __forceinline__ bool sk_dir_rows(const SkDirView &v, u32 first, u32 qt, int lane, u32 &b, u32 &d0, u32 &d1)
+{
+    const u32 i0 = first + ((u32)lane & 7u) * 1024u, i1 = i0 + 1023u;
+    u32 q = qt;
+    while (i0 >= v.bnd[q + 1])
+        q++;
+    b = v.bnd[q + 1];
+    d0 = (v.s0 + q) * v.cap - v.bnd[q];
+    d1 = d0;
+    bool ok = true;
+    if (i1 >= b) {
+        u32 p = q + 1;
+        while (p + 1 < SK_DIR_WIN && v.bnd[p + 1] == v.bnd[p])
+            p++;
+        d1 = (v.s0 + p) * v.cap - v.bnd[p];
+        ok = i1 < v.bnd[p + 1];
+    }
+    return __ballot(ok) == ~0ull;
+}
+
+__global__ __launch_bounds__(1024) void sk_dir_map_kernel(SkDir dir, u32 off, u32 len, u32 tile, u32 *__restrict__ out)
+{
+    __shared__ u32 bnd[SK_DIR_WIN + 1], s0_sh;
+    const int tid = threadIdx.x;
+    SkDirView dv;
+    u32 qt = 0;
+    for (u32 t0 = 0; t0 < len; t0 += tile) {
+        const u32 n_tile = len - t0 < tile ? len - t0 : tile;
+        const bool in_win = sk_dir_tile<1024>(dv, dir, 0, t0 == 0, off + t0, n_tile, bnd, &s0_sh, tid, qt);
+        u32 q = in_win ? qt : 0u, rb = 0, rd0 = 0, rd1 = 0;
+        if (in_win && n_tile == 8192u && sk_dir_rows(dv, off + t0, qt, tid & 63, rb, rd0, rd1)) {
+#pragma unroll
+            for (int j = 0; j < 8; j++) {
+                const u32 i = off + t0 + (u32)tid + (u32)j * 1024u;
+                const u32 b = (u32)__builtin_amdgcn_readlane((int)rb, j);
+                out[i - off] = i + (i >= b ? (u32)__builtin_amdgcn_readlane((int)rd1, j) : (u32)__builtin_amdgcn_readlane((int)rd0, j));
+            }
+        } else {
+            for (u32 i = (u32)tid; i < n_tile; i += 1024)
+                out[t0 + i] = in_win ? sk_dir_slot_win(dv, off + t0 + i, q) : sk_dir_slot(dv, off + t0 + i, q);
+        }
+        __syncthreads();
+    }
+}
+
 constexpr int SK1_NT = 1024;
+template <bool DIR>
 __global__ __launch_bounds__(SK1_NT) void sk_hist1_kernel(const Node *__restrict__ nodes, const Chunk *__restrict__ chunks,
                                                           u32 n_chunks, const ull2_t *__restrict__ recs,
-                                                          u32 *__restrict__ hist, u32 *__restrict__ kcount, int shift)
+                                                          u32 *__restrict__ hist, u32 *__restrict__ kcount, int shift, SkDir dir)
 {
     __shared__ u32 h[ROW_STRIDE];
     __shared__ u32 kc[ROW_STRIDE];
+    __shared__ u32 bnd[DIR ? SK_DIR_WIN + 1 : 1], s0_sh;
     if (blockIdx.x >= n_chunks)
         return;
     const Chunk ch = chunks[blockIdx.x];
@@ -727,17 +861,24 @@
         h[d] = 0;
         kc[d] = 0;
     }
+    constexpr bool by_dir = DIR;
+    SkDirView dv;
+    u32 q = 0;
+    if (by_dir)
+        sk_dir_open<SK1_NT>(dv, dir, ch.node, ch.off, bnd, &s0_sh, (int)threadIdx.x);
     __syncthreads();
-    const u64 *hi = reinterpret_cast<const u64 *>(recs + (u64)nd.start + ch.off) + 1;
+    const u64 *hi = reinterpret_cast<const u64 *>(recs + (u64)nd.start + (by_dir ? 0u : ch.off)) + 1;
     u32 i = threadIdx.x;
     for (; i + 3u * SK1_NT < ch.len; i += 4u * SK1_NT) {
         u64 m[4];
 #pragma unroll
-        for (int j = 0; j < 4; j++)
-            m[j] = __builtin_nontemporal_load(&hi[(u64)(i + (u32)j * SK1_NT) * 2]);
-#pragma unroll
         for (int j = 0; j < 4; j++) {
-            if (m[j] >> 63)
+            const u32 at = i + (u32)j * SK1_NT;
+            m[j] = __builtin_nontemporal_load(&hi[(u64)(by_dir ? sk_dir_slot(dv, ch.off + at, q) : at) * 2]);
+        }
+#pragma unroll
+        for (int j = 0; j < 4; j++) {
+            if (!DIR && (m[j] >> 63))
                 continue;
             const u32 d1 = (u32)(m[j] >> shift) & (R - 1);
             atomicAdd(&h[d1], 1u);
@@ -745,8 +886,8 @@
         }
     }
     for (; i < ch.len; i += SK1_NT) {
-        const u64 m = __builtin_nontemporal_load(&hi[(u64)i * 2]);
-        if (m >> 63)
+        const u64 m = __builtin_nontemporal_load(&hi[(u64)(by_dir ? sk_dir_slot(dv, ch.off + i, q) : i) * 2]);
+        if (!DIR && (m >> 63))
             continue;
         const u32 d1 = (u32)(m >> shift) & (R - 1);
         atomicAdd(&h[d1], 1u);
@@ -764,10 +905,13 @@
 constexpr u32 SK1_SAMPLE_LEN = 1024, SK1_SAMPLE_EVERY = 8;
 u32 sk_sample1_len() { return SK1_SAMPLE_LEN; }
 u32 sk_sample1_every() { return SK1_SAMPLE_EVERY; }
+template <bool DIR>
 __global__ __launch_bounds__(SK1_NT) void sk_sample1_kernel(const Node *__restrict__ nodes, const Chunk *__restrict__ chunks,
-                                                            u32 n_chunks, const ull2_t *__restrict__ recs, u32 *__restrict__ est)
+                                                            u32 n_chunks, const ull2_t *__restrict__ recs, u32 *__restrict__ est,
+                                                            SkDir dir)
 {
     __shared__ u32 h[ROW_STRIDE];
+    __shared__ u32 bnd[DIR ? SK_DIR_WIN + 1 : 1], s0_sh;
     if (blockIdx.x >= n_chunks)
         return;
     const Chunk ch = chunks[blockIdx.x];
@@ -775,11 +919,16 @@
     const u32 R = 1u << nd.split;
     for (u32 d = threadIdx.x; d < R; d += SK1_NT)
         h[d] = 0;
+    constexpr bool by_dir = DIR;
+    SkDirView dv;
+    u32 q = 0;
+    if (by_dir && ch.len)
+        sk_dir_open<SK1_NT>(dv, dir, ch.node, ch.off, bnd, &s0_sh, (int)threadIdx.x);
     __syncthreads();
-    const u64 *hi = reinterpret_cast<const u64 *>(recs + (u64)nd.start + ch.off) + 1;
+    const u64 *hi = reinterpret_cast<const u64 *>(recs + (u64)nd.start + (by_dir ? 0u : ch.off)) + 1;
     for (u32 i = threadIdx.x; i < ch.len; i += SK1_NT) {
-        const u64 m = __builtin_nontemporal_load(&hi[(u64)i * 2]);
-        if (!(m >> 63))
+        const u64 m = __builtin_nontemporal_load(&hi[(u64)(by_dir ? sk_dir_slot(dv, ch.off + i, q) : i) * 2]);
+        if (DIR || !(m >> 63))
             atomicAdd(&h[(u32)(m >> 49) & (R - 1)], 1u);
     }
     __syncthreads();
@@ -801,16 +950,18 @@
 constexpr int SK1_ITEMS = 8;
 constexpr int SK1_TILE = SK1_NT * SK1_ITEMS;
 constexpr int SK1_STAGE = SK1_TILE / 2 + 64;
-template <bool SPEC>
+template <bool SPEC, bool DIR>
 __global__ __launch_bounds__(SK1_NT, 8) void sk_scatter1_kernel(const Node *__restrict__ nodes, const Chunk *__restrict__ chunks,
                                                              u32 n_chunks, const ull2_t *__restrict__ src_all,
                                                              ull2_t *__restrict__ dst_all, const u32 *__restrict__ hist,
                                                              const u32 *__restrict__ tot, int shift, u32 *__restrict__ gcur,
                                                              const u32 *__restrict__ spec, u32 *__restrict__ kcount,
                                                              u32 *__restrict__ over, const u32 *__restrict__ rstart,
-                                                             const u32 *__restrict__ rcapv )
+                                                             const u32 *__restrict__ rcapv ,
+                                                             SkDir dir)
 {
     __shared__ u32 cnt[ROW_STRIDE];
+    __shared__ u32 bnd[DIR ? SK_DIR_WIN + 1 : 1], s0_sh;
     __shared__ u32 glim[SPEC ? ROW_STRIDE : 1];
     __shared__ u32 gadj[ROW_STRIDE];
     __shared__ u32 gpos[SPEC ? 1 : ROW_STRIDE];
@@ -832,9 +983,11 @@
     if (!SPEC && !gc)
         for (u32 d = tid; d < R; d += SK1_NT)
             gpos[d] = trow[d] + hrow[d];
-    const ull2_t *src = src_all + (u64)nd.start + ch.off;
+    const ull2_t *src = src_all + (u64)nd.start + (DIR ? 0u : ch.off);
     const u32 dmask = R - 1;
     bool dropped = false;
+    SkDirView dv;
+    u32 qt = 0;
     if (SPEC) {
         const u32 reg0 = spec[2 * ch.node], rcap = spec[2 * ch.node + 1];
         for (u32 d = tid; d < R; d += SK1_NT)
@@ -878,6 +1031,9 @@
     };
     for (u32 t0 = 0; t0 < ch.len; t0 += SK1_TILE) {
         const u32 n_tile = ch.len - t0 < (u32)SK1_TILE ? ch.len - t0 : (u32)SK1_TILE;
+        bool in_win = true;
+        if (DIR)
+            in_win = sk_dir_tile<SK1_NT>(dv, dir, ch.node, t0 == 0, ch.off + t0, n_tile, bnd, &s0_sh, tid, qt);
         asm volatile("" : "+v"(tid));
         for (u32 d = tid; d <= R; d += SK1_NT) {
             if (SPEC)
@@ -890,15 +1046,28 @@
             split[2] = 0;
         }
         __syncthreads();
-        bool gather = n_tile != (u32)SK1_TILE, placed = false;
+        u32 rb = 0, rd0 = 0, rd1 = 0;
+        if (DIR && in_win && n_tile == (u32)SK1_TILE)
+            in_win = sk_dir_rows(dv, ch.off + t0, qt, tid & 63, rb, rd0, rd1);
+        bool gather = n_tile != (u32)SK1_TILE || !in_win, placed = false;
         if (!gather) {
             ull2_t rec[SK1_ITEMS];
-#pragma unroll
-            for (int j = 0; j < SK1_ITEMS; j++)
-                rec[j] = src[t0 + tid + j * SK1_NT];
+            if (DIR) {
+#pragma unroll
+                for (int j = 0; j < SK1_ITEMS; j++) {
+                    const u32 i = ch.off + t0 + (u32)tid + (u32)j * SK1_NT;
+                    const u32 b = (u32)__builtin_amdgcn_readlane((int)rb, j);
+                    rec[j] = src[i + (i >= b ? (u32)__builtin_amdgcn_readlane((int)rd1, j)
+                                             : (u32)__builtin_amdgcn_readlane((int)rd0, j))];
+                }
+            } else {
+#pragma unroll
+                for (int j = 0; j < SK1_ITEMS; j++)
+                    rec[j] = src[t0 + tid + j * SK1_NT];
+            }
 #pragma unroll
             for (int j = 0; j < SK1_ITEMS; j++) {
-                const bool null = (rec[j].y >> 63) != 0;
+                const bool null = !DIR && (rec[j].y >> 63) != 0;
                 const u32 dg = null ? R : (u32)(rec[j].y >> shift) & dmask;
                 if (SPEC)
                     atomicAdd(reinterpret_cast<unsigned long long *>(&c64[dg]),
@@ -929,7 +1098,7 @@
 #pragma unroll
                     for (int j = 0; j < SK1_ITEMS; j++) {
                         const u32 dg = (u32)(rec[j].y >> shift) & dmask;
-                        if (!(rec[j].y >> 63) && (dg >= s_dig) == (h != 0))
+                        if ((DIR || !(rec[j].y >> 63)) && (dg >= s_dig) == (h != 0))
                             stage[atomicAdd(&cnt[dg], 1u) - lo] = rec[j];
                     }
                     place_finish();
@@ -958,14 +1127,15 @@
         }
         if (gather) {
             u32 dig[SK1_ITEMS], rank[SK1_ITEMS];
+            u32 q = qt;
 #pragma unroll
             for (int j = 0; j < SK1_ITEMS; j++) {
                 const u32 i = tid + j * SK1_NT;
                 dig[j] = 0;
                 rank[j] = 0;
                 if (i < n_tile) {
-                    const u64 m = reinterpret_cast<const u64 *>(src + t0 + i)[1];
-                    const bool null = (m >> 63) != 0;
+                    const u64 m = reinterpret_cast<const u64 *>(src + (DIR ? sk_dir_slot(dv, ch.off + t0 + i, q) : t0 + i))[1];
+                    const bool null = !DIR && (m >> 63) != 0;
                     dig[j] = null ? R : (u32)(m >> shift) & dmask;
                     if (SPEC && !placed) {
                         rank[j] = (u32)atomicAdd(reinterpret_cast<unsigned long long *>(&c64[dig[j]]),
@@ -995,7 +1165,8 @@
             for (int j = 0; j < SK1_ITEMS; j++) {
                 const u32 sl = tid + j * SK1_NT;
                 if (sl < cnt[R]) {
-                    const ull2_t r = src[t0 + idx[sl]];
+                    u32 qg = qt;
+                    const ull2_t r = src[DIR ? sk_dir_slot(dv, ch.off + t0 + idx[sl], qg) : t0 + idx[sl]];
                     const u32 d = (u32)(r.y >> shift) & dmask;
                     const u32 p = gadj[d] + sl;
                     if (!SPEC || p < glim[d])
@@ -2624,12 +2795,12 @@
 template <int W, bool BATCH>
 static void launch_front(bool scatter, u32 n_chunks, hipStream_t s, const Chunk *chunks, const u64 *words, u64 n_words,
                          u64 first, int k, u32 lmax, u32 mmask, u32 c0n, u32 b1mask, u32 r0n, u32 *hist, const u32 *tot, void *recs,
-                         u32 *aux, const u32 *marks, u64 n_mark_words)
+                         u32 *aux, const u32 *marks, u64 n_mark_words, u32 *dir)
 {
     if (scatter)
         hipLaunchKernelGGL((sk_scatter0_kernel<W, BATCH>), dim3(n_chunks), dim3(SK_NT), 0, s, chunks, n_chunks, words, n_words, first,
                            k, lmax, mmask, c0n, b1mask, r0n, hist, tot, reinterpret_cast<ull2_t *>(recs), sk_dbg(), aux, marks,
-                           n_mark_words);
+                           n_mark_words, dir);
     else
         hipLaunchKernelGGL((sk_hist0_kernel<W, BATCH>), dim3(n_chunks), dim3(SK_NT), 0, s, chunks, n_chunks, words, n_words, first,
                            lmax, mmask, c0n, b1mask, r0n, hist, aux, marks, n_mark_words);
@@ -2640,10 +2811,12 @@
 
 hipError_t launch_sk_level0(bool scatter, const Chunk *chunks, u32 n_chunks, const u64 *words, u64 n_words, u64 first, int k,
                             u32 c0n, u32 b1bits, u32 r0bits, u32 *hist, const u32 *tot, void *recs, hipStream_t s, u32 *aux,
-                            const u32 *marks, u64 n_mark_words)
+                            const u32 *marks, u64 n_mark_words, u32 *dir)
 {
     if (n_chunks == 0)
         return hipSuccess;
+    if (scatter && (aux != nullptr) != (dir != nullptr))
+        return hipErrorInvalidValue;
     const int m = sk_minimizer_len(k);
     const int w = k - m + 1;
     const u32 mmask = (1u << (2 * m)) - 1u;
@@ -2654,8 +2827,8 @@
     if (r0n > (u32)SK_MAX_C0)
         return hipErrorInvalidValue;
 #define SK_CASE(W_) case W_: \
-        if (marks) launch_front<W_, true>(scatter, n_chunks, s, chunks, words, n_words, first, k, lmax, mmask, c0n, b1mask, r0n, hist, tot, recs, aux, marks, n_mark_words); \
-        else launch_front<W_, false>(scatter, n_chunks, s, chunks, words, n_words, first, k, lmax, mmask, c0n, b1mask, r0n, hist, tot, recs, aux, nullptr, 0); \
+        if (marks) launch_front<W_, true>(scatter, n_chunks, s, chunks, words, n_words, first, k, lmax, mmask, c0n, b1mask, r0n, hist, tot, recs, aux, marks, n_mark_words, dir); \
+        else launch_front<W_, false>(scatter, n_chunks, s, chunks, words, n_words, first, k, lmax, mmask, c0n, b1mask, r0n, hist, tot, recs, aux, nullptr, 0, dir); \
         break;
     switch (w) {
         SK_CASE(9) SK_CASE(10) SK_CASE(11) SK_CASE(12) SK_CASE(13) SK_CASE(14) SK_CASE(15) SK_CASE(16) SK_CASE(17) SK_CASE(18)
@@ -2683,24 +2856,47 @@
     return hipGetLastError();
 }
 
+hipError_t launch_sk_slab_prefix(u32 *dir, u32 r0bits, u32 n_slabs, Node *nodes, hipStream_t s)
+{
+    hipLaunchKernelGGL(sk_slab_prefix_kernel, dim3(1u << r0bits), dim3(256), 0, s, dir, n_slabs, nodes);
+    return hipGetLastError();
+}
+
+hipError_t launch_sk_dir_map(const SkDir &dir, u32 off, u32 len, u32 tile, u32 *out, hipStream_t s)
+{
+    if (len == 0 || tile == 0)
+        return hipSuccess;
+    hipLaunchKernelGGL(sk_dir_map_kernel, dim3(1), dim3(1024), 0, s, dir, off, len, tile, out);
+    return hipGetLastError();
+}
+
 hipError_t launch_sk_hist1(const Node *nodes, const Chunk *chunks, u32 n_chunks, const void *recs, u32 *hist, u32 *kcount,
-                           hipStream_t s, bool by_d2)
+                           hipStream_t s, bool by_d2, const SkDir *dir)
 {
     if (n_chunks == 0)
         return hipSuccess;
-    hipLaunchKernelGGL(sk_hist1_kernel, dim3(n_chunks), dim3(SK1_NT), 0, s, nodes, chunks, n_chunks,
-                       reinterpret_cast<const ull2_t *>(recs), hist, kcount, by_d2 ? 59 : 49);
+    if (dir)
+        hipLaunchKernelGGL(sk_hist1_kernel<true>, dim3(n_chunks), dim3(SK1_NT), 0, s, nodes, chunks, n_chunks,
+                           reinterpret_cast<const ull2_t *>(recs), hist, kcount, by_d2 ? 59 : 49, *dir);
+    else
+        hipLaunchKernelGGL(sk_hist1_kernel<false>, dim3(n_chunks), dim3(SK1_NT), 0, s, nodes, chunks, n_chunks,
+                           reinterpret_cast<const ull2_t *>(recs), hist, kcount, by_d2 ? 59 : 49, SkDir{});
     return hipGetLastError();
 }
 
 hipError_t launch_sk_scatter1(const Node *nodes, const Chunk *chunks, u32 n_chunks, const void *src, void *dst, const u32 *hist,
-                              const u32 *tot, hipStream_t s, bool by_d2, u32 *gcur)
+                              const u32 *tot, hipStream_t s, bool by_d2, u32 *gcur, const SkDir *dir)
 {
     if (n_chunks == 0)
         return hipSuccess;
-    hipLaunchKernelGGL(sk_scatter1_kernel<false>, dim3(n_chunks), dim3(SK1_NT), 0, s, nodes, chunks, n_chunks,
-                       reinterpret_cast<const ull2_t *>(src), reinterpret_cast<ull2_t *>(dst), hist, tot, by_d2 ? 59 : 49, gcur,
-                       nullptr, nullptr, nullptr, nullptr, nullptr);
+    if (dir)
+        hipLaunchKernelGGL((sk_scatter1_kernel<false, true>), dim3(n_chunks), dim3(SK1_NT), 0, s, nodes, chunks, n_chunks,
+                           reinterpret_cast<const ull2_t *>(src), reinterpret_cast<ull2_t *>(dst), hist, tot, by_d2 ? 59 : 49, gcur,
+                           nullptr, nullptr, nullptr, nullptr, nullptr, *dir);
+    else
+        hipLaunchKernelGGL((sk_scatter1_kernel<false, false>), dim3(n_chunks), dim3(SK1_NT), 0, s, nodes, chunks, n_chunks,
+                           reinterpret_cast<const ull2_t *>(src), reinterpret_cast<ull2_t *>(dst), hist, tot, by_d2 ? 59 : 49, gcur,
+                           nullptr, nullptr, nullptr, nullptr, nullptr, SkDir{});
     return hipGetLastError();
 }
 
@@ -2714,14 +2910,17 @@
 }
 
 hipError_t launch_sk_sampled_regions(const Node *nodes, const Chunk *samples, u32 n_samples, const void *recs, u32 n_mid, u32 *est,
-                                     u32 *rcap, u32 *rstart, u32 *scan_tmp, u32 *total, hipStream_t s)
+                                     u32 *rcap, u32 *rstart, u32 *scan_tmp, u32 *total, hipStream_t s, const SkDir *dir)
 {
     hipError_t e = hipMemsetAsync(est, 0, (size_t)n_mid * sizeof(u32), s);
     if (e != hipSuccess)
         return e;
-    if (n_samples)
-        hipLaunchKernelGGL(sk_sample1_kernel, dim3(n_samples), dim3(SK1_NT), 0, s, nodes, samples, n_samples,
-                           reinterpret_cast<const ull2_t *>(recs), est);
+    if (n_samples && dir)
+        hipLaunchKernelGGL(sk_sample1_kernel<true>, dim3(n_samples), dim3(SK1_NT), 0, s, nodes, samples, n_samples,
+                           reinterpret_cast<const ull2_t *>(recs), est, *dir);
+    else if (n_samples)
+        hipLaunchKernelGGL(sk_sample1_kernel<false>, dim3(n_samples), dim3(SK1_NT), 0, s, nodes, samples, n_samples,
+                           reinterpret_cast<const ull2_t *>(recs), est, SkDir{});
     hipLaunchKernelGGL(sk_sampled_caps_kernel, dim3((n_mid + 255) / 256), dim3(256), 0, s, est, n_mid, rcap);
     e = hipGetLastError();
     if (e != hipSuccess)
@@ -2730,13 +2929,19 @@
 }
 
 hipError_t launch_sk_scatter1_spec(const Node *nodes, const Chunk *chunks, u32 n_chunks, const void *src, void *dst, u32 *gcur,
-                                   const u32 *spec, u32 *kcount, u32 *over, hipStream_t s, const u32 *rstart, const u32 *rcap)
+                                   const u32 *spec, u32 *kcount, u32 *over, hipStream_t s, const u32 *rstart, const u32 *rcap,
+                                   const SkDir *dir)
 {
     if (n_chunks == 0)
         return hipSuccess;
-    hipLaunchKernelGGL(sk_scatter1_kernel<true>, dim3(n_chunks), dim3(SK1_NT), 0, s, nodes, chunks, n_chunks,
-                       reinterpret_cast<const ull2_t *>(src), reinterpret_cast<ull2_t *>(dst), nullptr, nullptr, 49, gcur, spec,
-                       kcount, over, rstart, rcap);
+    if (dir)
+        hipLaunchKernelGGL((sk_scatter1_kernel<true, true>), dim3(n_chunks), dim3(SK1_NT), 0, s, nodes, chunks, n_chunks,
+                           reinterpret_cast<const ull2_t *>(src), reinterpret_cast<ull2_t *>(dst), nullptr, nullptr, 49, gcur, spec,
+                           kcount, over, rstart, rcap, *dir);
+    else
+        hipLaunchKernelGGL((sk_scatter1_kernel<true, false>), dim3(n_chunks), dim3(SK1_NT), 0, s, nodes, chunks, n_chunks,
+                           reinterpret_cast<const ull2_t *>(src), reinterpret_cast<ull2_t *>(dst), nullptr, nullptr, 49, gcur, spec,
+                           kcount, over, rstart, rcap, SkDir{});
     return hipGetLastError();
 }
 
```

Result: no change. 164.1 billion k-mers/s (-0.7%).
